# irecsys/CARSKit

Measured on AMD Instinct MI355X. Metric: SGD rating-updates/sec, CAMF_CI k=128, higher is better.
Workload: dtype f32

## Files before the change

carskit_amd/capi.py:

```python
import ctypes as C
import os

import numpy as np

_HERE = os.path.dirname(os.path.abspath(__file__))
LIB_PATH = os.environ.get("CMI_LIB_PATH") or os.path.join(_HERE, "lib", "libcarskit_mi355x.so")

OK, E_INVALID, E_NO_DEVICE, E_HIP, E_NUMERIC, E_UNSUPPORTED, E_HOST, E_BUSY = 0, -1, -2, -3, -4, -5, -6, -7

MODEL_IDS = {"BiasedMF": 0, "CAMF_C": 1, "CAMF_CI": 2, "CAMF_CU": 3, "CAMF_CUCI": 4, "PMF": 5,
             "SVD++": 6, "CAMF_ICS": 7, "CAMF_LCS": 8, "CAMF_MCS": 9}
STATE_IDS = {"P": 0, "Q": 1, "userBias": 2, "itemBias": 3, "condBias": 4, "ucBias": 5, "icBias": 6,
             "Y": 7, "ccMatrix": 8, "cfMatrix": 9, "cVector": 10}
MODEL_STATES = {
    "BiasedMF": ("P", "Q", "userBias", "itemBias"),
    "CAMF_C": ("P", "Q", "userBias", "itemBias", "condBias"),
    "CAMF_CI": ("P", "Q", "userBias", "icBias"),
    "CAMF_CU": ("P", "Q", "itemBias", "ucBias"),
    "CAMF_CUCI": ("P", "Q", "ucBias", "icBias"),
    "PMF": ("P", "Q"),
    "SVD++": ("P", "Q", "userBias", "itemBias", "Y"),
    "CAMF_ICS": ("P", "Q", "ccMatrix"),
    "CAMF_LCS": ("P", "Q", "cfMatrix"),
    "CAMF_MCS": ("P", "Q", "cVector"),
# ... 19 lines not shown
    ("cmi_abi_version", C.c_int, []),
    ("cmi_device_count", C.c_int, []),
    ("cmi_create", C.c_int, [C.c_int, C.c_int, C.c_int, C.c_int, C.c_int, C.c_int, C.c_uint, C.POINTER(_vp)]),
    ("cmi_destroy", C.c_int, [_vp]),
    ("cmi_last_error", C.c_char_p, [_vp]),
    ("cmi_set_ratings", C.c_int, [_vp, _i64, _vp, _vp, _vp, _vp, _i32, _vp, _vp]),
    ("cmi_set_state", C.c_int, [_vp, C.c_int, _vp, _i64, C.c_int]),
    ("cmi_get_state", C.c_int, [_vp, C.c_int, _vp, _i64, C.c_int]),
    ("cmi_set_sim_params", C.c_int, [_vp, C.c_int, C.c_int, _vp, C.c_int]),
    ("cmi_set_hparams", C.c_int, [_vp, _dbl, _dbl, _dbl, _dbl, _dbl]),
    ("cmi_set_device_share", C.c_int, [_vp, C.c_int]),
    ("cmi_train_epoch", C.c_int, [_vp, _dbl, C.POINTER(_dbl)]),
    ("cmi_train", C.c_int, [_vp, C.c_int, _dbl, _dbl, C.c_int, _dbl, C.c_int, _vp, _vp, C.POINTER(C.c_int),
                            C.POINTER(_dbl)]),
    ("cmi_train_from", C.c_int, [_vp, C.c_int, _dbl, C.c_int, _dbl, _dbl, C.c_int, _dbl, C.c_int, _vp, _vp, C.POINTER(C.c_int),
                                 C.POINTER(_dbl)]),
    ("cmi_predict_batch", C.c_int, [_vp, _i64, _vp, _vp, _vp, C.c_int, _dbl, _dbl, _vp]),
    ("cmi_eval_ratings", C.c_int, [_vp, _i64, _vp, _vp, _vp, _vp, _dbl, _dbl, _vp, C.POINTER(_i64)]),
    ("cmi_set_eval_ratings", C.c_int, [_vp, _i64, _vp, _vp, _vp, _vp]),
    ("cmi_eval_resident", C.c_int, [_vp, _dbl, _dbl, _vp, C.POINTER(_i64)]),
    ("cmi_eval_rankings", C.c_int, [_vp, _i64, _vp, _vp, _vp, _vp, _i64, _vp, _vp, _vp, _vp, _dbl, C.c_int, C.c_int,
                                    C.c_int, _vp, C.POINTER(_i64), _vp, _vp, _vp, _vp, _vp]),
    ("cmi_fm_eval_rankings", C.c_int, [_vp, _i64, _vp, _vp, _vp, _vp, _i64, _vp, _vp, _vp, _vp, _dbl, C.c_int, C.c_int,
                                       C.c_int, _vp, C.POINTER(_i64), _vp, _vp, _vp, _vp, _vp]),
    ("cmi_last_rank_ms", C.c_int, [_vp, C.POINTER(C.c_float), C.POINTER(_dbl)]),
    ("cmi_last_rank_host_ms", C.c_int, [_vp, _vp]),
    ("cmi_last_rank_kernel_ms", C.c_int, [_vp, _vp]),
    ("cmi_group_set_eval_ratings", C.c_int, [_vp, _i64, _vp, _vp, _vp, _vp]),
    ("cmi_group_eval_resident", C.c_int, [_vp, _dbl, _dbl, _vp, C.POINTER(_i64)]),
    ("cmi_comm_unique_id", C.c_int, [_vp]),
    ("cmi_comm_init", C.c_int, [_vp, _vp, C.c_int, C.c_int]),
    ("cmi_comm_exchange", C.c_int, [_vp, _dbl]),
    ("cmi_comm_train_epoch", C.c_int, [_vp, _dbl, _dbl, C.POINTER(_dbl)]),
    ("cmi_comm_last_exchange_ms", C.c_int, [_vp, C.POINTER(C.c_float)]),
    ("cmi_rank_plan", C.c_int, [C.c_int32, C.c_int32, _i64, _vp, _vp, _vp, _vp, _i64, _vp, _vp, _vp, _vp, _dbl, C.c_int,
                                C.POINTER(_i64), _vp, _vp, _vp, _vp, _vp, _vp, _vp]),
    ("cmi_rank_list_measures", C.c_int, [_vp, C.c_int, _vp, C.c_int, C.c_int, C.c_int, _vp]),
    ("cmi_narrow_runs", C.c_int, [_i64, _vp, _i64, _i64, _vp, C.POINTER(_i64)]),
    ("cmi_conflict_free_blocks", C.c_int, [_i64, _vp, _vp, C.c_int32, C.c_int32, C.c_int32, _vp, _i64, C.POINTER(_i64)]),
    ("cmi_java_int_hashset_order", C.c_int, [_i64, _vp, _vp, C.POINTER(_i64)]),
    ("cmi_state_device_ptr", C.c_int, [_vp, C.c_int, C.POINTER(_vp), C.POINTER(_i64), C.POINTER(C.c_int)]),
    ("cmi_stream", C.c_int, [_vp, C.POINTER(_vp)]),
    ("cmi_synchronize", C.c_int, [_vp]),
    ("cmi_train_epoch_async", C.c_int, [_vp, _dbl]),
    ("cmi_last_loss", C.c_int, [_vp, C.POINTER(_dbl)]),
    ("cmi_save_model", C.c_int, [_vp, C.c_char_p, C.c_double, C.c_double, C.c_int]),
    ("cmi_load_model", C.c_int, [_vp, C.c_char_p, C.POINTER(C.c_double), C.POINTER(C.c_double), C.POINTER(C.c_int)]),
    ("cmi_measure_hbm", C.c_int, [C.c_int, _i64, C.POINTER(C.c_double)]),
    ("cmi_schedule_info", C.c_int, [_vp, C.POINTER(_i64)]),
    ("cmi_schedule_traffic", C.c_int, [_vp, C.POINTER(_i64)]),
    ("cmi_schedule_note", C.c_char_p, [_vp]),
    ("cmi_arena_positions", C.c_int, [_i64, _vp, _i32, _vp, _vp]),
    ("cmi_exchange_setup", C.c_int, [_vp, _i64, C.POINTER(_vp), C.POINTER(_i64)]),
    ("cmi_group_create", C.c_int, [C.c_int, C.c_int, C.c_int, C.c_int, C.c_int, C.c_int, _vp, C.c_uint, C.POINTER(_vp)]),
    ("cmi_group_destroy", C.c_int, [_vp]),
    ("cmi_group_last_error", C.c_char_p, [_vp]),
    ("cmi_group_size", C.c_int, [_vp]),
    ("cmi_group_set_hparams", C.c_int, [_vp, C.c_double, C.c_double, C.c_double, C.c_double, C.c_double]),
    ("cmi_group_set_ratings", C.c_int, [_vp, _i64, _vp, _vp, _vp, _vp, _i32, _vp, _vp]),
    ("cmi_group_set_state", C.c_int, [_vp, C.c_int, _vp, _i64, C.c_int]),
    ("cmi_group_get_state", C.c_int, [_vp, C.c_int, _vp, _i64, C.c_int]),
    ("cmi_group_train_epoch", C.c_int, [_vp, C.c_double, C.POINTER(C.c_double)]),
    ("cmi_group_set_lr_scale", C.c_int, [_vp, C.c_double]),
    ("cmi_group_train", C.c_int, [_vp, C.c_int, C.c_double, C.c_double, C.c_int, C.c_double, C.c_int, _vp, _vp, C.POINTER(C.c_int),
                                  C.POINTER(C.c_double)]),
    ("cmi_group_train_from", C.c_int, [_vp, C.c_int, C.c_double, C.c_int, C.c_double, C.c_double, C.c_int, C.c_double, C.c_int, _vp, _vp,
                                       C.POINTER(C.c_int), C.POINTER(C.c_double)]),
    ("cmi_group_eval_ratings", C.c_int, [_vp, _i64, _vp, _vp, _vp, _vp, C.c_double, C.c_double, _vp, C.POINTER(_i64)]),
    ("cmi_group_predict_batch", C.c_int, [_vp, _i64, _vp, _vp, _vp, C.c_int, C.c_double, C.c_double, _vp]),
    ("cmi_group_shard_info", C.c_int, [_vp, C.c_int, C.POINTER(_i64)]),
    ("cmi_group_last_times", C.c_int, [_vp, C.POINTER(C.c_float), C.POINTER(C.c_float)]),
    ("cmi_group_exchange_path", C.c_char_p, [_vp]),
    ("cmi_group_member", C.c_int, [_vp, C.c_int, C.POINTER(_vp)]),
    ("cmi_exchange_pack", C.c_int, [_vp]),
    ("cmi_exchange_apply", C.c_int, [_vp, C.c_double]),
    ("cmi_loss_device_ptr", C.c_int, [_vp, C.POINTER(_vp)]),
    ("cmi_last_epoch_ms", C.c_int, [_vp, C.POINTER(C.c_float)]),
    ("cmi_level_schedule", C.c_int, [_i64, _vp, _vp, _i32, _i32, C.c_int, _vp, _vp, _i64, C.POINTER(_i64)]),
    ("cmi_owner_schedule", C.c_int, [_i64, _vp, _vp, _i32, _i32, C.c_int, C.c_int, C.c_int, _vp, _vp, _vp, _vp, C.POINTER(C.c_int)]),
    ("cmi_chain_schedule", C.c_int, [_i64, _vp, _vp, _i32, _i32, C.c_int, C.c_int, _vp, _vp, _i64, _vp, _i64, C.POINTER(_i64),
                                     C.POINTER(_i64), C.POINTER(C.c_int)]),
    ("cmi_chain_schedule_device", C.c_int, [C.c_int, _i64, _vp, _vp, _i32, _i32, C.c_int, C.c_int, _vp, _vp, _i64, _vp, _i64, C.POINTER(_i64),
                                     C.POINTER(_i64), C.POINTER(C.c_int)]),
    ("cmi_dao_read", C.c_int, [C.c_char_p, C.POINTER(_vp)]),
    ("cmi_dao_read_shared", C.c_int, [C.c_char_p, _vp, C.POINTER(_vp)]),
    ("cmi_dao_destroy", C.c_int, [_vp]),
    ("cmi_dao_last_error", C.c_char_p, [_vp]),
    ("cmi_dao_counts", C.c_int, [_vp, C.POINTER(_i64)]),
    ("cmi_dao_matrix", C.c_int, [_vp, _vp, _vp, _vp]),
    ("cmi_dao_ui_maps", C.c_int, [_vp, _vp, _vp]),
    ("cmi_dao_ctx_nnz", _i64, [_vp]),
    ("cmi_dao_ctx_table", C.c_int, [_vp, _vp, _vp]),
    ("cmi_dao_cond_info", C.c_int, [_vp, _vp, _vp, C.POINTER(_i32)]),
    ("cmi_dao_rating_scale", C.c_int, [_vp, _vp, _i32, C.POINTER(_i32)]),
    ("cmi_dao_raw_id", C.c_char_p, [_vp, C.c_int, _i32]),
    ("cmi_java_hashmap_order", C.c_int, [_i64, _vp, _vp, C.POINTER(C.c_int)]),
    ("cmi_transform_compact_to_binary", C.c_int, [C.c_char_p, C.c_char_p, C.POINTER(C.c_int)]),
    ("cmi_validate_data_format", C.c_int, [C.c_char_p]),
    ("cmi_transform", C.c_int, [C.c_char_p, C.c_char_p, C.c_char_p, C.c_char_p, C.POINTER(C.c_int)]),
    ("cmi_fm_create", C.c_int, [C.c_int, C.c_int, C.c_int, C.c_int, C.c_int, C.c_int, C.c_uint, C.POINTER(_vp)]),
    ("cmi_fm_destroy", C.c_int, [_vp]),
    ("cmi_fm_last_error", C.c_char_p, [_vp]),
    ("cmi_fm_set_hparams", C.c_int, [_vp, _dbl, _dbl, _i64]),
    ("cmi_fm_set_ratings", C.c_int, [_vp, _i64, _vp, _vp, _vp, _vp]),
    ("cmi_fm_set_model", C.c_int, [_vp, _dbl, _vp, _vp]),
    ("cmi_fm_get_model", C.c_int, [_vp, C.POINTER(_dbl), _vp, _vp]),
    ("cmi_fm_init", C.c_int, [_vp]),
    ("cmi_fm_sweep", C.c_int, [_vp]),
    ("cmi_fm_train", C.c_int, [_vp, C.c_int]),
    ("cmi_fm_predict_batch", C.c_int, [_vp, _i64, _vp, _vp, _vp, C.c_int, _dbl, _dbl, _vp]),
    ("cmi_knn_measure", C.c_int, [C.c_char_p]),
    ("cmi_knn_create", C.c_int, [C.c_int, C.c_int, C.c_int, C.c_int, C.c_uint, C.POINTER(_vp)]),
    ("cmi_knn_destroy", C.c_int, [_vp]),
    ("cmi_knn_last_error", C.c_char_p, [_vp]),
    ("cmi_knn_set_ratings", C.c_int, [_vp, _i64, _vp, _vp, _vp]),
    ("cmi_knn_build", C.c_int, [_vp, C.c_int, C.c_int, _dbl, _dbl]),
    ("cmi_knn_get_similarity", C.c_int, [_vp, C.c_int32, C.c_int32, _vp]),
    ("cmi_knn_predict_batch", C.c_int, [_vp, _i64, _vp, _vp, C.c_int, _dbl, C.c_int, _dbl, _dbl, _vp]),
    ("cmi_knn_last_build_ms", C.c_int, [_vp, C.POINTER(C.c_float)]),
    ("cmi_fm_synchronize", C.c_int, [_vp]),
    ("cmi_fm_stream", C.c_int, [_vp, C.POINTER(_vp)]),
    ("cmi_fm_num_phases", C.c_int, [_vp]),
    ("cmi_fm_phase_reduce", C.c_int, [_vp, C.c_int]),
    ("cmi_fm_phase_buffer", C.c_int, [_vp, C.c_int, C.POINTER(_vp), C.POINTER(_i64)]),
    ("cmi_fm_phase_apply", C.c_int, [_vp, C.c_int]),
    ("cmi_fm_phase_run", C.c_int, [_vp, C.c_int]),
    ("cmi_fm_layout", C.c_int, [_vp, _vp]),
    ("cmi_fm_comm_init", C.c_int, [_vp, _vp, C.c_int, C.c_int]),
    ("cmi_fm_comm_sweep", C.c_int, [_vp]),
    ("cmi_fm_time_reduce", C.c_int, [_vp, C.c_int, C.c_int, C.POINTER(_dbl)]),
]

_LIB = None


RANK_MEASURES = ("Pre5", "Pre10", "PreN", "Rec5", "Rec10", "RecN", "AUC5", "AUC10", "AUCN", "MAP5", "MAP10", "MAPN",
                 "NDCG5", "NDCG10", "NDCGN", "MRR5", "MRR10", "MRRN", "D5", "D10", "DN")


def java_int_hashset_order(values):
    v = np.ascontiguousarray(values, dtype=np.int32)
    out, n = np.zeros(max(len(v), 1), np.int32), _i64()
    rc = lib().cmi_java_int_hashset_order(len(v), _p(v), _p(out), C.byref(n))
    if rc:
        raise CmiError(rc, "cmi_java_int_hashset_order")
    return out[:n.value].copy()


def narrow_runs(level_off, max_tuples=256, min_levels=16):
    off = np.ascontiguousarray(level_off, dtype=np.int64)
    run = np.zeros(max(len(off) - 1, 1), np.int32)
    nl = _i64()
    rc = lib().cmi_narrow_runs(len(off) - 1, _p(off), max_tuples, min_levels, _p(run), C.byref(nl))
    if rc:
        raise CmiError(rc, "cmi_narrow_runs")
    return run[:len(off) - 1].copy(), nl.value


def conflict_free_blocks(u, j, n_users, n_items, max_block=64):
    u = np.ascontiguousarray(u, dtype=np.int32)
    j = np.ascontiguousarray(j, dtype=np.int32)
    nb = _i64()
    rc = lib().cmi_conflict_free_blocks(len(u), _p(u), _p(j), n_users, n_items, max_block, None, 0, C.byref(nb))
    if rc:
        raise CmiError(rc, "cmi_conflict_free_blocks")
    off = np.zeros(nb.value + 1, np.int32)
    rc = lib().cmi_conflict_free_blocks(len(u), _p(u), _p(j), n_users, n_items, max_block, _p(off), len(off), C.byref(nb))
    if rc:
        raise CmiError(rc, "cmi_conflict_free_blocks")
    return off


def rank_list_measures(ranked, truth, num_dropped, num_recs):
    rk = np.ascontiguousarray(ranked, dtype=np.int32)
    tr = np.ascontiguousarray(sorted(set(truth)), dtype=np.int32)
    out = np.zeros(18)
    rc = lib().cmi_rank_list_measures(_p(rk), len(rk), _p(tr), len(tr), int(num_dropped), int(num_recs), _p(out))
    if rc:
        raise CmiError(rc, "cmi_rank_list_measures")
    return dict(zip(RANK_MEASURES[:18], out.tolist()))


def rank_plan(n_users, n_items, train, test, bin_thold=-1.0, num_ignore=0):
    c32 = lambda a: np.ascontiguousarray(a, dtype=np.int32)
    f64 = lambda a: np.ascontiguousarray(a, dtype=np.float64)
    tu, tj, tc, tr = c32(train[0]), c32(train[1]), c32(train[2]), f64(train[3])
    su, sj, sc, sr = c32(test[0]), c32(test[1]), c32(test[2]), f64(test[3])
    sizes = (_i64 * 4)()
    args = (n_users, n_items, len(tu), _p(tu), _p(tj), _p(tc), _p(tr), len(su), _p(su), _p(sj), _p(sc), _p(sr), float(bin_thold),
            int(num_ignore), sizes)
    rc = lib().cmi_rank_plan(*args, None, None, None, None, None, None, None)
    if rc:
        raise CmiError(rc, "cmi_rank_plan")
    nc, nq, nt, ne = list(sizes)
    cand, qu, qc = np.zeros(max(nc, 1), np.int32), np.zeros(max(nq, 1), np.int32), np.zeros(max(nq, 1), np.int32)
    tp, ti = np.zeros(nq + 1, np.int64), np.zeros(max(nt, 1), np.int32)
    ep, ei = np.zeros(nq + 1, np.int64), np.zeros(max(ne, 1), np.int32)
    rc = lib().cmi_rank_plan(*args, _p(cand), _p(qu), _p(qc), _p(tp), _p(ti), _p(ep), _p(ei))
    if rc:
        raise CmiError(rc, "cmi_rank_plan")
    queries = [(int(qu[q]), int(qc[q]), ti[tp[q]:tp[q + 1]].tolist(), ei[ep[q]:ep[q + 1]].tolist()) for q in range(nq)]
    return cand[:nc].tolist(), queries


COMM_ID_BYTES = 128


def comm_unique_id():
    buf = (C.c_char * COMM_ID_BYTES)()
    rc = lib().cmi_comm_unique_id(buf)
    if rc:
        raise CmiError(rc, "cmi_comm_unique_id")
    return bytes(buf)


class CmiError(RuntimeError):
    def __init__(self, code, msg):
        super().__init__("libcarskit_mi355x error %d: %s" % (code, msg))
        self.code = code


def lib():
    global _LIB
    if _LIB is None:
        if not os.path.exists(LIB_PATH):
            raise OSError("%s not found: build it with `python __graft_entry__.py` or `make -C carskit_amd/csrc` "
                          "(there is no Python/CPU fallback for the compute path)" % LIB_PATH)
        L = C.CDLL(LIB_PATH)
        for name, res, args in SYMBOLS:
            fn = getattr(L, name)
            fn.restype = res
            fn.argtypes = args
        _LIB = L
    return _LIB


def device_count():
    return lib().cmi_device_count()


def _p(a):
    return None if a is None else a.ctypes.data_as(C.c_void_p)


def measure_hbm(device=0, nbytes=4 << 30):
    out = (C.c_double * 2)()
    rc = lib().cmi_measure_hbm(device, nbytes, out)
    if rc != OK:
        raise CmiError(rc, "cmi_measure_hbm")
    return float(out[0]), float(out[1])


def level_schedule(u, j, n_users, n_items, order=0):
    u = np.ascontiguousarray(u, dtype=np.int32)
    j = np.ascontiguousarray(j, dtype=np.int32)
    n = len(u)
    nl = _i64()
    rc = lib().cmi_level_schedule(n, _p(u), _p(j), n_users, n_items, order, None, None, 0, C.byref(nl))
    if rc != OK:
        raise CmiError(rc, "cmi_level_schedule")
    perm = np.empty(n, dtype=np.int32)
    off = np.empty(nl.value + 1, dtype=np.int64)
    rc = lib().cmi_level_schedule(n, _p(u), _p(j), n_users, n_items, order, _p(perm), _p(off), len(off), C.byref(nl))
    if rc != OK:
        raise CmiError(rc, "cmi_level_schedule")
    return perm, off


def chain_schedule(u, j, n_users, n_items, hub=-1, max_chain=16):
    u = np.ascontiguousarray(u, dtype=np.int32)
    j = np.ascontiguousarray(j, dtype=np.int32)
    n = len(u)
    nu, nl, hub_used = _i64(), _i64(), C.c_int()
    rc = lib().cmi_chain_schedule(n, _p(u), _p(j), n_users, n_items, hub, max_chain, None, None, 0, None, 0, C.byref(nu),
                                  C.byref(nl), C.byref(hub_used))
    if rc != OK:
        raise CmiError(rc, "cmi_chain_schedule")
    perm = np.empty(n, dtype=np.int32)
    unit_off = np.empty(nu.value + 1, dtype=np.int32)
    level_off = np.empty(nl.value + 1, dtype=np.int64)
    rc = lib().cmi_chain_schedule(n, _p(u), _p(j), n_users, n_items, hub, max_chain, _p(perm), _p(unit_off), len(unit_off),
                                  _p(level_off), len(level_off), C.byref(nu), C.byref(nl), C.byref(hub_used))
    if rc != OK:
        raise CmiError(rc, "cmi_chain_schedule")
    return perm, unit_off, level_off, bool(hub_used.value)


def chain_schedule_device(u, j, n_users, n_items, hub=-1, max_chain=16, device=0):
    u = np.ascontiguousarray(u, dtype=np.int32)
    j = np.ascontiguousarray(j, dtype=np.int32)
    n = len(u)
    nu, nl, hub_used = _i64(), _i64(), C.c_int()
    rc = lib().cmi_chain_schedule(n, _p(u), _p(j), n_users, n_items, hub, max_chain, None, None, 0, None, 0, C.byref(nu), C.byref(nl), C.byref(hub_used))
    if rc != OK:
        raise CmiError(rc, "cmi_chain_schedule")
    perm = np.empty(n, dtype=np.int32)
    unit_off = np.empty(nu.value + 1, dtype=np.int32)
    level_off = np.empty(nl.value + 1, dtype=np.int64)
    rc = lib().cmi_chain_schedule_device(device, n, _p(u), _p(j), n_users, n_items, hub, max_chain, _p(perm), _p(unit_off), len(unit_off),
                                         _p(level_off), len(level_off), C.byref(nu), C.byref(nl), C.byref(hub_used))
    if rc != OK:
        raise CmiError(rc, "cmi_chain_schedule_device")
    return perm, unit_off[:nu.value + 1], level_off[:nl.value + 1], bool(hub_used.value)


def owner_schedule(u, j, n_users, n_items, n_owners, hub=-1, depth=8):
    u = np.ascontiguousarray(u, dtype=np.int32)
    j = np.ascontiguousarray(j, dtype=np.int32)
    n = len(u)
    perm = np.empty(n, dtype=np.int32)
    own_off = np.empty(n_owners + 1, dtype=np.int64)
    want = np.empty(n, dtype=np.uint32)
    flags = np.empty(n, dtype=np.uint32)
    hub_used = C.c_int()
    rc = lib().cmi_owner_schedule(n, _p(u), _p(j), n_users, n_items, hub, n_owners, depth, _p(perm), _p(own_off), _p(want), _p(flags),
                                  C.byref(hub_used))
    if rc != OK:
        raise CmiError(rc, "cmi_owner_schedule")
    return perm, own_off, want, flags, bool(hub_used.value)


def arena_positions(spoke, n_spokes):
    spoke = np.ascontiguousarray(spoke, dtype=np.int32)
    nxt, first = np.empty(len(spoke), dtype=np.int32), np.empty(n_spokes, dtype=np.int32)
    rc = lib().cmi_arena_positions(len(spoke), _p(spoke), n_spokes, _p(nxt), _p(first))
    if rc != OK:
        raise CmiError(rc, "cmi_arena_positions")
    return nxt, first


def _eval_rankings(fn, chk, h, train, test, bin_thold=-1.0, num_recs=10, num_ignore=0, strategy="ucu", with_lists=False):
    c32 = lambda a: np.ascontiguousarray(a, dtype=np.int32)
    f64 = lambda a: np.ascontiguousarray(a, dtype=np.float64)
    tu, tj, tc, tr = c32(train[0]), c32(train[1]), c32(train[2]), f64(train[3])
    su, sj, sc, sr = c32(test[0]), c32(test[1]), c32(test[2]), f64(test[3])
    out, nq = np.zeros(len(RANK_MEASURES)), _i64()
    n = max(len(su), 1)
    if with_lists:
        qu, qc, qn = (np.zeros(n, np.int32) for _ in range(3))
        items, scores = np.zeros(n * num_recs, np.int32), np.zeros(n * num_recs)
    else:
        qu = qc = qn = items = scores = None
    chk(fn(h, len(tu), _p(tu), _p(tj), _p(tc), _p(tr), len(su), _p(su), _p(sj), _p(sc),
                                       _p(sr), float(bin_thold), int(num_recs), int(num_ignore),
                                       {"ucu": 0, "uc": 1}[strategy], _p(out), C.byref(nq), _p(qu), _p(qc), _p(qn),
                                       _p(items), _p(scores)))
    res = dict(zip(RANK_MEASURES, out.tolist()))
    res["n_queries"] = nq.value
    if not with_lists:
        return res
    lists = {}
    for q in range(nq.value):
        if qn[q] > 0:
            lists[(int(qu[q]), int(qc[q]))] = [(int(items[q * num_recs + i]), float(scores[q * num_recs + i]))
                                               for i in range(qn[q])]
    return res, lists


class _Handle:

    _api = ("", "", "")

    def __init__(self, *args):
        self.L = lib()
        create, _, last_error = (getattr(self.L, n) for n in self._api)
        self.h = _vp()
        rc = create(*args, C.byref(self.h))
        if rc != OK:
            self.h = None
            raise CmiError(rc, last_error(None).decode())

    def _chk(self, rc):
        if rc != OK:
            raise CmiError(rc, getattr(self.L, self._api[2])(self.h).decode())

    def close(self):
        if getattr(self, "h", None):
            getattr(self.L, self._api[1])(self.h)
            self.h = None

    def __del__(self):
        try:
            self.close()
        except Exception:
            pass

# ... 141 lines not shown
        r = np.ascontiguousarray(r, dtype=np.float64)
        n_ctx = 0 if ctx_ptr is None else len(ctx_ptr) - 1
        self._chk(self.L.cmi_set_ratings(self.h, len(r), _p(u), _p(j), _p(ctx), _p(r), n_ctx, _p(ctx_ptr),
                                         _p(ctx_conds)))

    def set_state(self, name, arr):
        a = np.ascontiguousarray(arr)
        if a.dtype not in (np.float32, np.float64):
            a = a.astype(np.float64)
        self._chk(self.L.cmi_set_state(self.h, STATE_IDS[name], _p(a), a.size, 1 if a.dtype == np.float64 else 0))

    def set_states(self, state):
        for name, arr in state.items():
            if arr is not None:
                self.set_state(name, arr)

    def state_shape(self, name):
        return {"P": (self.n_users, self.k), "Q": (self.n_items, self.k), "userBias": (self.n_users,),
                "itemBias": (self.n_items,), "condBias": (self.n_conds,), "ucBias": (self.n_users, self.n_conds),
                "icBias": (self.n_items, self.n_conds), "Y": (self.n_items, self.k), "ccMatrix": (self.n_conds, self.n_conds),
                "cfMatrix": (self.n_conds, self.num_f), "cVector": (self.n_conds,)}[name]

    def get_state(self, name, dtype=np.float64):
        out = np.empty(self.state_shape(name), dtype=dtype)
        self._chk(self.L.cmi_get_state(self.h, STATE_IDS[name], _p(out), out.size, 1 if dtype == np.float64 else 0))
        return out

    def get_states(self, dtype=np.float64):
        return {name: self.get_state(name, dtype) for name in MODEL_STATES[self.model]}

    def set_hparams(self, regU, regI, regB, regC, global_mean):
        self._chk(self.L.cmi_set_hparams(self.h, regU, regI, regB, regC, global_mean))

    def set_device_share(self, instances):
        self._chk(self.L.cmi_set_device_share(self.h, int(instances)))

    def train_epoch(self, lrate):
        loss = _dbl()
        self._chk(self.L.cmi_train_epoch(self.h, lrate, C.byref(loss)))
        return loss.value

    def train_epoch_async(self, lrate):
        self._chk(self.L.cmi_train_epoch_async(self.h, lrate))

    def last_loss(self):
        loss = _dbl()
        self._chk(self.L.cmi_last_loss(self.h, C.byref(loss)))
        return loss.value

    def train(self, num_iters, init_lrate, max_lrate=-1.0, bold_driver=False, decay=-1.0, early_stop=0, first_iter=1,
              prev_loss=0.0):
        losses, lrs = np.zeros(num_iters), np.zeros(num_iters)
        n, final = C.c_int(0), _dbl(0)
        rc = self.L.cmi_train_from(self.h, first_iter, prev_loss, num_iters, init_lrate, max_lrate, int(bold_driver), decay,
                                   early_stop, _p(losses), _p(lrs), C.byref(n), C.byref(final))
        self.iters_run, self.final_lrate = n.value, final.value
        self._chk(rc)
        return losses[:n.value], lrs[:n.value]

    def synchronize(self):
        self._chk(self.L.cmi_synchronize(self.h))

    def stream_ptr(self):
        p = _vp()
        self._chk(self.L.cmi_stream(self.h, C.byref(p)))
        return p.value

    def last_epoch_ms(self):
        ms = C.c_float()
        self._chk(self.L.cmi_last_epoch_ms(self.h, C.byref(ms)))
        return ms.value

    def schedule_info(self):
        info = (_i64 * 8)()
        self._chk(self.L.cmi_schedule_info(self.h, info))
        d = dict(zip(("levels", "max_level", "tuples", "dmax", "state_bytes", "tuple_bytes", "kind", "flow_blocks"),
                     list(info)))
        d["kind"] = ("level", "serial", "flow", "two-lane", "chain-item", "chain-user", "owner-item", "owner-user")[d["kind"]]
        if d["kind"].startswith("owner"):
            d["teams"] = d["flow_blocks"] >> 32
            d["flow_blocks"] &= 0xffffffff
        return d

    def schedule_note(self):
        return self.L.cmi_schedule_note(self.h).decode()

    def schedule_traffic(self):
        out = (_i64 * 4)()
        self._chk(self.L.cmi_schedule_traffic(self.h, out))
        return {"sector": out[0], "own": out[1], "algorithmic": out[2], "models_reuse": bool(out[3] & 1), "spoke_arena": bool(out[3] & 2)}

    def stream(self):
        s = _vp()
        self._chk(self.L.cmi_stream(self.h, C.byref(s)))
        return s.value

    def save_model(self, path, lrate=0.0, last_loss=0.0, epochs_done=0):
        self._chk(self.L.cmi_save_model(self.h, str(path).encode(), lrate, last_loss, epochs_done))

    def load_model(self, path):
        lr, ll, ep = C.c_double(), C.c_double(), C.c_int()
        self._chk(self.L.cmi_load_model(self.h, str(path).encode(), C.byref(lr), C.byref(ll), C.byref(ep)))
        if self.model == "CAMF_LCS" and self.n_conds > 0:
            self.num_f = self.state_device_ptr("cfMatrix")[1] // self.n_conds
        return lr.value, ll.value, ep.value

    def exchange_setup(self, pad_to=1):
        ptr, cnt = _vp(), _i64()
        self._chk(self.L.cmi_exchange_setup(self.h, pad_to, C.byref(ptr), C.byref(cnt)))
        return ptr.value, cnt.value, (np.float64 if self.flags & FLAG_STATE_F64 else np.float32)

    def exchange_pack(self):
        self._chk(self.L.cmi_exchange_pack(self.h))

    def exchange_apply(self, scale):
        self._chk(self.L.cmi_exchange_apply(self.h, float(scale)))

    def loss_device_ptr(self):
        p = _vp()
        self._chk(self.L.cmi_loss_device_ptr(self.h, C.byref(p)))
        return p.value

    def comm_init(self, unique_id, rank, world):
        buf = (C.c_char * COMM_ID_BYTES).from_buffer_copy(bytes(unique_id))
        self._chk(self.L.cmi_comm_init(self.h, buf, int(rank), int(world)))

    def comm_last_exchange_ms(self):
        ms = C.c_float()
        self._chk(self.L.cmi_comm_last_exchange_ms(self.h, C.byref(ms)))
        return ms.value

    def comm_exchange(self, scale):
        self._chk(self.L.cmi_comm_exchange(self.h, float(scale)))

    def comm_train_epoch(self, lrate, scale):
        loss = _dbl()
        self._chk(self.L.cmi_comm_train_epoch(self.h, float(lrate), float(scale), C.byref(loss)))
        return loss.value

    def state_device_ptr(self, name):
        ptr, cnt, dt = _vp(), _i64(), C.c_int()
        self._chk(self.L.cmi_state_device_ptr(self.h, STATE_IDS[name], C.byref(ptr), C.byref(cnt), C.byref(dt)))
        return ptr.value, cnt.value, (np.float64 if dt.value else np.float32)

    def predict(self, u, j, ctx=None, bound=None):
        c32 = lambda a: None if a is None else np.ascontiguousarray(a, dtype=np.int32)
        u, j, ctx = c32(u), c32(j), c32(ctx)
        out = np.empty(len(u))
        lo, hi = bound if bound else (0.0, 0.0)
        self._chk(self.L.cmi_predict_batch(self.h, len(u), _p(u), _p(j), _p(ctx), 1 if bound else 0, lo, hi, _p(out)))
        return out

    def eval_ratings(self, u, j, ctx, r, min_rate, max_rate):
        c32 = lambda a: None if a is None else np.ascontiguousarray(a, dtype=np.int32)
        u, j, ctx = c32(u), c32(j), c32(ctx)
        r = np.ascontiguousarray(r, dtype=np.float64)
        out, cnt = np.zeros(5), _i64()
        self._chk(self.L.cmi_eval_ratings(self.h, len(r), _p(u), _p(j), _p(ctx), _p(r), min_rate, max_rate, _p(out),
                                          C.byref(cnt)))
        res = dict(zip(("MAE", "RMSE", "NMAE", "rMAE", "rRMSE"), out.tolist()))
        res["n"] = cnt.value
        return res

    def set_eval_ratings(self, u, j, ctx, r):
        c32 = lambda a: None if a is None else np.ascontiguousarray(a, dtype=np.int32)
        u, j, ctx = c32(u), c32(j), c32(ctx)
# ... 173 lines not shown
```

carskit_amd/csrc/chain_kernels.hip:

```cpp
#include "mf_sgd_kernels.hpp"
#include "sgd_device.hpp"

#include <cstdlib>

namespace cmi {

template <typename T>
struct Vec16;
template <>
struct Vec16<float> {
    typedef float4 type;
    static constexpr int E = 4;
};
template <>
struct Vec16<double> {
    typedef double2 type;
    static constexpr int E = 2;
};
__device__ __forceinline__ void unpack(const float4 &v, float *x) { x[0] = v.x, x[1] = v.y, x[2] = v.z, x[3] = v.w; }
__device__ __forceinline__ void unpack(const double2 &v, double *x) { x[0] = v.x, x[1] = v.y; }
__device__ __forceinline__ float4 pack(const float *x) { return make_float4(x[0], x[1], x[2], x[3]); }
__device__ __forceinline__ double2 pack(const double *x) { return make_double2(x[0], x[1]); }

__device__ __forceinline__ void chain_lds_order() { asm volatile("" ::: "memory"); }

template <typename T, int NV>
struct SpokeRow {
    typename Vec16<T>::type v[NV];
    T sc;
    T *psc;
    int spoke, cond;
    T *dst;
};

template <typename T, int MODEL, int NV, bool RAGGED, bool HUB_ITEM>
__device__ __forceinline__ void chain_load_spoke(const SgdArgs<T> &a, int spoke, int cond, int l16, int K, SpokeRow<T, NV> &r, int64_t pos = 0,
                                                 int nx = 0) {
    using M = Traits<MODEL>;
    using V = typename Vec16<T>::type;
    constexpr int E = Vec16<T>::E;
    constexpr bool SC = HUB_ITEM ? M::has_uc : M::has_ic;
    T *tab = HUB_ITEM ? a.P : a.Q;
    const T *src = a.arena ? a.arena + (size_t)pos * K : tab + (size_t)spoke * K;
    r.dst = a.arena ? a.arena + (size_t)nx * K : tab + (size_t)spoke * K;
    const V *row = reinterpret_cast<const V *>(src) + l16;
    r.spoke = spoke;
    r.cond = cond;
#pragma unroll
    for (int v = 0; v < NV; ++v) {
        T z[E];
#pragma unroll
        for (int c = 0; c < E; ++c) z[c] = (T)0;
        r.v[v] = pack(z);
        if (!RAGGED || E * l16 + 16 * E * v < K) r.v[v] = row[v * 16];
    }
    r.sc = (T)0;
    r.psc = nullptr;
    if (SC && cond >= 0) {
        r.psc = (HUB_ITEM ? a.ucBias : a.icBias) + (size_t)spoke * a.n_conds + cond;
        r.sc = *r.psc;
    }
}

template <typename T>
struct ChainHp {
    T lr, regU, regI, regB, regC, gm;
};

template <typename T, int MODEL, int NV, bool RAGGED, bool HUB_ITEM>
__device__ __forceinline__ void chain_step(const SgdArgs<T> &a, const ChainHp<T> &hp, T (&h)[NV][Vec16<T>::E], T &hb, T *s_hc, T *s_sb,
                                           const SpokeRow<T, NV> &cur, T rr, int l16, int K, double &gloss) {
    using M = Traits<MODEL>;
    using V = typename Vec16<T>::type;
    constexpr int E = Vec16<T>::E;
    constexpr bool HB = HUB_ITEM ? M::has_bj : M::has_bu;
    constexpr bool SB = HUB_ITEM ? M::has_bu : M::has_bj;
    constexpr bool HC = HUB_ITEM ? M::has_ic : M::has_uc;
    constexpr bool SC = HUB_ITEM ? M::has_uc : M::has_ic;
    const T lr = hp.lr, regU = hp.regU, regI = hp.regI, regB = hp.regB, regC = hp.regC;

    T sp[NV][E];
#pragma unroll
    for (int v = 0; v < NV; ++v) unpack(cur.v[v], sp[v]);
    T part = (T)0;
#pragma unroll
    for (int v = 0; v < NV; ++v)
#pragma unroll
        for (int c = 0; c < E; ++c) part += HUB_ITEM ? sp[v][c] * h[v][c] : h[v][c] * sp[v][c];
    const T dot = row_sum16(part);

    T hcv = (T)0;
    if (HC) {
        chain_lds_order();
        if (cur.cond >= 0) hcv = s_hc[cur.cond];
    }
    const T sbv = SB ? *s_sb : (T)0;
    const T bu = HUB_ITEM ? sbv : hb, bj = HUB_ITEM ? hb : sbv;
    const T bic = HUB_ITEM ? hcv : cur.sc, buc = HUB_ITEM ? cur.sc : hcv;
    T pred = hp.gm;
    if (M::has_bu) pred += bu;
    if (M::has_bj) pred += bj;
    pred += dot;
    if (M::has_ctx) {
        T term = (T)0;
        if (M::has_ic && M::has_uc) term = bic + buc;
        else if (M::has_ic) term = bic;
        else if (M::has_uc) term = buc;
        pred += row_sum16(term);
    }
    const T e = rr - pred;

    if (HB) hb = hb + lr * (e - regB * hb);
    if (SB && l16 == 0) *s_sb = sbv + lr * (e - regB * sbv);
    T ctx_loss = (T)0;
    if (cur.cond >= 0) {
        if (M::has_ic) ctx_loss += bic * bic;
        if (M::has_uc) ctx_loss += buc * buc;
        if (HC) s_hc[cur.cond] = hcv + lr * (e - regC * hcv);
        if (SC) *cur.psc = cur.sc + lr * (e - regC * cur.sc);
    }
    if (HC) chain_lds_order();

    T lsum = (T)0;
    V *srow = reinterpret_cast<V *>(cur.dst) + l16;
#pragma unroll
    for (int v = 0; v < NV; ++v) {
        T sn[E];
#pragma unroll
        for (int c = 0; c < E; ++c) {
            const T p = HUB_ITEM ? sp[v][c] : h[v][c], q = HUB_ITEM ? h[v][c] : sp[v][c];
            const T pn = p + lr * (e * q - regU * p);
            const T qn = q + lr * (e * p - regI * q);
            lsum += (regU * p) * p + (regI * q) * q;
            h[v][c] = HUB_ITEM ? qn : pn;
            sn[c] = HUB_ITEM ? pn : qn;
        }
        if (!RAGGED || E * l16 + 16 * E * v < K) srow[v * 16] = pack(sn);
    }
    const T reg_loss = row_sum16(lsum);
    const T ctx_sum = M::has_ctx ? row_sum16(ctx_loss) : (T)0;
    if (l16 == 0) {
        double l = (double)e * (double)e;
        if (M::has_bu) l += (double)regB * bu * bu;
        if (M::has_bj) l += (double)regB * bj * bj;
        if (M::has_ctx) l += (double)regC * ctx_sum;
        gloss += l + (double)reg_loss;
    }
}

__host__ __device__ inline size_t chain_group_lds(int n_conds_hub, int dmax, size_t esize) {
    size_t b = (size_t)n_conds_hub * esize + 32 * esize + 32 * 4 + (size_t)16 * (dmax > 0 ? dmax : 0) * 4;
    return (b + 15) & ~(size_t)15;
}

template <typename T>
struct ChainPre {
    int32_t tb, len;
    int hub, sp0, cd0, my_sp, my_nx, nx0;
    T my_rr;
    int cdv[4];
};

template <typename T, bool HAS_CTX, bool HUB_ITEM>
__device__ __forceinline__ ChainPre<T> chain_prefetch_ids(const SgdArgs<T> &a, int32_t tb, int32_t te, int l16, int dmax) {
    ChainPre<T> p;
    p.tb = tb;
    p.len = te - tb;
    p.hub = HUB_ITEM ? a.sj[tb] : a.su[tb];
    p.sp0 = HUB_ITEM ? a.su[tb] : a.sj[tb];
    p.cd0 = (HAS_CTX && l16 < dmax) ? a.sconds[(int64_t)tb * dmax + l16] : -1;
    p.my_sp = 0;
    p.my_nx = 0;
    p.my_rr = (T)0;
    p.nx0 = a.next_pos ? a.next_pos[tb] : 0;
    if (l16 < p.len) {
        p.my_sp = HUB_ITEM ? a.su[tb + l16] : a.sj[tb + l16];
        p.my_rr = a.sr[tb + l16];
        if (a.next_pos) p.my_nx = a.next_pos[tb + l16];
    }
    const int n_cd = p.len * dmax;
#pragma unroll
    for (int r = 0; r < 4; ++r) {
        p.cdv[r] = -1;
        if (l16 + 16 * r < n_cd) p.cdv[r] = a.sconds[(int64_t)tb * dmax + l16 + 16 * r];
    }
    return p;
}

template <typename T, int MODEL, int NV, bool RAGGED, bool HUB_ITEM>
__device__ __forceinline__ void chain_unit(const SgdArgs<T> &a, const ChainHp<T> &hp, const ChainPre<T> &pre, unsigned char *gbase, int l16,
                                           int K, int dmax, double &gloss) {
    using M = Traits<MODEL>;
    using V = typename Vec16<T>::type;
    constexpr int E = Vec16<T>::E;
    constexpr bool HB = HUB_ITEM ? M::has_bj : M::has_bu;
    constexpr bool HC = HUB_ITEM ? M::has_ic : M::has_uc;
    constexpr bool SB = HUB_ITEM ? M::has_bu : M::has_bj;
    const int len = pre.len;
    const int32_t tb = pre.tb;
    T *s_hc = reinterpret_cast<T *>(gbase);
    T *s_rr = s_hc + (HC ? a.n_conds : 0);
    T *s_sb = s_rr + 16;
    int *s_sp = reinterpret_cast<int *>(s_sb + 16);
    int *s_nx = s_sp + 16;
    int *s_cd = s_nx + 16;
    const int n_cd = len * dmax;

    T *htab = HUB_ITEM ? a.Q : a.P;
    V *hrow = reinterpret_cast<V *>(htab + (size_t)pre.hub * K) + l16;
    T h[NV][E];
#pragma unroll
    for (int v = 0; v < NV; ++v) {
#pragma unroll
        for (int c = 0; c < E; ++c) h[v][c] = (T)0;
        if (!RAGGED || E * l16 + 16 * E * v < K) {
            const V t = hrow[v * 16];
            unpack(t, h[v]);
        }
    }
    T hb = (T)0;
    T *phb = nullptr;
    if (HB) {
        phb = (HUB_ITEM ? a.itemBias : a.userBias) + pre.hub;
        hb = *phb;
    }
    T *hc_row = nullptr;
    T hcv4[4];
    if (HC) {
        hc_row = (HUB_ITEM ? a.icBias : a.ucBias) + (size_t)pre.hub * a.n_conds;
#pragma unroll
        for (int r = 0; r < 4; ++r) {
            hcv4[r] = (T)0;
            if (l16 + 16 * r < a.n_conds) hcv4[r] = hc_row[l16 + 16 * r];
        }
    }
    T *sb_tab = HUB_ITEM ? a.userBias : a.itemBias;
    T my_sb = (T)0;
    if (SB && l16 < len) my_sb = sb_tab[pre.my_sp];
    SpokeRow<T, NV> A, B;
    chain_load_spoke<T, MODEL, NV, RAGGED, HUB_ITEM>(a, pre.sp0, pre.cd0, l16, K, A, tb, pre.nx0);

    if (l16 < len) {
        s_sp[l16] = pre.my_sp;
        s_nx[l16] = pre.my_nx;
        s_rr[l16] = pre.my_rr;
        if (SB) s_sb[l16] = my_sb;
    }
#pragma unroll
    for (int r = 0; r < 4; ++r)
        if (l16 + 16 * r < n_cd) s_cd[l16 + 16 * r] = pre.cdv[r];
    for (int c = l16 + 64; c < n_cd; c += 16) s_cd[c] = a.sconds[(int64_t)tb * dmax + c];
    if (HC) {
#pragma unroll
        for (int r = 0; r < 4; ++r)
            if (l16 + 16 * r < a.n_conds) s_hc[l16 + 16 * r] = hcv4[r];
        for (int c = l16 + 64; c < a.n_conds; c += 16) s_hc[c] = hc_row[c];
    }
    chain_lds_order();

    __builtin_amdgcn_s_waitcnt(0x0F70);
    const int pairs = len >> 1;
    for (int t = 0; t < pairs; ++t) {
        const int i = 2 * t;
        chain_load_spoke<T, MODEL, NV, RAGGED, HUB_ITEM>(a, s_sp[i + 1], l16 < dmax ? s_cd[(i + 1) * dmax + l16] : -1, l16, K, B, tb + i + 1, s_nx[i + 1]);
        chain_lds_order();
        chain_step<T, MODEL, NV, RAGGED, HUB_ITEM>(a, hp, h, hb, s_hc, s_sb + i, A, s_rr[i], l16, K, gloss);
        {
            const int nx = i + 2 < len ? i + 2 : len - 1;
            chain_load_spoke<T, MODEL, NV, RAGGED, HUB_ITEM>(a, s_sp[nx], l16 < dmax ? s_cd[nx * dmax + l16] : -1, l16, K, A, tb + nx, s_nx[nx]);
        }
        chain_lds_order();
        chain_step<T, MODEL, NV, RAGGED, HUB_ITEM>(a, hp, h, hb, s_hc, s_sb + i + 1, B, s_rr[i + 1], l16, K, gloss);
    }
    if (len & 1) chain_step<T, MODEL, NV, RAGGED, HUB_ITEM>(a, hp, h, hb, s_hc, s_sb + len - 1, A, s_rr[len - 1], l16, K, gloss);

#pragma unroll
    for (int v = 0; v < NV; ++v)
        if (!RAGGED || E * l16 + 16 * E * v < K) hrow[v * 16] = pack(h[v]);
    if (HB && l16 == 0) *phb = hb;
    if (SB) {
        chain_lds_order();
        if (l16 < len) sb_tab[s_sp[l16]] = s_sb[l16];
    }
    if (HC) {
        chain_lds_order();
        for (int c = l16; c < a.n_conds; c += 16) hc_row[c] = s_hc[c];
    }
}

template <typename T, int MODEL, int NV, bool RAGGED, bool HUB_ITEM>
__global__ __launch_bounds__(256) void sgd_chain_level(SgdArgs<T> a, const int32_t *__restrict__ unit_off, int64_t ubegin, int count,
                                                       int64_t slot0) {
    using M = Traits<MODEL>;
    constexpr int E = Vec16<T>::E;
    static_assert(MODEL != CAMF_C, "CAMF_C has no level schedule (shared condBias)");
    constexpr bool HC = HUB_ITEM ? M::has_ic : M::has_uc;
    extern __shared__ __attribute__((aligned(16))) unsigned char chain_smem[];
    __shared__ double s_loss[16];
    const int tid = threadIdx.x, l16 = tid & 15, gib = tid >> 4;
    const int g = blockIdx.x * 16 + gib;
    const int K = RAGGED ? a.k : NV * 16 * E;
    const int dmax = M::has_ctx ? a.dmax : 0;
    double gloss = 0.0;
    const HParams hpd = *a.hp;
    const ChainHp<T> hp{(T)hpd.lr, (T)hpd.regU, (T)hpd.regI, (T)hpd.regB, (T)hpd.regC, (T)hpd.gm};

    if (g < count) {
        const int32_t tb = unit_off[ubegin + g], te = unit_off[ubegin + g + 1];
        const ChainPre<T> pre = chain_prefetch_ids<T, M::has_ctx, HUB_ITEM>(a, tb, te, l16, dmax);
        chain_unit<T, MODEL, NV, RAGGED, HUB_ITEM>(a, hp, pre, chain_smem + (size_t)gib * chain_group_lds(HC ? a.n_conds : 0, dmax, sizeof(T)),
                                                   l16, K, dmax, gloss);
    }

    if (l16 == 0) s_loss[gib] = gloss;
    __syncthreads();
    if (tid == 0) {
        double s = 0.0;
#pragma unroll
        for (int i = 0; i < 16; ++i) s += s_loss[i];
        a.loss_part[slot0 + blockIdx.x] = s;
    }
}

struct SmallSpoke {
    float v[4];
    float sb, sc;
    float *psc;
    int spoke, cond;
};

template <int MODEL, int LPT, bool HUB_ITEM>
__device__ __forceinline__ void small_load_spoke(const SgdArgs<float> &a, int spoke, int cond, int lt, int k, SmallSpoke &r) {
    using M = Traits<MODEL>;
    constexpr bool SB = HUB_ITEM ? M::has_bu : M::has_bj;
    constexpr bool SC = HUB_ITEM ? M::has_uc : M::has_ic;
    const float *row = (HUB_ITEM ? a.P : a.Q) + (size_t)spoke * k + lt;
    r.spoke = spoke;
    r.cond = cond;
#pragma unroll
    for (int v = 0; v < 4; ++v) {
        r.v[v] = 0.f;
        if (lt + v * LPT < k) r.v[v] = row[v * LPT];
    }
    r.sb = r.sc = 0.f;
    r.psc = nullptr;
    if (SB) r.sb = (HUB_ITEM ? a.userBias : a.itemBias)[spoke];
    if (SC && cond >= 0) {
        r.psc = (HUB_ITEM ? a.ucBias : a.icBias) + (size_t)spoke * a.n_conds + cond;
        r.sc = *r.psc;
    }
}

template <int MODEL, int LPT, bool HUB_ITEM>
__device__ __forceinline__ void small_step(const SgdArgs<float> &a, const ChainHp<float> &hp, float (&h)[4], float &hb, float *s_hc,
                                           const SmallSpoke &cur, float rr, int lt, int k, double &gloss) {
    using M = Traits<MODEL>;
    constexpr bool HB = HUB_ITEM ? M::has_bj : M::has_bu;
    constexpr bool SB = HUB_ITEM ? M::has_bu : M::has_bj;
    constexpr bool HC = HUB_ITEM ? M::has_ic : M::has_uc;
    constexpr bool SC = HUB_ITEM ? M::has_uc : M::has_ic;
    const float lr = hp.lr, regU = hp.regU, regI = hp.regI, regB = hp.regB, regC = hp.regC;
    float part = 0.f;
#pragma unroll
    for (int v = 0; v < 4; ++v) part += HUB_ITEM ? cur.v[v] * h[v] : h[v] * cur.v[v];
    const float dot = group_sum<LPT>(part);
    float hcv = 0.f;
    if (HC) {
        chain_lds_order();
        if (cur.cond >= 0) hcv = s_hc[cur.cond];
    }
    const float bu = HUB_ITEM ? cur.sb : hb, bj = HUB_ITEM ? hb : cur.sb;
    const float bic = HUB_ITEM ? hcv : cur.sc, buc = HUB_ITEM ? cur.sc : hcv;
    float pred = hp.gm;
    if (M::has_bu) pred += bu;
    if (M::has_bj) pred += bj;
    pred += dot;
    if (M::has_ctx) {
        float term = 0.f;
        if (M::has_ic && M::has_uc) term = bic + buc;
        else if (M::has_ic) term = bic;
        else if (M::has_uc) term = buc;
        pred += group_sum<LPT>(term);
    }
    const float e = rr - pred;
    if (HB) hb = hb + lr * (e - regB * hb);
    if (SB && lt == 0) (HUB_ITEM ? a.userBias : a.itemBias)[cur.spoke] = cur.sb + lr * (e - regB * cur.sb);
    float ctx_loss = 0.f;
    if (cur.cond >= 0) {
        if (M::has_ic) ctx_loss += bic * bic;
        if (M::has_uc) ctx_loss += buc * buc;
        if (HC) s_hc[cur.cond] = hcv + lr * (e - regC * hcv);
        if (SC) *cur.psc = cur.sc + lr * (e - regC * cur.sc);
    }
    if (HC) chain_lds_order();
    float lsum = 0.f;
    float *srow = (HUB_ITEM ? a.P : a.Q) + (size_t)cur.spoke * k + lt;
#pragma unroll
    for (int v = 0; v < 4; ++v)
        if (lt + v * LPT < k) {
            const float pv = HUB_ITEM ? cur.v[v] : h[v], qv = HUB_ITEM ? h[v] : cur.v[v];
            const float pn = pv + lr * (e * qv - regU * pv);
            const float qn = qv + lr * (e * pv - regI * qv);
            lsum += (regU * pv) * pv + (regI * qv) * qv;
            h[v] = HUB_ITEM ? qn : pn;
            srow[v * LPT] = HUB_ITEM ? pn : qn;
        }
    const float reg_loss = group_sum<LPT>(lsum);
    const float ctx_sum = M::has_ctx ? group_sum<LPT>(ctx_loss) : 0.f;
    if (lt == 0) {
        double l = (double)e * (double)e;
        if (M::has_bu) l += (double)regB * bu * bu;
        if (M::has_bj) l += (double)regB * bj * bj;
        if (M::has_ctx) l += (double)regC * ctx_sum;
        gloss += l + (double)reg_loss;
    }
}

template <int MODEL, int LPT, bool HUB_ITEM>
__global__ __launch_bounds__(256) void sgd_chain_small(SgdArgs<float> a, const int32_t *__restrict__ unit_off, int64_t ubegin, int count,
                                                       int64_t slot0) {
    using M = Traits<MODEL>;
    static_assert(MODEL != CAMF_C, "CAMF_C has no level schedule (shared condBias)");
    constexpr bool HB = HUB_ITEM ? M::has_bj : M::has_bu;
    constexpr bool HC = HUB_ITEM ? M::has_ic : M::has_uc;
    constexpr int GPB = 256 / LPT;
    extern __shared__ __attribute__((aligned(16))) unsigned char chain_smem[];
    __shared__ double s_loss[GPB];
    const int tid = threadIdx.x, lt = tid % LPT, gib = tid / LPT;
    const int g = blockIdx.x * GPB + gib;
    const int k = a.k;
    const int dmax = M::has_ctx ? a.dmax : 0;
    double gloss = 0.0;
    const HParams hpd = *a.hp;
    const ChainHp<float> hp{(float)hpd.lr, (float)hpd.regU, (float)hpd.regI, (float)hpd.regB, (float)hpd.regC, (float)hpd.gm};

    if (g < count) {
        const int32_t tb = unit_off[ubegin + g], te = unit_off[ubegin + g + 1];
        const int len = te - tb;
        unsigned char *gbase = chain_smem + (size_t)gib * chain_group_lds(HC ? a.n_conds : 0, dmax, sizeof(float));
        float *s_hc = reinterpret_cast<float *>(gbase);
        float *s_rr = s_hc + (HC ? a.n_conds : 0);
        int *s_sp = reinterpret_cast<int *>(s_rr + 16);
        int *s_cd = s_sp + 16;
        const int n_cd = len * dmax;

        const int hub = HUB_ITEM ? a.sj[tb] : a.su[tb];
        const int sp0 = HUB_ITEM ? a.su[tb] : a.sj[tb];
        const int cd0 = lt < dmax ? a.sconds[(int64_t)tb * dmax + lt] : -1;
        int my_sp[16 / LPT];
        float my_rr[16 / LPT];
#pragma unroll
        for (int r = 0; r < 16 / LPT; ++r) {
            my_sp[r] = 0;
            my_rr[r] = 0.f;
            if (lt + r * LPT < len) {
                my_sp[r] = HUB_ITEM ? a.su[tb + lt + r * LPT] : a.sj[tb + lt + r * LPT];
                my_rr[r] = a.sr[tb + lt + r * LPT];
            }
        }
        int cdv[4];
#pragma unroll
        for (int r = 0; r < 4; ++r) {
            cdv[r] = -1;
            if (lt + r * LPT < n_cd) cdv[r] = a.sconds[(int64_t)tb * dmax + lt + r * LPT];
        }
        float *hrow = (HUB_ITEM ? a.Q : a.P) + (size_t)hub * k + lt;
        float h[4];
#pragma unroll
        for (int v = 0; v < 4; ++v) {
            h[v] = 0.f;
            if (lt + v * LPT < k) h[v] = hrow[v * LPT];
        }
        float hb = 0.f;
        float *phb = nullptr;
        if (HB) {
            phb = (HUB_ITEM ? a.itemBias : a.userBias) + hub;
            hb = *phb;
        }
        float *hc_row = HC ? (HUB_ITEM ? a.icBias : a.ucBias) + (size_t)hub * a.n_conds : nullptr;
        SmallSpoke A, B;
        small_load_spoke<MODEL, LPT, HUB_ITEM>(a, sp0, cd0, lt, k, A);
#pragma unroll
        for (int r = 0; r < 16 / LPT; ++r)
            if (lt + r * LPT < len) {
                s_sp[lt + r * LPT] = my_sp[r];
                s_rr[lt + r * LPT] = my_rr[r];
            }
#pragma unroll
        for (int r = 0; r < 4; ++r)
            if (lt + r * LPT < n_cd) s_cd[lt + r * LPT] = cdv[r];
        for (int c = lt + 4 * LPT; c < n_cd; c += LPT) s_cd[c] = a.sconds[(int64_t)tb * dmax + c];
        if (HC)
            for (int c = lt; c < a.n_conds; c += LPT) s_hc[c] = hc_row[c];
        chain_lds_order();

        int i = 0;
        while (true) {
            if (i + 1 < len) small_load_spoke<MODEL, LPT, HUB_ITEM>(a, s_sp[i + 1], lt < dmax ? s_cd[(i + 1) * dmax + lt] : -1, lt, k, B);
            small_step<MODEL, LPT, HUB_ITEM>(a, hp, h, hb, s_hc, A, s_rr[i], lt, k, gloss);
            if (++i >= len) break;
            if (i + 1 < len) small_load_spoke<MODEL, LPT, HUB_ITEM>(a, s_sp[i + 1], lt < dmax ? s_cd[(i + 1) * dmax + lt] : -1, lt, k, A);
            small_step<MODEL, LPT, HUB_ITEM>(a, hp, h, hb, s_hc, B, s_rr[i], lt, k, gloss);
            if (++i >= len) break;
        }
#pragma unroll
        for (int v = 0; v < 4; ++v)
            if (lt + v * LPT < k) hrow[v * LPT] = h[v];
        if (HB && lt == 0) *phb = hb;
        if (HC) {
            chain_lds_order();
            for (int c = lt; c < a.n_conds; c += LPT) hc_row[c] = s_hc[c];
        }
    }
    if (lt == 0) s_loss[gib] = gloss;
    __syncthreads();
    if (tid < 64) {
        double sum = 0.0;
        for (int q = tid; q < GPB; q += 64) sum += s_loss[q];
        sum = wave_sum64(sum);
        if (tid == 0) a.loss_part[slot0 + blockIdx.x] = sum;
    }
}

template <typename T, bool TO_ARENA>
__global__ __launch_bounds__(256) void arena_rows_kernel(T *table, T *arena, const int32_t *__restrict__ first_pos, int64_t n_rows, int k) {
    using V = typename Vec16<T>::type;
    constexpr int E = Vec16<T>::E;
    const int vec_per_row = k / E;
    const int64_t i = (int64_t)blockIdx.x * blockDim.x + threadIdx.x;
    const int64_t row = i / vec_per_row;
// ... 14 lines not shown
    return hipGetLastError();
}
template <typename T>
hipError_t launch_arena_gather(T *table, const T *arena, const int32_t *first_pos, int64_t n_rows, int k, hipStream_t s) {
    const int64_t n = n_rows * (k / Vec16<T>::E);
    if (n <= 0) return hipSuccess;
    hipLaunchKernelGGL((arena_rows_kernel<T, false>), dim3((unsigned)((n + 255) / 256)), dim3(256), 0, s, table, const_cast<T *>(arena), first_pos, n_rows, k);
    return hipGetLastError();
}
template hipError_t launch_arena_scatter<float>(const float *, float *, const int32_t *, int64_t, int, hipStream_t);
template hipError_t launch_arena_scatter<double>(const double *, double *, const int32_t *, int64_t, int, hipStream_t);
template hipError_t launch_arena_gather<float>(float *, const float *, const int32_t *, int64_t, int, hipStream_t);
template hipError_t launch_arena_gather<double>(double *, const double *, const int32_t *, int64_t, int, hipStream_t);


bool has_chain_path(int model, int k, int dmax, int n_conds, bool f64, bool strict) {
    if (strict || model == CAMF_C) return false;
    if (dmax > 16) return false;
    if (f64) {
        if (k < 32 || k > 256 || k % 2 != 0) return false;
    } else {
        if (k > 256 || (k >= 64 && k % 4 != 0)) return false;
    }
    const int groups = chain_groups_per_block(k, dmax, f64);
    if (groups * chain_lds_bytes(model, n_conds, dmax, f64, true) / 16 > 64 * 1024 || groups * chain_lds_bytes(model, n_conds, dmax, f64, false) / 16 > 64 * 1024)
        return false;
    return true;
}

size_t chain_lds_bytes(int model, int n_conds, int dmax, bool f64, bool hub_is_item) {
    const ModelParams mp = model_params(model);
    const bool hc = hub_is_item ? mp.has_ic : mp.has_uc;
    return 16 * chain_group_lds(hc ? n_conds : 0, mp.has_ctx ? dmax : 0, f64 ? 8 : 4);
}

int chain_groups_per_block(int k, int dmax, bool f64) { return (!f64 && k < 64) ? 256 / small_lpt(k, dmax) : 16; }
int chain_level_blocks(int k, int dmax, bool f64, int count) {
    const int g = chain_groups_per_block(k, dmax, f64);
    return (count + g - 1) / g;
}

template <typename T, int MODEL, int NV, bool RAGGED>
static void *chain_kernel_hub(bool hub_is_item) {
    return hub_is_item ? (void *)sgd_chain_level<T, MODEL, NV, RAGGED, true> : (void *)sgd_chain_level<T, MODEL, NV, RAGGED, false>;
}

template <typename T, int MODEL>
static void *chain_kernel_k(int k, bool hub_is_item) {
    constexpr int E = Vec16<T>::E;
    const int per = 16 * E;
    if (k % per == 0) {
        switch (k / per) {
        case 1: return chain_kernel_hub<T, MODEL, 1, false>(hub_is_item);
        case 2: return chain_kernel_hub<T, MODEL, 2, false>(hub_is_item);
        case 4: return chain_kernel_hub<T, MODEL, 4, false>(hub_is_item);
        case 8: if (E == 2) return chain_kernel_hub<T, MODEL, 8, false>(hub_is_item); break;
        }
    }
    const int nv = (k + per - 1) / per;
    if (nv <= 2) return chain_kernel_hub<T, MODEL, 2, true>(hub_is_item);
    if (nv <= 3) return chain_kernel_hub<T, MODEL, 3, true>(hub_is_item);
    if (nv <= 4) return chain_kernel_hub<T, MODEL, 4, true>(hub_is_item);
    if (E == 2) {
        if (nv <= 6) return chain_kernel_hub<T, MODEL, 6, true>(hub_is_item);
        if (nv <= 8) return chain_kernel_hub<T, MODEL, 8, true>(hub_is_item);
    }
    return nullptr;
}

template <int MODEL, int LPT>
static void *chain_small_hub(bool hub_is_item) {
    return hub_is_item ? (void *)sgd_chain_small<MODEL, LPT, true> : (void *)sgd_chain_small<MODEL, LPT, false>;
}
template <int MODEL>
static void *chain_small_lpt_ptr(int lpt, bool hub_is_item) {
    switch (lpt) {
    case 4: return chain_small_hub<MODEL, 4>(hub_is_item);
    case 8: return chain_small_hub<MODEL, 8>(hub_is_item);
    default: return chain_small_hub<MODEL, 16>(hub_is_item);
    }
}

template <typename T>
hipError_t launch_chain_level(const SgdArgs<T> &a, const LaunchCfg &cfg, bool hub_is_item, const int32_t *unit_off, int64_t ubegin,
                              int count, int64_t slot0, hipStream_t s) {
    if (count <= 0) return hipSuccess;
    const bool f64 = sizeof(T) == 8;
    const int groups = chain_groups_per_block(a.k, a.dmax, f64);
    void *fn = dispatch_model<ModelSet::PARALLEL>(cfg.model, (void *)nullptr, [&](auto m) {
        constexpr int MODEL = decltype(m)::value;
        return (!f64 && a.k < 64) ? chain_small_lpt_ptr<MODEL>(256 / groups, hub_is_item) : chain_kernel_k<T, MODEL>(a.k, hub_is_item);
    });
    if (!fn) return hipErrorInvalidValue;
    SgdArgs<T> args = a;
    void *params[] = {&args, &unit_off, &ubegin, &count, &slot0};
    const size_t lds = (size_t)groups * (chain_lds_bytes(cfg.model, a.n_conds, a.dmax, f64, hub_is_item) / 16);
    return hipLaunchKernel(fn, dim3((unsigned)chain_level_blocks(a.k, a.dmax, f64, count)), dim3(256), params, lds, s);
}
template hipError_t launch_chain_level<float>(const SgdArgs<float> &, const LaunchCfg &, bool, const int32_t *, int64_t, int, int64_t,
                                              hipStream_t);
template hipError_t launch_chain_level<double>(const SgdArgs<double> &, const LaunchCfg &, bool, const int32_t *, int64_t, int, int64_t,
                                               hipStream_t);

}
```

carskit_amd/csrc/cmi_api.cpp:

```cpp
#include "../../include/carskit_mi355x.h"

#include <hip/hip_runtime.h>

#include <algorithm>
#include <chrono>
#include <cmath>
#include <cstdio>
#include <cstdlib>
#include <cstring>
#include <functional>
#include <initializer_list>
#include <string>
#include <condition_variable>
#include <mutex>
#include <vector>

#include "abi.hpp"
#include "cmi_instance.hpp"
#include "host_pool.hpp"
#include "level_schedule.hpp"
#include "sched_device.hpp"
#include "mf_sgd_kernels.hpp"

using namespace cmi;

std::string &cmi_thread_err() {
    static thread_local std::string err;
    return err;
}

#include "owner_gate.hpp"

bool cmi_model_has(int model, int which) {
    switch (which) {
    case CMI_STATE_P:
    case CMI_STATE_Q: return true;
    case CMI_STATE_USER_BIAS: return model == CMI_MODEL_BIASEDMF || model == CMI_MODEL_CAMF_C || model == CMI_MODEL_CAMF_CI || model == CMI_MODEL_SVDPP;
    case CMI_STATE_ITEM_BIAS: return model == CMI_MODEL_BIASEDMF || model == CMI_MODEL_CAMF_C || model == CMI_MODEL_CAMF_CU || model == CMI_MODEL_SVDPP;
    case CMI_STATE_Y: return model == CMI_MODEL_SVDPP;
    case CMI_STATE_CC_MATRIX: return model == CMI_MODEL_CAMF_ICS;
    case CMI_STATE_CF_MATRIX: return model == CMI_MODEL_CAMF_LCS;
    case CMI_STATE_C_VECTOR: return model == CMI_MODEL_CAMF_MCS;
    case CMI_STATE_COND_BIAS: return model == CMI_MODEL_CAMF_C;
    case CMI_STATE_UC_BIAS: return model == CMI_MODEL_CAMF_CU || model == CMI_MODEL_CAMF_CUCI;
    case CMI_STATE_IC_BIAS: return model == CMI_MODEL_CAMF_CI || model == CMI_MODEL_CAMF_CUCI;
    }
    return false;
}

static int64_t state_elems(const cmi_instance *h, int which) {
    switch (which) {
    case CMI_STATE_P: return (int64_t)h->n_users * h->k;
    case CMI_STATE_Q: return (int64_t)h->n_items * h->k;
    case CMI_STATE_USER_BIAS: return h->n_users;
    case CMI_STATE_ITEM_BIAS: return h->n_items;
    case CMI_STATE_COND_BIAS: return h->n_conds;
    case CMI_STATE_UC_BIAS: return (int64_t)h->n_users * h->n_conds;
    case CMI_STATE_IC_BIAS: return (int64_t)h->n_items * h->n_conds;
    case CMI_STATE_Y: return (int64_t)h->n_items * h->k;
    case CMI_STATE_CC_MATRIX: return (int64_t)h->n_conds * h->n_conds;
    case CMI_STATE_CF_MATRIX: return (int64_t)h->n_conds * h->num_f;
    case CMI_STATE_C_VECTOR: return h->n_conds;
    }
    return 0;
}

static size_t esize(const cmi_instance *h) { return h->f64 ? 8 : 4; }
static bool is_ext_model(int model) { return model >= CMI_MODEL_SVDPP && model <= CMI_MODEL_CAMF_MCS; }
static bool is_2d_model(int model) { return model == CMI_MODEL_BIASEDMF || model == CMI_MODEL_PMF || model == CMI_MODEL_SVDPP; }

extern "C" int cmi_abi_version(void) { return CMI_ABI_VERSION; }

extern "C" int cmi_device_count(void) {
    int n = 0;
    if (hipGetDeviceCount(&n) != hipSuccess) return 0;
    return n;
}

extern "C" const char *cmi_last_error(cmi_handle h) { return h ? h->err.c_str() : cmi_thread_err().c_str(); }

static void free_eval_set(cmi_instance *h) {
    abi_free(h->d_eu, h->d_ej, h->d_ectx, h->d_er, h->d_epart);
    h->n_eval = 0;
}

static void release_arena(cmi_instance *h) {
    abi_free(h->d_arena, h->d_next, h->d_first);
    h->arena_on = h->arena_valid = false;
    h->table_valid = true;
}

static void free_ratings(cmi_instance *h) {
    if (h->arena_on && h->arena_valid && !h->table_valid) cmi_sync_table_from_arena(h);
    release_arena(h);
    h->arena_probe = false;
    free_eval_set(h);
    if (h->graph_exec) {
        hipGraphExecDestroy(h->graph_exec);
        h->graph_exec = nullptr;
    }
    abi_free(h->d_su, h->d_sj, h->d_sconds, h->d_ctx_ptr, h->d_ctx_conds, h->d_sr, h->d_loss_part, h->d_flow_err, h->d_tail_off, h->d_blk_off,
             h->d_unit_off, h->d_ui_ptr, h->d_ui_items, h->d_own_recs, h->d_own_off, h->d_tagged);
    h->sched = Sched::NONE;
    h->level_kernel = LevelKernel::GENERIC;
    h->owner_stalled = false;
    h->n_units = 0;
    h->blk_off.clear();
    h->n_launches = h->n_tail = 0;
    h->tail_len.clear();
    h->have_ratings = false;
    h->n = 0;
}

extern "C" int cmi_destroy(cmi_handle h) {
    if (!h) return CMI_OK;
    hipSetDevice(h->device);
    if (h->stream) hipStreamSynchronize(h->stream);
    free_ratings(h);
    cmi_comm_release(h);
    h->rank_ws.release();
    for (void *&p : h->state) abi_free(p);
    abi_free(h->d_empty, h->d_xbucket, h->d_xsnap, h->d_scratch, h->d_loss, h->d_hp);
    if (h->h_loss) hipHostFree(h->h_loss);
    if (h->ev0) hipEventDestroy(h->ev0);
    if (h->ev1) hipEventDestroy(h->ev1);
    if (h->stream) hipStreamDestroy(h->stream);
    delete h;
    return CMI_OK;
}

extern "C" int cmi_create(int model, int k, int n_users, int n_items, int n_conds, int device, unsigned flags,
                          cmi_handle *out) {
    return abi_barrier(cmi_thread_err(), "cmi_create", [&] {
        if (out) *out = nullptr;
        if (!out || model < 0 || model > CMI_MODEL_CAMF_MCS || k <= 0 || n_users <= 0 || n_items <= 0 || n_conds < 0) {
            cmi_thread_err() = "cmi_create: invalid argument";
            return CMI_E_INVALID;
        }
        if (int rc = abi_check_device(cmi_thread_err(), "cmi_create", device)) return rc;
        if (model == CMI_MODEL_CAMF_C && !(flags & CMI_FLAG_SCHED_SERIAL)) {
            cmi_thread_err() =
                "cmi_create: CAMF_C updates the shared condBias vector on every tuple, so its tuples do not commute and "
                "no order-exact level schedule exists; pass CMI_FLAG_SCHED_SERIAL";
            return CMI_E_UNSUPPORTED;
        }
        if (is_ext_model(model) && !(flags & CMI_FLAG_SCHED_SERIAL)) {
            cmi_thread_err() =
                "cmi_create: SVD++ / CAMF_ICS / CAMF_LCS / CAMF_MCS update parameters shared by (nearly) every tuple, so no order-exact "
                "parallel schedule exists; pass CMI_FLAG_SCHED_SERIAL";
            return CMI_E_UNSUPPORTED;
        }
        cmi_instance *h = new cmi_instance();
        h->model = model;
        h->k = k;
        h->n_users = n_users;
        h->n_items = n_items;
        h->n_conds = n_conds;
        h->device = device;
        h->flags = flags;
        h->f64 = flags & CMI_FLAG_STATE_F64;
        h->strict = flags & CMI_FLAG_STRICT;
        h->use_graph = !(flags & CMI_FLAG_NO_GRAPH);
        const char *step = "";
        hipError_t e = hipSuccess;
    #define TRY(x)                                                                                          \
        if (e == hipSuccess) {                                                                              \
            step = #x;                                                                                      \
            e = (x);                                                                                        \
        }
        TRY(hipSetDevice(device));
        TRY(hipStreamCreateWithFlags(&h->stream, hipStreamNonBlocking));
        TRY(hipEventCreate(&h->ev0));
        TRY(hipEventCreate(&h->ev1));
        for (int w = 0; w < CMI_STATE_COUNT; ++w) {
            if (!cmi_model_has(model, w)) continue;
            h->state_count[w] = state_elems(h, w);
            size_t bytes = (size_t)h->state_count[w] * esize(h);
            if (bytes == 0) continue;
            TRY(hipMalloc(&h->state[w], bytes));
            TRY(hipMemsetAsync(h->state[w], 0, bytes, h->stream));
        }
        TRY(hipMalloc((void **)&h->d_scratch, 256 * sizeof(double)));
        TRY(hipMalloc((void **)&h->d_loss, sizeof(double)));
        TRY(hipMalloc((void **)&h->d_hp, sizeof(HParams)));
        TRY(hipHostMalloc((void **)&h->h_loss, sizeof(double), hipHostMallocDefault));
// ... 540 lines not shown
        if (h->tail_len[(size_t)l] > 0) blocks = 1;
        else if (h->tail_len[(size_t)l] < 0) blocks = 0;
        if (h->tail_len[(size_t)l] >= 0) ++h->n_launches;
        h->slot_off[(size_t)l + 1] = h->slot_off[(size_t)l] + blocks;
    }
    h->n_slots = h->slot_off[(size_t)n_levels];
    h->n_tail = 0;
    for (int32_t t : h->tail_len)
        if (t > 0) h->n_tail += t;
}

static void gather_stream(const cmi_instance *h, const RatingsIn &in, int dmax, const LevelSchedule &sch, HostStream &hs) {
    const int64_t ns = in.n;
    const int32_t *u = in.u, *j = in.j, *ctx = in.ctx;
    const double *r = in.r;
    hs.su = HostBuf<int32_t>((size_t)ns);
    hs.sj = HostBuf<int32_t>((size_t)ns);
    hs.sconds = HostBuf<int32_t>((size_t)ns * (size_t)dmax);
    hs.sr32 = HostBuf<float>(h->f64 ? 0 : (size_t)ns);
    hs.sr64 = HostBuf<double>(h->f64 ? (size_t)ns : 0);
    const bool in_order = in_input_order(h->sched);
    parallel_ranges(ns, host_threads(ns), [&](int, int64_t s0, int64_t s1) {
        for (int64_t s = s0; s < s1; ++s) {
            if (!in_order && s + 16 < s1) {
                const int64_t tp = sch.perm[(size_t)s + 16];
                if (tp >= 0) {
                    __builtin_prefetch(&u[tp]);
                    __builtin_prefetch(&j[tp]);
                    __builtin_prefetch(&r[tp]);
                    if (dmax > 0) __builtin_prefetch(&ctx[tp]);
                }
            }
            const int64_t t = in_order ? s : sch.perm[(size_t)s];
            int32_t *row = dmax > 0 ? &hs.sconds[(size_t)s * (size_t)dmax] : nullptr;
            if (t < 0) {
                hs.su[(size_t)s] = -1;
                hs.sj[(size_t)s] = 0;
                if (h->f64) hs.sr64[(size_t)s] = 0.0;
                else hs.sr32[(size_t)s] = 0.f;
                for (int d = 0; d < dmax; ++d) row[d] = -1;
                continue;
            }
            hs.su[(size_t)s] = u[t];
            hs.sj[(size_t)s] = j[t];
            if (h->f64) hs.sr64[(size_t)s] = r[t];
            else hs.sr32[(size_t)s] = (float)r[t];
            if (dmax > 0) {
                const int32_t b = in.ctx_ptr[ctx[t]], e = in.ctx_ptr[ctx[t] + 1];
                int d = 0;
                for (int32_t q = b; q < e; ++q) row[d++] = in.ctx_conds[q];
                for (; d < dmax; ++d) row[d] = -1;
            }
        }
    });
}

static hipError_t upload_stream(cmi_instance *h, const RatingsIn &in, int dmax, bool dev_stream, const HostStream &hs,
                                ChainDeviceKeep &keep, const ChainSchedule &csch) {
    const int64_t ns = in.n;
    hipError_t e = hipSuccess;
    if (!dev_stream) {
        e = abi_upload(&h->d_su, hs.su, h->stream);
        if (e == hipSuccess) e = abi_upload(&h->d_sj, hs.sj, h->stream);
        if (e == hipSuccess) e = abi_upload(&h->d_sconds, hs.sconds, h->stream);
        if (e == hipSuccess) e = h->f64 ? abi_upload(&h->d_sr, hs.sr64, h->stream) : abi_upload(&h->d_sr, hs.sr32, h->stream);
    }
    if (e == hipSuccess && !is_2d_model(h->model)) {
        std::vector<int32_t> cp(in.ctx_ptr, in.ctx_ptr + in.n_ctx + 1), cc(in.ctx_conds, in.ctx_conds + in.ctx_ptr[in.n_ctx]);
        h->ctx_nnz = (int64_t)cc.size();
        e = abi_upload(&h->d_ctx_ptr, cp, h->stream);
        if (e == hipSuccess) e = abi_upload(&h->d_ctx_conds, cc, h->stream);
        if (e == hipSuccess) e = hipStreamSynchronize(h->stream);
    }
    if (e == hipSuccess && dev_stream) {
        e = hipMalloc((void **)&h->d_su, (size_t)ns * 4);
        if (e == hipSuccess) e = hipMalloc((void **)&h->d_sj, (size_t)ns * 4);
        if (e == hipSuccess && dmax > 0) e = hipMalloc((void **)&h->d_sconds, (size_t)ns * (size_t)dmax * 4);
        if (e == hipSuccess) e = hipMalloc(&h->d_sr, (size_t)ns * esize(h));
        if (e == hipSuccess)
            e = (hipError_t)stream_build_device(h->stream, ns, keep.d_u, keep.d_j, keep.d_perm, in.ctx, in.r, h->d_ctx_ptr, h->d_ctx_conds, dmax,
                                                h->f64, h->d_su, h->d_sj, h->d_sconds, h->d_sr);
    }
    free_keep(keep);
    if (e == hipSuccess && h->sched == Sched::CHAIN) e = abi_upload(&h->d_unit_off, csch.unit_off, h->stream);
    return e;
}

static hipError_t setup_arena(cmi_instance *h, int64_t n, bool dev_stream, const HostStream &hs, SpecArena &spec) {
    if (h->sched != Sched::CHAIN || !arena_kernel_ok(h)) return hipSuccess;
    const int64_t spokes = h->chain_hub_item ? h->n_users : h->n_items;
    const size_t table_bytes = (size_t)spokes * (size_t)h->k * esize(h), arena_bytes = (size_t)n * (size_t)h->k * esize(h);
    size_t free_b = 0, total_b = 0;
    (void)hipMemGetInfo(&free_b, &total_b);
    if (spec.ptr && spec.bytes == arena_bytes) free_b += spec.bytes;
    const bool forced = h->flags & CMI_FLAG_SPOKE_ARENA;
    const bool large = table_bytes >= ((size_t)2 << 30) && (double)arena_bytes <= 0.6 * (double)free_b;
    const char *pe = getenv("CMI_ARENA_PROBE");
    const bool probe = !forced && !large && (pe ? atoi(pe) != 0 : (!h->strict && table_bytes >= ((size_t)256 << 20) && (double)arena_bytes <= 0.3 * (double)free_b));
    h->arena_probe = false;
    if (!forced && !large && !probe) return hipSuccess;
    const int32_t *d_spoke = h->chain_hub_item ? h->d_su : h->d_sj;
    hipError_t e = hipMalloc((void **)&h->d_next, (size_t)n * 4);
    if (e == hipSuccess) e = hipMalloc((void **)&h->d_first, (size_t)spokes * 4);
    if (e == hipSuccess && (hipError_t)arena_positions_device(h->stream, n, d_spoke, spokes, h->d_next, h->d_first) != hipSuccess) {
        (void)hipGetLastError();
        HostBuf<int32_t> nxt((size_t)n), first((size_t)spokes), back(dev_stream ? (size_t)n : 0);
        if (dev_stream) {
            e = hipMemcpyAsync(back.data(), d_spoke, (size_t)n * 4, hipMemcpyDeviceToHost, h->stream);
            if (e == hipSuccess) e = hipStreamSynchronize(h->stream);
        }
        if (e == hipSuccess) {
            const HostBuf<int32_t> &sp = dev_stream ? back : (h->chain_hub_item ? hs.su : hs.sj);
            arena_positions(n, sp.data(), spokes, nxt.data(), first.data());
            e = hipMemcpyAsync(h->d_next, nxt.data(), (size_t)n * 4, hipMemcpyHostToDevice, h->stream);
        }
        if (e == hipSuccess) e = hipMemcpyAsync(h->d_first, first.data(), (size_t)spokes * 4, hipMemcpyHostToDevice, h->stream);
        if (e == hipSuccess) e = hipStreamSynchronize(h->stream);
    }
    if (e == hipSuccess) {
        h->d_arena = spec.take(arena_bytes);
        if (!h->d_arena) e = hipMalloc(&h->d_arena, arena_bytes);
    }
    if (e == hipSuccess) e = hipStreamSynchronize(h->stream);
    if (e == hipSuccess) {
        h->arena_on = true;
        h->arena_valid = false;
        h->table_valid = true;
        h->arena_which = h->chain_hub_item ? CMI_STATE_P : CMI_STATE_Q;
        h->arena_probe = probe;
        h->arena_probe_table = pe && atoi(pe) < 0;
    } else if (!forced) {
        (void)hipGetLastError();
        release_arena(h);
        e = hipSuccess;
    }
    return e;
}

static hipError_t pack_owner_records(cmi_instance *h, const RatingsIn &in, const OwnerSchedule &osch, const LevelSchedule &sch) {
    const int64_t n = in.n;
    const int32_t n_spokes = h->owner_hub_item ? h->n_users : h->n_items;
    const int64_t rec_bytes = h->own_stride * 8;
    const int pad = 2 * owner_depth();
    const int ncw = owner_mask_words(h->model, h->n_conds);
    const size_t rb = owner_rec_bytes(ncw);
    std::vector<uint64_t> recs(((size_t)n + (size_t)h->n_owners * (size_t)pad) * (rb / 8), 0);
    auto put = [&](int64_t pos, uint32_t off, int32_t hub, uint32_t want, uint32_t flags, double rating, const uint64_t *mask) {
        unsigned char *q = reinterpret_cast<unsigned char *>(recs.data()) + (size_t)pos * rb;
        memcpy(q, &off, 4);
        memcpy(q + 4, &hub, 4);
        memcpy(q + 8, &want, 4);
        memcpy(q + 12, &flags, 4);
        if (h->f64) memcpy(q + 16, &rating, 8);
        else {
            const float rf = (float)rating;
            memcpy(q + 16, &rf, 4);
        }
        if (mask) memcpy(q + 24, mask, 8 * (size_t)ncw);
    };
    int64_t out = 0;
    int32_t w = 0;
    auto nop = [&](int32_t owner) {
        put(out++, (uint32_t)(((int64_t)n_spokes + owner) * rec_bytes), 0, 0, OWN_HUB_FWD | OWN_SPK_FWD | OWN_NOP, 0.0, nullptr);
    };
    for (; w < h->n_owners && osch.own_off[(size_t)w + 1] == 0; ++w)
        for (int i = 0; i < pad; ++i) nop(w);
    for (int64_t s = 0; s < n; ++s) {
        const int64_t t = sch.perm[(size_t)s];
        uint64_t mask[6] = {0, 0, 0, 0, 0, 0};
        if (!is_2d_model(h->model))
            for (int32_t c = in.ctx_ptr[in.ctx[t]]; c < in.ctx_ptr[in.ctx[t] + 1]; ++c) mask[in.ctx_conds[c] >> 6] |= (uint64_t)1 << (in.ctx_conds[c] & 63);
        put(out++, (uint32_t)((int64_t)(h->owner_hub_item ? in.u[t] : in.j[t]) * rec_bytes), h->owner_hub_item ? in.j[t] : in.u[t], osch.want[(size_t)s],
            osch.flags[(size_t)s], in.r[t], mask);
        while (w < h->n_owners && s + 1 == osch.own_off[(size_t)w + 1]) {
            for (int i = 0; i < pad; ++i) nop(w);
            ++w;
        }
    }
    for (; w < h->n_owners; ++w)
        for (int i = 0; i < pad; ++i) nop(w);
    hipError_t e = abi_upload(&h->d_own_recs, recs, h->stream);
    if (e == hipSuccess) e = abi_upload(&h->d_own_off, osch.own_off, h->stream);
    if (e == hipSuccess) e = hipMalloc(&h->d_tagged, ((size_t)n_spokes + (size_t)h->n_owners) * (size_t)h->own_stride * 8);
    if (e == hipSuccess) e = hipMalloc((void **)&h->d_flow_err, 16);
    if (e == hipSuccess) e = hipMemsetAsync(h->d_flow_err, 0, 16, h->stream);
    if (e == hipSuccess) e = hipStreamSynchronize(h->stream);
    return e;
}

static hipError_t build_user_items(cmi_instance *h, const RatingsIn &in) {
    const int64_t n = in.n;
    std::vector<int32_t> ptr((size_t)h->n_users + 1, 0), items((size_t)n);
    for (int64_t t = 0; t < n; ++t) ptr[(size_t)in.u[t] + 1]++;
    for (int32_t x = 0; x < h->n_users; ++x) ptr[(size_t)x + 1] += ptr[(size_t)x];
    {
        std::vector<int32_t> cur(ptr.begin(), ptr.end() - 1);
        for (int64_t t = 0; t < n; ++t) items[(size_t)cur[(size_t)in.u[t]]++] = in.j[t];
    }
    for (int32_t x = 0; x < h->n_users; ++x) std::sort(items.begin() + ptr[(size_t)x], items.begin() + ptr[(size_t)x + 1]);
    hipError_t e = abi_upload(&h->d_ui_ptr, ptr, h->stream);
    if (e == hipSuccess) e = abi_upload(&h->d_ui_items, items, h->stream);
    if (e == hipSuccess) e = hipStreamSynchronize(h->stream);
    return e;
}

static hipError_t alloc_launch_buffers(cmi_instance *h) {
    hipError_t e = hipSuccess;
    if (h->n_slots > 0) {
        e = hipMalloc((void **)&h->d_loss_part, (size_t)h->n_slots * sizeof(double));
        if (e == hipSuccess) e = hipMemsetAsync(h->d_loss_part, 0, (size_t)h->n_slots * sizeof(double), h->stream);
    }
    if (e == hipSuccess && h->sched == Sched::CAMFC_BLOCKS) e = abi_upload(&h->d_blk_off, h->blk_off, h->stream);
    if (e == hipSuccess && h->n_tail > 0) e = abi_upload(&h->d_tail_off, h->level_off, h->stream);
    return e;
}

static int build_ratings(cmi_instance *h, const RatingsIn &in) {
    const bool times = getenv("CMI_SETUP_TIMES") != nullptr;
    auto T0 = std::chrono::steady_clock::now();
    auto lap = [&](const char *w) {
        if (!times) return;
        const auto t = std::chrono::steady_clock::now();
        fprintf(stderr, "set_ratings %s %.3f s\n", w, std::chrono::duration<double>(t - T0).count());
        T0 = t;
    };
    const int64_t n = in.n;
    int dmax = 0;
    if (int rc = validate_ratings(h, in, dmax)) return rc;
    lap("validate");
    h->n = n;
    h->n_ctx = is_2d_model(h->model) ? 0 : in.n_ctx;
    h->dmax = dmax;

    bool chain_ok = false;
    if (int rc = check_schedule_flags(h, dmax, chain_ok)) return rc;
    SpecArena spec;
    speculative_arena(h, n, chain_ok, spec);
    lap("arena allocation");
    LevelSchedule sch;
    ChainSchedule csch;
    OwnerSchedule osch;
    ChainDeviceKeep keep;
    h->sched = choose_schedule(h, in, dmax, chain_ok, csch, keep);
    if (h->sched == Sched::LEVELS) h->level_kernel = level_kernel(h->k, dmax, h->f64, LaunchCfg{h->model, h->strict});
    if (h->sched == Sched::OWNER) {
        if (int rc = build_owner_lists(h, in, osch, sch)) return rc;
    } else {
        if (int rc = build_levels(h, in, csch, sch)) return rc;
        level_slots(h, dmax, sch);
    }
    lap("schedule");
    const bool dev_stream = h->sched == Sched::CHAIN && keep.d_perm != nullptr;
    HostStream hs;
    if (!dev_stream) gather_stream(h, in, dmax, sch, hs);
    lap("stream");
    hipError_t e = upload_stream(h, in, dmax, dev_stream, hs, keep, csch);
    lap("uploads");
    if (e == hipSuccess) e = setup_arena(h, n, dev_stream, hs, spec);
    lap("arena");
    if (e == hipSuccess && h->sched == Sched::OWNER) e = pack_owner_records(h, in, osch, sch);
    if (e == hipSuccess && h->model == CMI_MODEL_SVDPP) e = build_user_items(h, in);
    if (e == hipSuccess) e = alloc_launch_buffers(h);
    if (e == hipSuccess) e = hipStreamSynchronize(h->stream);
    if (e != hipSuccess) CMI_FAIL(h, CMI_E_HIP, "set_ratings: upload failed: %s", hipGetErrorString(e));
    lap("rest");
    if (h->sched == Sched::OWNER)
        h->tuple_bytes = (n + (int64_t)h->n_owners * 2 * owner_depth()) * (int64_t)owner_rec_bytes(owner_mask_words(h->model, h->n_conds));
    else
        h->tuple_bytes = n * (8 + (int64_t)esize(h) + 4 * (int64_t)dmax) + (h->sched == Sched::CHAIN ? 4 * (h->n_units + 1) : 0) +
                         (h->arena_on ? 4 * n : 0);
    h->have_ratings = true;
    return CMI_OK;
}

static int set_ratings_impl(cmi_instance *h, const RatingsIn &in) {
    if (int rc = check_ratings_args(h, in)) return rc;
    CMI_HIP(h, hipSetDevice(h->device));
    CMI_HIP(h, hipStreamSynchronize(h->stream));
    free_ratings(h);
    const int rc = build_ratings(h, in);
    if (rc != CMI_OK) free_ratings(h);
    return rc;
}

extern "C" int cmi_set_ratings(cmi_handle h, int64_t n, const int32_t *u, const int32_t *j, const int32_t *ctx,
                               const double *r, int32_t n_ctx, const int32_t *ctx_ptr, const int32_t *ctx_conds) {
    if (!h) return CMI_E_INVALID;
    return abi_barrier(h->err, "set_ratings", [&] { return set_ratings_impl(h, RatingsIn{n, u, j, ctx, r, n_ctx, ctx_ptr, ctx_conds}); },
                       [h] { free_ratings(h); });
}

extern "C" int cmi_schedule_info(cmi_handle h, int64_t info[8]) {
    if (!h || !info) return CMI_E_INVALID;
    if (!h->have_ratings) CMI_FAIL(h, CMI_E_INVALID, "schedule_info: call cmi_set_ratings first");
    info[0] = h->n_tail > 0 ? h->n_launches : h->sched_levels;
    info[1] = h->max_level;
    info[2] = h->n;
    info[3] = h->dmax;
    int64_t sb = 0;
    for (int w = 0; w < CMI_STATE_COUNT; ++w) sb += h->state_count[w] * (int64_t)esize(h);
    info[4] = sb;
    info[5] = h->tuple_bytes;
    info[6] = info[7] = 0;
    switch (h->sched) {
    case Sched::SERIAL:
    case Sched::EXT_SERIAL: info[6] = 1; break;
    case Sched::CAMFC_BLOCKS: info[6] = 1; info[7] = (int64_t)h->blk_off.size() - 1; break;
    case Sched::CHAIN: info[6] = h->chain_hub_item ? 4 : 5; info[7] = h->n_units; break;
    case Sched::OWNER: info[6] = h->owner_hub_item ? 6 : 7; info[7] = (int64_t)h->n_owners | ((int64_t)h->n_team << 32); break;
    default: break;
    }
    return CMI_OK;
}

extern "C" int cmi_schedule_traffic(cmi_handle h, int64_t out[4]) {
    if (!h || !out) return CMI_E_INVALID;
    if (!h->have_ratings) CMI_FAIL(h, CMI_E_INVALID, "schedule_traffic: call cmi_set_ratings first");
    const int64_t e = (int64_t)esize(h), K = h->k, D = h->dmax, NC = h->n_conds, n = h->n;
    const bool bu = cmi_model_has(h->model, CMI_STATE_USER_BIAS), bj = cmi_model_has(h->model, CMI_STATE_ITEM_BIAS);
    const bool uc = cmi_model_has(h->model, CMI_STATE_UC_BIAS), ic = cmi_model_has(h->model, CMI_STATE_IC_BIAS);
    const bool cb = cmi_model_has(h->model, CMI_STATE_COND_BIAS);
    const int64_t SECT = 64;
    const int64_t row = 2 * K * e, stream = 8 + e + 4 * D;
    const int64_t row_sectors = (NC * e + SECT - 1) / SECT;
    const int64_t cells_sect = 2 * SECT * std::min<int64_t>(D, row_sectors), cells_own = 2 * e * D;
    const int64_t ctx_row_sect = 2 * row_sectors * SECT, ctx_row_own = 2 * NC * e;
    const int64_t S = (bu ? 1 : 0) + (bj ? 1 : 0), T = (uc ? 1 : 0) + (ic ? 1 : 0) + (cb ? 1 : 0);
    out[2] = n * (12 + e + 4 * D + 2 * row + 2 * e * S + 2 * e * D * T);
    if (h->sched == Sched::CHAIN) {
        const bool hi = h->chain_hub_item;
        const bool hub_b = hi ? bj : bu, spk_b = hi ? bu : bj, hub_c = hi ? ic : uc, spk_c = hi ? uc : ic;
        const int64_t unit_sect = row + (hub_b ? 2 * SECT : 0) + (hub_c ? ctx_row_sect : 0) + 4;
        const int64_t unit_own = row + (hub_b ? 2 * e : 0) + (hub_c ? ctx_row_own : 0) + 4;
        const int64_t arena_idx = h->arena_on ? 4 : 0;
        const int64_t tup_sect = stream + arena_idx + row + (spk_b ? 2 * SECT : 0) + (spk_c ? cells_sect : 0);
        const int64_t tup_own = stream + arena_idx + row + (spk_b ? 2 * e : 0) + (spk_c ? cells_own : 0);
        out[0] = h->n_units * unit_sect + n * tup_sect;
        out[1] = h->n_units * unit_own + n * tup_own;
        out[3] = 1 | (h->arena_on ? 2 : 0);
    } else {
        out[0] = n * (stream + 2 * row + S * 2 * SECT + T * cells_sect);
        out[1] = n * (stream + 2 * row + S * 2 * e + T * cells_own);
        out[3] = 0;
    }
    return CMI_OK;
}

extern "C" const char *cmi_schedule_note(cmi_handle h) { return h ? h->sched_note.c_str() : ""; }


template <typename T>
static SgdArgs<T> make_args(cmi_instance *h) {
    SgdArgs<T> a;
    a.P = (T *)h->state[CMI_STATE_P];
    a.Q = (T *)h->state[CMI_STATE_Q];
    a.userBias = (T *)h->state[CMI_STATE_USER_BIAS];
    a.itemBias = (T *)h->state[CMI_STATE_ITEM_BIAS];
    a.condBias = (T *)h->state[CMI_STATE_COND_BIAS];
    a.ucBias = (T *)h->state[CMI_STATE_UC_BIAS];
    a.icBias = (T *)h->state[CMI_STATE_IC_BIAS];
    a.su = h->d_su;
    a.sj = h->d_sj;
    a.sr = (const T *)h->d_sr;
    a.sconds = h->d_sconds;
    a.hp = h->d_hp;
    a.loss_part = h->d_loss_part;
    a.k = h->k;
    a.n_conds = h->n_conds;
    a.dmax = h->dmax;
    if (h->arena_on) {
        a.arena = (T *)h->d_arena;
        a.next_pos = h->d_next;
    }
#ifdef CMI_OWNER_TRACE
    a.trace = h->d_trace;
#endif
    return a;
}

#ifdef CMI_OWNER_TRACE
extern "C" int cmi_debug_owner_trace(cmi_handle h) {
    if (!h || h->sched != Sched::OWNER) return CMI_E_INVALID;
    if (hipSetDevice(h->device) != hipSuccess) return CMI_E_HIP;
    if (!h->d_trace) {
        h->trace_doubles = ((size_t)h->n + (size_t)h->n_owners * 2 * (size_t)owner_depth()) * 12 * 64;
        CMI_HIP(h, hipMalloc((void **)&h->d_trace, h->trace_doubles * 8));
    }
    CMI_HIP(h, hipMemsetAsync(h->d_trace, 0, h->trace_doubles * 8, h->stream));
    CMI_HIP(h, hipStreamSynchronize(h->stream));
    return CMI_OK;
}
extern "C" int cmi_debug_owner_trace_dump(cmi_handle h, const char *path) {
    if (!h || !h->d_trace || !path) return CMI_E_INVALID;
    return abi_barrier(h->err, "debug_owner_trace_dump", [&] {
        if (hipSetDevice(h->device) != hipSuccess) return CMI_E_HIP;
        std::vector<double> host(h->trace_doubles);
        CMI_HIP(h, hipMemcpyAsync(host.data(), h->d_trace, h->trace_doubles * 8, hipMemcpyDeviceToHost, h->stream));
        CMI_HIP(h, hipStreamSynchronize(h->stream));
        FILE *f = fopen(path, "wb");
        if (!f) CMI_FAIL(h, CMI_E_INVALID, "cannot open %s", path);
        const size_t wrote = fwrite(host.data(), 8, host.size(), f);
        fclose(f);
        (void)hipFree(h->d_trace);
        h->d_trace = nullptr;
        return wrote == host.size() ? CMI_OK : CMI_E_INVALID;
    });
}
#endif

int cmi_sync_table_from_arena(cmi_instance *h) {
    if (!h->arena_on || h->table_valid) return CMI_OK;
    CMI_HIP(h, hipSetDevice(h->device));
    const int64_t rows = h->arena_which == CMI_STATE_P ? h->n_users : h->n_items;
    CMI_HIP(h, h->f64 ? launch_arena_gather<double>((double *)h->state[h->arena_which], (const double *)h->d_arena, h->d_first, rows, h->k, h->stream)
                      : launch_arena_gather<float>((float *)h->state[h->arena_which], (const float *)h->d_arena, h->d_first, rows, h->k, h->stream));
    h->table_valid = true;
// ... 2 lines not shown
static int sync_arena_from_table(cmi_instance *h) {
    if (!h->arena_on || h->arena_valid) return CMI_OK;
    const int64_t rows = h->arena_which == CMI_STATE_P ? h->n_users : h->n_items;
    CMI_HIP(h, h->f64 ? launch_arena_scatter<double>((const double *)h->state[h->arena_which], (double *)h->d_arena, h->d_first, rows, h->k, h->stream)
                      : launch_arena_scatter<float>((const float *)h->state[h->arena_which], (float *)h->d_arena, h->d_first, rows, h->k, h->stream));
    h->arena_valid = true;
    return CMI_OK;
}

template <typename T>
static ExtArgs<T> make_ext_args(cmi_instance *h) {
    ExtArgs<T> a;
    a.P = (T *)h->state[CMI_STATE_P];
    a.Q = (T *)h->state[CMI_STATE_Q];
    a.userBias = (T *)h->state[CMI_STATE_USER_BIAS];
    a.itemBias = (T *)h->state[CMI_STATE_ITEM_BIAS];
    a.Y = (T *)h->state[CMI_STATE_Y];
    a.cc = (T *)h->state[CMI_STATE_CC_MATRIX];
    a.cf = (T *)h->state[CMI_STATE_CF_MATRIX];
    a.cv = (T *)h->state[CMI_STATE_C_VECTOR];
    a.su = h->d_su;
    a.sj = h->d_sj;
    a.sr = (const T *)h->d_sr;
    a.sconds = h->d_sconds;
    a.empty_conds = h->d_empty;
    a.ui_ptr = h->d_ui_ptr;
    a.ui_items = h->d_ui_items;
    a.hp = h->d_hp;
    a.upbound = 1.0 / std::sqrt((double)h->n_ctx_dims);
    a.lowbound = 1.0 / std::pow(10.0, 100.0);
    a.k = h->k;
    a.n_conds = h->n_conds;
    a.dmax = h->dmax;
    a.num_f = h->num_f;
    a.n_empty = (int32_t)h->empty_conds.size();
    return a;
}

template <typename T>
static hipError_t enqueue_owner_epoch(cmi_instance *h) {
    int cus = 0;
    if (hipDeviceGetAttribute(&cus, hipDeviceAttributeMultiprocessorCount, h->device) != hipSuccess || cus < 1) cus = 1;
    OwnerDeviceLock guard(h->device, h->n_team + (h->n_owners - h->n_team + 3) / 4, cus);
    if (!guard.ok) {
        h->owner_busy = true;
        h->owner_busy_why = guard.why;
        return hipErrorNotReady;
    }
    const int32_t n_spokes = h->owner_hub_item ? h->n_users : h->n_items;
    const uint32_t tag0 = (uint32_t)(++h->owner_epoch_seq) * 0x9E3779B1u;
    const bool strict = sizeof(T) == 8 && h->strict;
    hipError_t e = launch_owner_epoch<T>(make_args<T>(h), h->model, h->owner_hub_item, strict, h->d_own_recs, h->d_own_off, h->n_owners,
                                         h->n_team, h->d_tagged, h->own_stride, n_spokes, h->d_flow_err, tag0, h->stream);
    if (e == hipSuccess) e = launch_reduce_loss(h->d_loss_part, h->n_slots, h->d_scratch, h->d_loss, h->stream);
    int32_t stalled = 0;
    if (e == hipSuccess) e = hipMemcpyAsync(&stalled, h->d_flow_err, 4, hipMemcpyDeviceToHost, h->stream);
    if (e == hipSuccess) e = hipStreamSynchronize(h->stream);
    if (e == hipSuccess && stalled) {
        h->owner_stalled = true;
        e = hipErrorLaunchFailure;
    }
    return e;
}

template <typename T>
static hipError_t enqueue_levels(cmi_instance *h) {
    const LaunchCfg cfg{h->model, h->strict};
    switch (h->sched) {
    case Sched::EXT_SERIAL: return launch_ext_serial<T>(make_ext_args<T>(h), h->model, h->strict, h->n, h->d_loss, h->stream);
    case Sched::SERIAL: return launch_serial<T>(make_args<T>(h), cfg, h->n, h->d_loss, h->stream);
    case Sched::CAMFC_BLOCKS: return launch_camfc_blocks<T>(make_args<T>(h), h->d_blk_off, (int)h->blk_off.size() - 1, h->d_loss, h->stream);
    case Sched::OWNER: return enqueue_owner_epoch<T>(h);
    case Sched::CHAIN:
    case Sched::LEVELS: break;
    default: return hipErrorInvalidValue;
    }
    const SgdArgs<T> a = make_args<T>(h);
    const int64_t n_levels = (int64_t)h->level_off.size() - 1;
    hipError_t e = hipSuccess;
    for (int64_t l = 0; l < n_levels && e == hipSuccess; ++l) {
        const int64_t b = h->level_off[(size_t)l], slot = h->slot_off[(size_t)l];
        const int cnt = (int)(h->level_off[(size_t)l + 1] - b);
        const int32_t run = h->tail_len[(size_t)l];
        if (h->sched == Sched::CHAIN) e = launch_chain_level<T>(a, cfg, h->chain_hub_item, h->d_unit_off, b, cnt, slot, h->stream);
        else if (run > 0) {
            e = launch_narrow_run<T>(a, cfg, h->level_kernel, h->d_tail_off + l, run, slot, h->stream);
            l += run - 1;
        } else e = launch_level<T>(a, cfg, h->level_kernel, b, cnt, slot, h->stream);
    }
    if (e == hipSuccess) e = launch_reduce_loss(h->d_loss_part, h->n_slots, h->d_scratch, h->d_loss, h->stream);
    return e;
}
static hipError_t enqueue_levels(cmi_instance *h) { return h->f64 ? enqueue_levels<double>(h) : enqueue_levels<float>(h); }

static int arena_probe(cmi_instance *h);

static int enqueue_epoch(cmi_instance *h, double lrate, bool probing = false) {
    if (!h->have_ratings) CMI_FAIL(h, CMI_E_INVALID, "train: call cmi_set_ratings first");
    CMI_HIP(h, hipSetDevice(h->device));
    if (h->arena_probe && !probing)
        if (int rc = arena_probe(h)) return rc;
    h->hp.lr = lrate;
    CMI_HIP(h, launch_set_hparams(h->d_hp, h->hp, h->stream));
    if (h->n == 0) {
        CMI_HIP(h, hipMemsetAsync(h->d_loss, 0, sizeof(double), h->stream));
        h->epoch_timed = false;
        return CMI_OK;
    }
    const bool graph = h->use_graph && (h->sched == Sched::LEVELS || h->sched == Sched::CHAIN) && (h->n_tail > 0 ? h->n_launches : (int64_t)h->level_off.size() - 1) <= 65536;
    if (graph && !h->graph_exec) {
        hipGraph_t g = nullptr;
        CMI_HIP(h, hipStreamBeginCapture(h->stream, hipStreamCaptureModeThreadLocal));
        hipError_t e = enqueue_levels(h);
        hipError_t e2 = hipStreamEndCapture(h->stream, &g);
        if (e != hipSuccess || e2 != hipSuccess) {
            if (g) hipGraphDestroy(g);
            CMI_FAIL(h, CMI_E_HIP, "graph capture failed: %s", hipGetErrorString(e != hipSuccess ? e : e2));
        }
        e = hipGraphInstantiate(&h->graph_exec, g, nullptr, nullptr, 0);
        hipGraphDestroy(g);
        if (e != hipSuccess) {
            h->graph_exec = nullptr;
            CMI_FAIL(h, CMI_E_HIP, "hipGraphInstantiate failed: %s", hipGetErrorString(e));
        }
    }
    if (h->arena_on) {
        if (int rc = sync_arena_from_table(h)) return rc;
        h->table_valid = false;
    }
    CMI_HIP(h, hipEventRecord(h->ev0, h->stream));
    if (graph) CMI_HIP(h, hipGraphLaunch(h->graph_exec, h->stream));
    else {
        const hipError_t e = enqueue_levels(h);
        if (h->owner_busy) {
            h->owner_busy = false;
            CMI_FAIL(h, CMI_E_BUSY, "owner epoch not started on device %d: %s (persistent kernels of two processes must not share a device); "
                     "the model is untouched -- retry, or use CMI_FLAG_NO_OWNER", h->device, h->owner_busy_why);
        }
        if (h->owner_stalled)
            CMI_FAIL(h, CMI_E_HIP, "owner epoch stalled: a tuple waited past its bound for a predecessor's record (is another persistent kernel "
                     "holding compute units of device %d?) -- the model state is invalid; reload it and use CMI_FLAG_NO_OWNER", h->device);
        CMI_HIP(h, e);
    }
    CMI_HIP(h, hipEventRecord(h->ev1, h->stream));
    h->epoch_timed = true;
    return CMI_OK;
}

static int arena_probe(cmi_instance *h) {
    h->arena_probe = false;
    float ms[2] = {0.f, 0.f};
    for (int form = 0; form < 2; ++form) {
        h->arena_on = form == 1;
        if (h->graph_exec) {
            hipGraphExecDestroy(h->graph_exec);
            h->graph_exec = nullptr;
        }
        for (int rep = 0; rep < 2; ++rep)
            if (int rc = enqueue_epoch(h, 0.0, true)) return rc;
        CMI_HIP(h, hipStreamSynchronize(h->stream));
        CMI_HIP(h, hipEventElapsedTime(&ms[form], h->ev0, h->ev1));
        if (form == 1)
            if (int rc = cmi_sync_table_from_arena(h)) return rc;
    }
    const bool keep = ms[1] < 0.97f * ms[0] && !h->arena_probe_table;
    char note[200];
    snprintf(note, sizeof note, "spoke arena probe: table %.2f ms, arena %.2f ms per epoch -> %s", ms[0], ms[1], keep ? "arena" : "table");
// ... 429 lines not shown
    return abi_barrier(h->err, "eval_resident", [&] {
        double sums[5];
        if (int rc = cmi_eval_resident_sums(h, min_rate, max_rate, sums)) return rc;
        const double cnt = sums[4];
        const double mae = sums[0] / cnt;
        out[0] = mae;
        out[1] = std::sqrt(sums[1] / cnt);
        out[2] = mae / (max_rate - min_rate);
        out[3] = sums[2] / cnt;
        out[4] = std::sqrt(sums[3] / cnt);
        if (count) *count = (int64_t)cnt;
        return CMI_OK;
    });
}

extern "C" int cmi_level_schedule(int64_t n, const int32_t *u, const int32_t *j, int32_t n_users, int32_t n_items,
                                  int order, int32_t *perm, int64_t *level_off, int64_t level_cap,
                                  int64_t *n_levels) {
    return abi_barrier(cmi_thread_err(), "cmi_level_schedule", [&] {
        if (n < 0 || (n > 0 && (!u || !j)) || n_users <= 0 || n_items <= 0 || !n_levels || order < 0 || order > 3)
            return CMI_E_INVALID;
        for (int64_t t = 0; t < n; ++t)
            if (u[t] < 0 || u[t] >= n_users || j[t] < 0 || j[t] >= n_items) return CMI_E_INVALID;
        LevelSchedule sch;
        if (!build_level_schedule(n, u, j, n_users, n_items, order, sch)) return CMI_E_UNSUPPORTED;
        *n_levels = sch.n_levels();
        if (level_off) {
            if (level_cap < sch.n_levels() + 1) return CMI_E_INVALID;
            for (size_t i = 0; i < sch.level_off.size(); ++i) level_off[i] = sch.level_off[i];
        }
        if (perm)
            for (int64_t s = 0; s < n; ++s) perm[s] = sch.perm[(size_t)s];
        return CMI_OK;
    });
}

extern "C" int cmi_chain_schedule(int64_t n, const int32_t *u, const int32_t *j, int32_t n_users, int32_t n_items, int hub,
                                  int max_chain, int32_t *perm, int32_t *unit_off, int64_t unit_cap, int64_t *level_off,
                                  int64_t level_cap, int64_t *n_units, int64_t *n_levels, int *hub_used) {
    return abi_barrier(cmi_thread_err(), "cmi_chain_schedule", [&] {
        if (n < 0 || (n > 0 && (!u || !j)) || n_users <= 0 || n_items <= 0 || !n_units || !n_levels || max_chain < 1) return CMI_E_INVALID;
        for (int64_t t = 0; t < n; ++t)
            if (u[t] < 0 || u[t] >= n_users || j[t] < 0 || j[t] >= n_items) return CMI_E_INVALID;
        ChainSchedule cs;
        if (!build_chain_schedule(n, u, j, n_users, n_items, hub, max_chain, cs)) return CMI_E_UNSUPPORTED;
        *n_units = cs.n_units();
        *n_levels = cs.n_levels();
        if (hub_used) *hub_used = cs.hub_is_item;
        if (!perm) return CMI_OK;
        if (!unit_off || !level_off || unit_cap < cs.n_units() + 1 || level_cap < cs.n_levels() + 1) return CMI_E_INVALID;
        std::copy(cs.perm.begin(), cs.perm.end(), perm);
        std::copy(cs.unit_off.begin(), cs.unit_off.end(), unit_off);
        std::copy(cs.level_off.begin(), cs.level_off.end(), level_off);
        return CMI_OK;
    });
}

extern "C" int cmi_chain_schedule_device(int device, int64_t n, const int32_t *u, const int32_t *j, int32_t n_users, int32_t n_items, int hub,
                                         int max_chain, int32_t *perm, int32_t *unit_off, int64_t unit_cap, int64_t *level_off,
                                         int64_t level_cap, int64_t *n_units, int64_t *n_levels, int *hub_used) {
    return abi_barrier(cmi_thread_err(), "cmi_chain_schedule_device", [&] {
        if (n < 0 || (n > 0 && (!u || !j)) || n_users <= 0 || n_items <= 0 || !n_units || !n_levels || max_chain < 1) return CMI_E_INVALID;
        if (device < 0 || device >= cmi_device_count()) return CMI_E_NO_DEVICE;
        for (int64_t t = 0; t < n; ++t)
            if (u[t] < 0 || u[t] >= n_users || j[t] < 0 || j[t] >= n_items) return CMI_E_INVALID;
        ChainSchedule cs;
        hipStream_t st = nullptr;
        if (hipSetDevice(device) != hipSuccess || hipStreamCreateWithFlags(&st, hipStreamNonBlocking) != hipSuccess) return CMI_E_HIP;
        const bool ok = build_chain_schedule_device(device, st, n, u, j, n_users, n_items, hub, max_chain, cs);
        (void)hipStreamDestroy(st);
        if (!ok) return CMI_E_UNSUPPORTED;
        *n_units = cs.n_units();
        *n_levels = cs.n_levels();
        if (hub_used) *hub_used = cs.hub_is_item;
        if (!perm) return CMI_OK;
        if (!unit_off || !level_off || unit_cap < cs.n_units() + 1 || level_cap < cs.n_levels() + 1) return CMI_E_INVALID;
        std::copy(cs.perm.begin(), cs.perm.end(), perm);
        std::copy(cs.unit_off.begin(), cs.unit_off.end(), unit_off);
        std::copy(cs.level_off.begin(), cs.level_off.end(), level_off);
        return CMI_OK;
    });
}

extern "C" int cmi_owner_schedule(int64_t n, const int32_t *u, const int32_t *j, int32_t n_users, int32_t n_items, int hub, int n_owners,
                                  int depth, int32_t *perm, int64_t *own_off, uint32_t *want, uint32_t *flags, int *hub_used) {
    return abi_barrier(cmi_thread_err(), "cmi_owner_schedule", [&] {
        if (n < 0 || (n > 0 && (!u || !j)) || n_users <= 0 || n_items <= 0 || n_owners < 1 || depth < 1 || !perm || !own_off || !want || !flags)
            return CMI_E_INVALID;
        for (int64_t t = 0; t < n; ++t)
            if (u[t] < 0 || u[t] >= n_users || j[t] < 0 || j[t] >= n_items) return CMI_E_INVALID;
        OwnerSchedule os;
        if (!build_owner_schedule(n, u, j, n_users, n_items, hub, n_owners, depth, os)) return CMI_E_UNSUPPORTED;
        if (hub_used) *hub_used = os.hub_is_item;
        std::copy(os.perm.begin(), os.perm.end(), perm);
        std::copy(os.own_off.begin(), os.own_off.end(), own_off);
        std::copy(os.want.begin(), os.want.end(), want);
        std::copy(os.flags.begin(), os.flags.end(), flags);
        return CMI_OK;
    });
}

extern "C" int cmi_narrow_runs(int64_t n_levels, const int64_t *level_off, int64_t max_tuples, int64_t min_levels,
                               int32_t *run_len, int64_t *n_launches) {
    return abi_barrier(cmi_thread_err(), "cmi_narrow_runs", [&] {
        if (n_levels < 0 || !level_off || !n_launches || (n_levels > 0 && !run_len)) return CMI_E_INVALID;
        std::vector<int64_t> off(level_off, level_off + n_levels + 1);
        std::vector<int32_t> rl;
        *n_launches = build_narrow_runs(off, max_tuples, min_levels, rl);
        for (int64_t l = 0; l < n_levels; ++l) run_len[l] = rl[(size_t)l];
        return CMI_OK;
    });
}

extern "C" int cmi_conflict_free_blocks(int64_t n, const int32_t *u, const int32_t *j, int32_t n_users, int32_t n_items,
                                        int32_t max_block, int32_t *off, int64_t off_cap, int64_t *n_blocks) {
    return abi_barrier(cmi_thread_err(), "cmi_conflict_free_blocks", [&] {
        if (n < 0 || (n > 0 && (!u || !j)) || n_users <= 0 || n_items <= 0 || max_block <= 0 || !n_blocks || n >= ((int64_t)1 << 31))
            return CMI_E_INVALID;
        for (int64_t t = 0; t < n; ++t)
            if (u[t] < 0 || u[t] >= n_users || j[t] < 0 || j[t] >= n_items) return CMI_E_INVALID;
        std::vector<int32_t> o;
        build_conflict_free_blocks(n, u, j, n_users, n_items, max_block, o);
        *n_blocks = (int64_t)o.size() - 1;
        if (!off) return CMI_OK;
        if (off_cap < (int64_t)o.size()) return CMI_E_INVALID;
        std::copy(o.begin(), o.end(), off);
        return CMI_OK;
    });
}
```

carskit_amd/csrc/cmi_instance.hpp:

```cpp
#pragma once
#include "rank_host.hpp"
#include "../../include/carskit_mi355x.h"

#include <hip/hip_runtime.h>

#include <cstdio>
#include <functional>
#include <string>
#include <vector>

#include "mf_sgd_kernels.hpp"

enum class Sched {
    NONE,
    LEVELS,
    SERIAL,
    CAMFC_BLOCKS,
    EXT_SERIAL,
    CHAIN,
    OWNER,
};

struct cmi_instance {
    int model = 0, k = 0, n_users = 0, n_items = 0, n_conds = 0, device = 0;
    unsigned flags = 0;
    bool f64 = false, strict = false, use_graph = true;
    Sched sched = Sched::NONE;
    cmi::LevelKernel level_kernel = cmi::LevelKernel::GENERIC;
    bool chain_hub_item = true;
    int32_t *d_unit_off = nullptr;
    int64_t n_units = 0;
    bool arena_on = false, arena_valid = false, table_valid = true;
    bool arena_probe_table = false;
    bool arena_probe = false;
    int arena_which = 0;
    void *d_arena = nullptr;
    int32_t *d_next = nullptr, *d_first = nullptr;
    bool owner_hub_item = true;
    uint32_t owner_epoch_seq = 0;
    bool owner_busy = false;
    const char *owner_busy_why = "";
    int device_share = 1;
    int n_owners = 0, n_team = 0;
    bool owner_stalled = false;
    void *d_own_recs = nullptr;
    int64_t *d_own_off = nullptr;
    void *d_tagged = nullptr;
    int64_t own_stride = 0;
#ifdef CMI_OWNER_TRACE
    double *d_trace = nullptr;
    size_t trace_doubles = 0;
#endif
    std::string err;
    std::string sched_note;
    hipStream_t stream = nullptr;
    void *state[CMI_STATE_COUNT] = {};
    int64_t state_count[CMI_STATE_COUNT] = {};
    int64_t n = 0;
    int dmax = 0;
    int32_t n_ctx = 0;
    int32_t *d_su = nullptr, *d_sj = nullptr, *d_sconds = nullptr, *d_ctx_ptr = nullptr, *d_ctx_conds = nullptr;
    void *d_sr = nullptr;
    int32_t *d_flow_err = nullptr;
    int64_t ctx_nnz = 0;
    std::vector<int64_t> level_off, slot_off;
    int64_t n_launches = 0, n_tail = 0;
    std::vector<int32_t> tail_len;
    int64_t *d_tail_off = nullptr;
    std::vector<int32_t> blk_off;
    int32_t *d_blk_off = nullptr;
    int64_t n_slots = 0, max_level = 0, tuple_bytes = 0, sched_levels = 0;
    double *d_loss_part = nullptr, *d_scratch = nullptr, *d_loss = nullptr;
    cmi::HParams *d_hp = nullptr;
    cmi::HParams hp{0, 0, 0, 0, 0, 0};
    double *h_loss = nullptr;
    hipGraphExec_t graph_exec = nullptr;
    hipEvent_t ev0 = nullptr, ev1 = nullptr;
    bool have_ratings = false, epoch_timed = false;
    double last_loss = 0.0;
    int32_t *d_eu = nullptr, *d_ej = nullptr, *d_ectx = nullptr;
    double *d_er = nullptr, *d_epart = nullptr;
    int64_t n_eval = 0;
    void *d_xbucket = nullptr, *d_xsnap = nullptr;
    int64_t x_count = 0;
    std::vector<int> x_which;
    std::vector<int64_t> x_off;
    int num_f = 0, n_ctx_dims = 1;
    bool sim_params_set = false;
    std::vector<int32_t> empty_conds;
    int32_t *d_empty = nullptr, *d_ui_ptr = nullptr, *d_ui_items = nullptr;
    void *comm = nullptr;
    int comm_rank = 0, comm_world = 0;
    hipEvent_t evx0 = nullptr, evx1 = nullptr;
    bool exchange_timed = false;
    cmi::RankWorkspace rank_ws;
    float last_rank_ms = 0.f;
    double last_rank_flops = 0.0;
};

bool cmi_model_has(int model, int which);
template <typename T>
cmi::ExtEvalArgs<T> cmi_ext_eval_args(cmi_instance *h, const int32_t *du, const int32_t *dj, const int32_t *dctx, const double *dr,
                                      double *dpreds, double *dpart, int bound, double lo, double hi, double min_rate);

int cmi_train_loop(const std::function<int(double, double *)> &epoch, std::string &err, int first_iter, double prev_loss, int num_iters,
                   double init_lrate, double max_lrate, int bold_driver, double decay, int early_stop, double *losses, double *lrates,
                   int *iters_run, double *final_lrate);
int cmi_eval_sums(cmi_instance *h, int64_t n, const int32_t *u, const int32_t *j, const int32_t *ctx, const double *r, double min_rate,
                  double max_rate, double sums[5]);

int cmi_eval_resident_sums(cmi_instance *h, double min_rate, double max_rate, double sums[5]);
void cmi_comm_release(cmi_instance *h);

// ... 2 lines not shown
```

carskit_amd/csrc/level_schedule.cpp:

```cpp
#include "level_schedule.hpp"

#include <system_error>
#include <cstdlib>
#include <thread>

#include "host_pool.hpp"

#include <queue>
#include <functional>
#include <utility>
#include <algorithm>
#include <numeric>

namespace cmi {

bool build_level_schedule(int64_t n, const int32_t *u, const int32_t *j, int32_t n_users, int32_t n_items,
                          int within_level_order, LevelSchedule &out) {
    out.perm.clear();
    out.level_off.clear();
    out.max_level = 0;
    if (n <= 0) {
        out.level_off.push_back(0);
        return true;
    }
// ... 152 lines not shown
    const int32_t n_hubs = hub ? n_items : n_users, n_spokes = hub ? n_users : n_items;
    const std::vector<int64_t> &deg = hub ? deg_j : deg_u;

    std::vector<int32_t> order;
    order.reserve((size_t)n_hubs);
    for (int32_t x = 0; x < n_hubs; ++x)
        if (deg[(size_t)x] > 0) order.push_back(x);
    std::sort(order.begin(), order.end(), [&](int32_t a, int32_t b) { return deg[(size_t)a] != deg[(size_t)b] ? deg[(size_t)a] > deg[(size_t)b] : a < b; });
    typedef std::pair<int64_t, int32_t> Load;
    std::priority_queue<Load, std::vector<Load>, std::greater<Load>> heap;
    for (int32_t w = 0; w < n_owners; ++w) heap.push(Load(0, w));
    std::vector<int32_t> owner((size_t)n_hubs, -1);
    std::vector<int64_t> load((size_t)n_owners, 0);
    for (int32_t x : order) {
        Load l = heap.top();
        heap.pop();
        owner[(size_t)x] = l.second;
        l.first += deg[(size_t)x];
        load[(size_t)l.second] = l.first;
        heap.push(l);
    }
    out.own_off.assign((size_t)n_owners + 1, 0);
    out.max_load = 0;
    for (int32_t w = 0; w < n_owners; ++w) {
        out.own_off[(size_t)w + 1] = out.own_off[(size_t)w] + load[(size_t)w];
        out.max_load = std::max(out.max_load, load[(size_t)w]);
    }
    out.perm.assign((size_t)n, 0);
    out.want.assign((size_t)n, 0);
    out.flags.assign((size_t)n, 0);
    {
        std::vector<int64_t> cur(out.own_off.begin(), out.own_off.end() - 1);
        std::vector<uint32_t> seen((size_t)n_spokes, 0);
        for (int64_t t = 0; t < n; ++t) {
            const int64_t pos = cur[(size_t)owner[(size_t)hv[t]]]++;
            out.perm[(size_t)pos] = (int32_t)t;
            out.want[(size_t)pos] = seen[(size_t)sv[t]]++;
        }
    }
    std::vector<int64_t> last_pos((size_t)n_hubs, -1);
    for (int32_t w = 0; w < n_owners; ++w) {
        const int64_t b = out.own_off[(size_t)w], e = out.own_off[(size_t)w + 1];
        for (int64_t pos = b; pos < e; ++pos) {
            const int64_t t = out.perm[(size_t)pos];
            uint32_t f = 0;
            const int64_t lp = last_pos[(size_t)hv[t]];
            if (lp >= 0) {
                if (pos - lp == 1) f |= OWN_HUB_FWD;
                else if (pos - lp <= depth) f |= OWN_HUB_LATE;
            }
            last_pos[(size_t)hv[t]] = pos;
            if (pos > b) {
                const int64_t tp = out.perm[(size_t)pos - 1];
                if (sv[tp] == sv[t] && out.want[(size_t)pos] == out.want[(size_t)pos - 1] + 1) f |= OWN_SPK_FWD;
            }
            out.flags[(size_t)pos] = f;
        }
        for (int64_t pos = b; pos < e; ++pos) {
            const uint32_t nf = pos + 1 < e ? out.flags[(size_t)pos + 1] : 0u;
            if (!(nf & OWN_HUB_FWD)) out.flags[(size_t)pos] |= OWN_HUB_STORE;
            if (!(nf & OWN_SPK_FWD)) out.flags[(size_t)pos] |= OWN_SPK_STORE;
        }
    }
    return true;
}


int64_t count_plain_levels(int64_t n, const int32_t *u, const int32_t *j, int32_t n_users, int32_t n_items) {
    if (n <= 0) return 0;
    int32_t nl = 0;
    int64_t nu = 0;
    chain_pass(n, j, u, n_items, n_users, 1, nullptr, nullptr, nullptr, nullptr, nl, nu);
    return nl;
}

bool build_chain_schedule(int64_t n, const int32_t *u, const int32_t *j, int32_t n_users, int32_t n_items, int hub, int max_chain,
                          ChainSchedule &out) {
    out = ChainSchedule();
    out.unit_off.push_back(0);
    out.level_off.push_back(0);
    if (max_chain < 1) max_chain = 1;
    if (max_chain > 255) max_chain = 255;
    out.hub_is_item = hub == 0 ? 0 : 1;
    if (n <= 0) return true;
    if (n >= (int64_t)1 << 31) return false;
    struct Side {
        std::vector<int32_t> unit_of, unit_level;
        std::vector<uint8_t> pos, unit_len;
        int32_t nl = 0;
        int64_t nu = 0;
    };
    auto run_side = [&](int item_hub, Side &sd) {
        sd.unit_of.resize((size_t)n);
        sd.pos.resize((size_t)n);
        if (item_hub) chain_pass(n, j, u, n_items, n_users, max_chain, &sd.unit_of, &sd.pos, &sd.unit_level, &sd.unit_len, sd.nl, sd.nu);
        else chain_pass(n, u, j, n_users, n_items, max_chain, &sd.unit_of, &sd.pos, &sd.unit_level, &sd.unit_len, sd.nl, sd.nu);
    };
    Side side;
    auto pick = [&](int64_t units_item, int64_t units_user) {
        if (hub == -2) return (double)units_user <= 1.3 * (double)units_item ? 0 : 1;
        if (hub == -3) return (double)units_item <= 1.3 * (double)units_user ? 1 : 0;
        return units_item <= units_user ? 1 : 0;
    };
    if (hub < 0 && n > ((int64_t)32 << 20)) {
        const int64_t m = n / 8;
        int32_t l1 = 0, l0 = 0;
        int64_t ui = 0, uu = 0;
        bool threaded = true;
        std::thread th;
        try {
            th = std::thread([&]() { chain_pass(m, u, j, n_users, n_items, max_chain, nullptr, nullptr, nullptr, nullptr, l0, uu); });
        } catch (const std::system_error &) {
            threaded = false;
        }
        chain_pass(m, j, u, n_items, n_users, max_chain, nullptr, nullptr, nullptr, nullptr, l1, ui);
        if (threaded) th.join();
        else chain_pass(m, u, j, n_users, n_items, max_chain, nullptr, nullptr, nullptr, nullptr, l0, uu);
        hub = pick(ui, uu);
    }
    if (hub < 0) {
        Side other;
        bool threaded = true;
        std::thread th;
        try {
            th = std::thread([&]() { run_side(0, other); });
        } catch (const std::system_error &) {
            threaded = false;
        }
        run_side(1, side);
        if (threaded) th.join();
        else run_side(0, other);
        hub = pick(side.nu, other.nu);
        if (!hub) std::swap(side, other);
    } else run_side(hub ? 1 : 0, side);
    out.hub_is_item = hub ? 1 : 0;
    const int32_t nl = side.nl;
    const int64_t nu = side.nu;
    const std::vector<int32_t> &unit_of = side.unit_of, &unit_level = side.unit_level;
    const std::vector<uint8_t> &unit_len = side.unit_len, &pos = side.pos;
    const size_t nkeys = (size_t)nl * (size_t)max_chain;
    std::vector<int64_t> key_off(nkeys + 1, 0);
    auto key = [&](int64_t q) { return (size_t)(unit_level[(size_t)q] - 1) * (size_t)max_chain + (size_t)(max_chain - unit_len[(size_t)q]); };
    for (int64_t q = 0; q < nu; ++q) key_off[key(q) + 1]++;
    for (size_t x = 0; x < nkeys; ++x) key_off[x + 1] += key_off[x];
    out.level_off.assign((size_t)nl + 1, 0);
    for (int32_t l = 0; l <= nl; ++l) out.level_off[(size_t)l] = key_off[(size_t)l * (size_t)max_chain];
    for (int32_t l = 0; l < nl; ++l) out.max_level_units = std::max(out.max_level_units, out.level_off[(size_t)l + 1] - out.level_off[(size_t)l]);
    std::vector<int32_t> rank((size_t)nu);
    {
        std::vector<int64_t> cur(key_off.begin(), key_off.end() - 1);
        for (int64_t q = 0; q < nu; ++q) rank[(size_t)q] = (int32_t)cur[key(q)]++;
    }
    out.unit_off.assign((size_t)nu + 1, 0);
    for (int64_t q = 0; q < nu; ++q) out.unit_off[(size_t)rank[(size_t)q] + 1] = unit_len[(size_t)q];
    for (int64_t q = 0; q < nu; ++q) out.unit_off[(size_t)q + 1] += out.unit_off[(size_t)q];
    out.perm.resize((size_t)n);
    parallel_ranges(n, host_threads(n), [&](int, int64_t b, int64_t e) {
        for (int64_t t = b; t < e; ++t)
            out.perm[(size_t)out.unit_off[(size_t)rank[(size_t)unit_of[(size_t)t]]] + pos[(size_t)t]] = (int32_t)t;
    });
    return true;
}

}
```

carskit_amd/csrc/level_schedule.hpp:

```cpp
#pragma once
#include <stdint.h>
#include <vector>

namespace cmi {

enum { LEVEL_ORDER_CRS = 0, LEVEL_ORDER_ITEM = 1, LEVEL_ORDER_USER = 2, LEVEL_ORDER_XCD = 3 };
static const int LEVEL_XCD_BLOCK = 32;

struct LevelSchedule {
    std::vector<int32_t> perm;
    std::vector<int64_t> level_off;
    int64_t max_level = 0;
    int64_t n_levels() const { return (int64_t)level_off.size() - 1; }
};

bool build_level_schedule(int64_t n, const int32_t *u, const int32_t *j, int32_t n_users, int32_t n_items,
                          int within_level_order, LevelSchedule &out);


struct ChainSchedule {
    std::vector<int32_t> perm;
    std::vector<int32_t> unit_off;
    std::vector<int64_t> level_off;
    int hub_is_item = 1;
    int64_t max_level_units = 0;
    int64_t n_units() const { return (int64_t)unit_off.size() - 1; }
    int64_t n_levels() const { return (int64_t)level_off.size() - 1; }
};
bool build_chain_schedule(int64_t n, const int32_t *u, const int32_t *j, int32_t n_users, int32_t n_items, int hub, int max_chain,
                          ChainSchedule &out);

enum { OWN_HUB_FWD = 1, OWN_HUB_LATE = 2, OWN_HUB_STORE = 4, OWN_SPK_FWD = 8, OWN_SPK_STORE = 16,
       OWN_NOP = 32  };
struct OwnerSchedule {
    std::vector<int32_t> perm;
    std::vector<int64_t> own_off;
    std::vector<uint32_t> want;
    std::vector<uint32_t> flags;
    int hub_is_item = 1;
    int64_t max_load = 0;
    int64_t n_owners() const { return (int64_t)own_off.size() - 1; }
};
bool build_owner_schedule(int64_t n, const int32_t *u, const int32_t *j, int32_t n_users, int32_t n_items, int hub, int n_owners,
                          int depth, OwnerSchedule &out);

int64_t count_plain_levels(int64_t n, const int32_t *u, const int32_t *j, int32_t n_users, int32_t n_items);

int64_t build_narrow_runs(const std::vector<int64_t> &level_off, int64_t max_tuples, int64_t min_levels, std::vector<int32_t> &run_len);

void build_conflict_free_blocks(int64_t n, const int32_t *u, const int32_t *j, int32_t n_users, int32_t n_items, int max_block,
                                std::vector<int32_t> &off);

}
```

carskit_amd/csrc/mf_sgd_kernels.hpp:

```cpp
#pragma once

#include <hip/hip_runtime.h>
#include <stdint.h>

namespace cmi {

enum Model { BIASEDMF = 0, CAMF_C = 1, CAMF_CI = 2, CAMF_CU = 3, CAMF_CUCI = 4, PMF = 5,
             SVDPP = 6, CAMF_ICS = 7, CAMF_LCS = 8, CAMF_MCS = 9 };

struct ModelParams {
    bool has_bu, has_bj, has_bc, has_ic, has_uc;
    bool has_ctx;
};
constexpr ModelParams model_params(int model) {
    return {model == BIASEDMF || model == CAMF_C || model == CAMF_CI, model == BIASEDMF || model == CAMF_C || model == CAMF_CU,
            model == CAMF_C, model == CAMF_CI || model == CAMF_CUCI, model == CAMF_CU || model == CAMF_CUCI,
            !(model == BIASEDMF || model == PMF)};
}

struct HParams {
    double lr, regU, regI, regB, regC, gm;
};

template <typename T>
struct SgdArgs {
    T *P, *Q;
    T *userBias, *itemBias;
    T *condBias;
    T *ucBias, *icBias;
    const int32_t *su, *sj;
    const T *sr;
    const int32_t *sconds;
    const HParams *hp;
    double *loss_part;
    int32_t k, n_conds, dmax;
    T *arena = nullptr;
    const int32_t *next_pos = nullptr;
    uint32_t owner_tag0 = 0;
#ifdef CMI_OWNER_TRACE
    double *trace = nullptr;
#endif
};

template <typename T>
hipError_t launch_arena_scatter(const T *table, T *arena, const int32_t *first_pos, int64_t n_rows, int k, hipStream_t s);
template <typename T>
hipError_t launch_arena_gather(T *table, const T *arena, const int32_t *first_pos, int64_t n_rows, int k, hipStream_t s);

bool camfc_pipe_supported(int k, int n_conds, int dmax);
template <typename T>
hipError_t launch_camfc_pipe(const SgdArgs<T> &a, int64_t n, double *loss_out, hipStream_t s);

struct LaunchCfg {
    int model;
    bool strict;
};

enum class LevelKernel { GENERIC, FAST, SMALL };
LevelKernel level_kernel(int k, int dmax, bool f64, const LaunchCfg &cfg);
int small_lpt(int k, int dmax);
int level_blocks(LevelKernel kn, int k, int dmax, int count);
template <typename T>
hipError_t launch_level(const SgdArgs<T> &a, const LaunchCfg &cfg, LevelKernel kn, int64_t begin, int count, int64_t slot0,
                        hipStream_t s);
template <typename T>
hipError_t launch_narrow_run(const SgdArgs<T> &a, const LaunchCfg &cfg, LevelKernel kn, const int64_t *tail_off, int n_tail,
                             int64_t slot, hipStream_t s);
size_t camfc_blocks_lds(int n_conds, int dmax, size_t esize);
template <typename T>
hipError_t launch_camfc_blocks(const SgdArgs<T> &a, const int32_t *blk_off, int n_blocks, double *loss_out, hipStream_t s);

bool has_chain_path(int model, int k, int dmax, int n_conds, bool f64, bool strict);
size_t chain_lds_bytes(int model, int n_conds, int dmax, bool f64, bool hub_is_item);
int chain_groups_per_block(int k, int dmax, bool f64);
int chain_level_blocks(int k, int dmax, bool f64, int count);
template <typename T>
hipError_t launch_chain_level(const SgdArgs<T> &a, const LaunchCfg &cfg, bool hub_is_item, const int32_t *unit_off, int64_t ubegin,
                              int count, int64_t slot0, hipStream_t s);

template <typename T>
hipError_t launch_serial(const SgdArgs<T> &a, const LaunchCfg &cfg, int64_t n, double *loss_out, hipStream_t s);

hipError_t launch_set_hparams(HParams *dst, HParams v, hipStream_t s);
hipError_t launch_reduce_loss(const double *loss_part, int64_t n_slots, double *scratch, double *loss_out,
                              hipStream_t s);

template <typename T>
struct EvalArgs {
    const T *P, *Q, *userBias, *itemBias, *condBias, *ucBias, *icBias;
    const int32_t *u, *j, *ctx;
    const double *r;
    const int32_t *ctx_ptr, *ctx_conds;
    double *preds;
    double *part;
    double gm, lo, hi, min_rate;
    int32_t k, n_conds, bound, model;
};
int eval_blocks(int64_t n);
template <typename T>
hipError_t launch_eval(const EvalArgs<T> &a, int64_t n, hipStream_t s);

hipError_t launch_delta_pack(const void *state, const void *snap, void *bucket, int64_t n, bool f64, hipStream_t s);
hipError_t launch_delta_apply(void *state, void *snap, const void *bucket, double scale, int64_t n, bool f64, hipStream_t s);

template <typename T>
struct ExtArgs {
    T *P, *Q, *userBias, *itemBias;
    T *Y;
    T *cc;
    T *cf;
    T *cv;
    const int32_t *su, *sj;
    const T *sr;
    const int32_t *sconds;
    const int32_t *empty_conds;
    const int32_t *ui_ptr, *ui_items;
    const HParams *hp;
    double upbound, lowbound;
    int32_t k, n_conds, dmax, num_f, n_empty;
};
template <typename T>
hipError_t launch_ext_serial(const ExtArgs<T> &a, int model, bool strict, int64_t n, double *loss_out, hipStream_t s);
bool svdpp_team_supported(int k);
template <typename T>
hipError_t launch_svdpp_team(const ExtArgs<T> &a, int64_t n, double *loss_out, hipStream_t s);

template <typename T>
struct ExtEvalArgs {
    const T *P, *Q, *userBias, *itemBias, *Y, *cc, *cf, *cv;
    const int32_t *u, *j, *ctx;
    const double *r;
    const int32_t *ctx_ptr, *ctx_conds, *empty_conds, *ui_ptr, *ui_items;
    double *preds, *part;
    double gm, lo, hi, min_rate;
    int32_t k, n_conds, num_f, n_empty, bound, model;
};
template <typename T>
hipError_t launch_ext_eval(const ExtEvalArgs<T> &a, int64_t n, hipStream_t s);
template <typename T>
hipError_t launch_ext_rank_items(const ExtEvalArgs<T> &a, const int32_t *cand, int nc, T *B, int kp, hipStream_t s);
template <typename T>
hipError_t launch_ext_rank_queries(const ExtEvalArgs<T> &a, const int32_t *qu, const int32_t *qc, int nq, T *A, T *row_const, int kp,
                                   hipStream_t s);

hipError_t launch_convert(const void *src, int src_f64, void *dst, int dst_f64, int64_t n, hipStream_t s);


template <int NCW>
struct OwnerRecT {
    uint32_t off;
    int32_t hub;
    uint32_t want;
    uint32_t flags;
    union {
        double d;
        float f;
    } rating;
    uint64_t mask[NCW];
};
inline size_t owner_rec_bytes(int ncw) { return 24 + 8 * (size_t)ncw; }
// ... 11 lines not shown
```

carskit_amd/csrc/sched_device.hip:

```cpp
#include <hip/hip_runtime.h>

#include <cstring>

#include <rocprim/device/device_radix_sort.hpp>
#include <rocprim/device/device_scan.hpp>
#include <rocprim/functional.hpp>

#include <algorithm>
#include <chrono>
#include <cstdint>
#include <cstdio>
#include <cstdlib>
#include <vector>

#include "level_schedule.hpp"
#include "sched_device.hpp"

namespace cmi {

namespace {

struct DevPool {
    std::vector<void *> ptrs;
    hipError_t err = hipSuccess;
// ... 159 lines not shown
                if ((int32_t)(v >> 32) != want) break;
                const int32_t t = a.lt[pos], B = (int32_t)(v & 0xFFFFFFFFu);
                int32_t l, p;
                if (lev > B && len < a.max_chain) {
                    l = lev;
                    p = len++;
                    if (a.unit_len) a.unit_len[unit] = (uint8_t)len;
                } else {
                    l = (lev > B ? lev : B) + 1;
                    p = 0;
                    len = 1;
                    unit = t;
                    ++units;
                    if (a.unit_level) {
                        a.unit_level[t] = l;
                        a.unit_len[t] = 1;
                    }
                }
                lev = l;
                top = l > top ? l : top;
                __hip_atomic_store(&a.spoke[sp], ((unsigned long long)(uint32_t)(want + 1) << 32) | (uint32_t)l, __ATOMIC_RELAXED, __HIP_MEMORY_SCOPE_AGENT);
                if (a.unit_of) {
                    a.unit_of[t] = unit;
                    a.pos[t] = (uint8_t)p;
                }
                ++pos;
                moved = true;
            }
            if (moved) {
                a.sv[4 * h] = pos;
                a.sv[4 * h + 1] = lev;
                a.sv[4 * h + 2] = unit;
                a.sv[4 * h + 3] = len;
                progressed = true;
            }
            left = left || pos < end;
        }
        if (__builtin_amdgcn_ballot_w64(left) == 0) break;
        if (__builtin_amdgcn_ballot_w64(progressed) == 0) {
            if (++idle > a.idle_limit) break;
            __builtin_amdgcn_s_sleep(8);
        } else idle = 0;
    }
    for (int64_t h = g; h < a.n_hub; h += T) remaining += (unsigned long long)(a.hub_off[h + 1] - a.sv[4 * h]);
#pragma unroll
    for (int m = 32; m >= 1; m >>= 1) {
        units += __shfl_xor(units, m, 64);
        remaining += __shfl_xor(remaining, m, 64);
        const int32_t o = __shfl_xor(top, m, 64);
        top = o > top ? o : top;
    }
    if ((threadIdx.x & 63) == 0) {
        if (units) atomicAdd(&a.counters[0], units);
        if (top) atomicMax(&a.counters[1], (unsigned long long)top);
        if (remaining) atomicAdd(&a.counters[2], remaining);
    }
}

__global__ void k_flags(const int32_t *unit_level, int64_t n, int32_t *flag) {
    for (int64_t i = (int64_t)blockIdx.x * blockDim.x + threadIdx.x; i < n; i += (int64_t)gridDim.x * blockDim.x) flag[i] = unit_level[i] != 0;
}
__global__ void k_units(const int32_t *unit_level, const uint8_t *unit_len, const int32_t *dense, int64_t n, int32_t max_chain, uint32_t *key,
                        int32_t *uid, uint8_t *ulen) {
    for (int64_t t = (int64_t)blockIdx.x * blockDim.x + threadIdx.x; t < n; t += (int64_t)gridDim.x * blockDim.x)
        if (unit_level[t] != 0) {
            const int32_t q = dense[t];
            key[q] = (uint32_t)(unit_level[t] - 1) * (uint32_t)max_chain + (uint32_t)(max_chain - unit_len[t]);
            uid[q] = q;
            ulen[q] = unit_len[t];
        }
}
__global__ void k_rank_units(const int32_t *sorted_uid, const uint8_t *ulen, int64_t nu, int32_t *rank_of, int32_t *len_sorted) {
    for (int64_t r = (int64_t)blockIdx.x * blockDim.x + threadIdx.x; r < nu; r += (int64_t)gridDim.x * blockDim.x) {
        const int32_t q = sorted_uid[r];
        rank_of[q] = (int32_t)r;
        len_sorted[r] = ulen[q];
    }
}
__global__ void k_perm(const int32_t *unit_of, const uint8_t *pos, const int32_t *dense, const int32_t *rank_of, const int32_t *unit_off, int64_t n,
                       int32_t *perm) {
    for (int64_t t = (int64_t)blockIdx.x * blockDim.x + threadIdx.x; t < n; t += (int64_t)gridDim.x * blockDim.x)
        perm[unit_off[rank_of[dense[unit_of[t]]]] + pos[t]] = (int32_t)t;
}
__global__ void k_level_off(const uint32_t *skey, int64_t nu, int32_t nl, int32_t max_chain, int64_t *level_off) {
    const int l = blockIdx.x * blockDim.x + threadIdx.x;
    if (l > nl) return;
    const uint64_t want = (uint64_t)l * (uint64_t)max_chain;
    int64_t lo = 0, hi = nu;
    while (lo < hi) {
        const int64_t mid = (lo + hi) / 2;
        if ((uint64_t)skey[mid] < want) lo = mid + 1;
        else hi = mid;
    }
    level_off[l] = lo;
}

__global__ void k_arena(const int32_t *skey, const int32_t *spos, int64_t n, int32_t *next, int32_t *first) {
    for (int64_t i = (int64_t)blockIdx.x * blockDim.x + threadIdx.x; i < n; i += (int64_t)gridDim.x * blockDim.x) {
        const int32_t r = skey[i];
        const bool head = i == 0 || skey[i - 1] != r, tail = i + 1 == n || skey[i + 1] != r;
        if (head) first[r] = spos[i];
        if (!tail) next[spos[i]] = spos[i + 1];
    }
}
__global__ void k_arena_wrap(const int32_t *skey, const int32_t *spos, int64_t n, int32_t *next, const int32_t *first) {
    for (int64_t i = (int64_t)blockIdx.x * blockDim.x + threadIdx.x; i < n; i += (int64_t)gridDim.x * blockDim.x)
        if (i + 1 == n || skey[i + 1] != skey[i]) next[spos[i]] = first[skey[i]];
}
__global__ void k_fill(int32_t *v, int64_t n, int32_t x) {
    for (int64_t i = (int64_t)blockIdx.x * blockDim.x + threadIdx.x; i < n; i += (int64_t)gridDim.x * blockDim.x) v[i] = x;
}

inline unsigned grid_for(int64_t n) { return (unsigned)std::max<int64_t>(1, std::min<int64_t>((n + 255) / 256, 8192)); }
inline unsigned bits_for(int64_t values) {
    unsigned b = 1;
    while (b < 32 && ((int64_t)1 << b) < values) ++b;
    return b;
}

#define SD(expr)                      \
    do {                              \
        const hipError_t e_ = (expr); \
        if (e_ != hipSuccess) return e_; \
    } while (0)

hipError_t sort_by(DevPool &pool, hipStream_t s, const int32_t *key, int64_t m, int32_t n_keys, int32_t *&skey, int32_t *&st, int32_t *&off) {
    int32_t *iota = pool.get<int32_t>((size_t)m), *cnt = pool.get<int32_t>((size_t)n_keys + 1);
    skey = pool.get<int32_t>((size_t)m);
    st = pool.get<int32_t>((size_t)m);
    off = pool.get<int32_t>((size_t)n_keys + 1);
    SD(pool.err);
    hipLaunchKernelGGL(k_iota, dim3(grid_for(m)), dim3(256), 0, s, iota, m);
    size_t tb = 0;
    SD(rocprim::radix_sort_pairs(nullptr, tb, key, skey, iota, st, (size_t)m, 0u, bits_for(n_keys), s));
    void *tmp = pool.get<char>(tb);
    SD(pool.err);
    SD(rocprim::radix_sort_pairs(tmp, tb, key, skey, iota, st, (size_t)m, 0u, bits_for(n_keys), s));
    SD(hipMemsetAsync(cnt, 0, ((size_t)n_keys + 1) * 4, s));
    hipLaunchKernelGGL(k_hist, dim3(grid_for(m)), dim3(256), 0, s, key, m, cnt);
    size_t tb2 = 0;
    SD(rocprim::exclusive_scan(nullptr, tb2, cnt, off, 0, (size_t)n_keys + 1, rocprim::plus<int32_t>(), s));
    void *tmp2 = pool.get<char>(tb2);
    SD(pool.err);
    SD(rocprim::exclusive_scan(tmp2, tb2, cnt, off, 0, (size_t)n_keys + 1, rocprim::plus<int32_t>(), s));
    return hipGetLastError();
}

struct Sorted {
    int32_t *skey = nullptr, *st = nullptr, *off = nullptr, *rank = nullptr;
};

template <int HMAX>
hipError_t launch_walk(const WalkArgs &a, unsigned blocks, hipStream_t s) {
    hipLaunchKernelGGL(k_walk<HMAX>, dim3(blocks), dim3(256), 0, s, a);
    return hipGetLastError();
}
template <int HMAX>
int resident_blocks(int device) {
    int per_cu = 0, cus = 0;
    if (hipOccupancyMaxActiveBlocksPerMultiprocessor(&per_cu, k_walk<HMAX>, 256, 0) != hipSuccess) return 0;
    if (hipDeviceGetAttribute(&cus, hipDeviceAttributeMultiprocessorCount, device) != hipSuccess) return 0;
    return per_cu * cus;
}

struct WalkOut {
    int32_t *unit_of = nullptr, *unit_level = nullptr;
// ... 2 lines not shown
hipError_t walk(DevPool &pool, int device, hipStream_t s, const Sorted &hubs, const Sorted &spokes, const int32_t *spoke_of, int64_t m, int32_t n_hub,
                int32_t n_spoke, int max_chain, const WalkOut *out, int64_t &n_units, int32_t &n_levels, bool &ok) {
    ok = false;
    int32_t *sp_h = pool.get<int32_t>((size_t)m), *want_h = pool.get<int32_t>((size_t)m), *sv = pool.get<int32_t>((size_t)n_hub * 4);
    unsigned long long *spoke = pool.get<unsigned long long>((size_t)n_spoke), *counters = pool.get<unsigned long long>(3);
    SD(pool.err);
    hipLaunchKernelGGL(k_lists, dim3(grid_for(m)), dim3(256), 0, s, hubs.st, spoke_of, spokes.rank, m, sp_h, want_h);
    hipLaunchKernelGGL(k_init_state, dim3(grid_for(n_hub)), dim3(256), 0, s, hubs.off, n_hub, sv);
    SD(hipMemsetAsync(spoke, 0, (size_t)n_spoke * 8, s));
    SD(hipMemsetAsync(counters, 0, 24, s));
    if (out) {
        SD(hipMemsetAsync(out->unit_level, 0, (size_t)m * 4, s));
    }
    WalkArgs a{hubs.st, sp_h, want_h, hubs.off, n_hub, max_chain, spoke, sv, out ? out->unit_of : nullptr, out ? out->pos : nullptr,
               out ? out->unit_level : nullptr, out ? out->unit_len : nullptr, counters, 4000};
    int hmax = 1;
    unsigned blocks = 0;
    for (; hmax <= 16; hmax *= 2) {
        const int rb = hmax == 1 ? resident_blocks<1>(device) : hmax == 2 ? resident_blocks<2>(device) : hmax == 4 ? resident_blocks<4>(device)
                       : hmax == 8 ? resident_blocks<8>(device) : resident_blocks<16>(device);
        if (rb <= 0) return hipErrorUnknown;
        const int rb_used = std::max(1, rb / 2);
        if ((int64_t)rb_used * 256 * hmax >= n_hub) {
            blocks = (unsigned)std::min<int64_t>(rb_used, ((int64_t)n_hub + (int64_t)256 * hmax - 1) / ((int64_t)256 * hmax));
            break;
        }
    }
    if (getenv("CMI_SCHED_WALK_MEM")) blocks = 0;
    if (!blocks) {
        hmax = 0;
        int per_cu = 0, cus = 0;
        if (hipOccupancyMaxActiveBlocksPerMultiprocessor(&per_cu, k_walk_mem, 256, 0) != hipSuccess) return hipErrorUnknown;
        if (hipDeviceGetAttribute(&cus, hipDeviceAttributeMultiprocessorCount, device) != hipSuccess) return hipErrorUnknown;
        blocks = (unsigned)std::max(1, per_cu * cus / 2);
    }
    for (int launch = 0; launch < 4096; ++launch) {
        SD(hipMemsetAsync(counters + 2, 0, 8, s));
        switch (hmax) {
        case 0:
            hipLaunchKernelGGL(k_walk_mem, dim3(blocks), dim3(256), 0, s, a);
            SD(hipGetLastError());
            break;
        case 1: SD(launch_walk<1>(a, blocks, s)); break;
        case 2: SD(launch_walk<2>(a, blocks, s)); break;
        case 4: SD(launch_walk<4>(a, blocks, s)); break;
        case 8: SD(launch_walk<8>(a, blocks, s)); break;
        default: SD(launch_walk<16>(a, blocks, s)); break;
        }
        unsigned long long c[3];
        SD(hipMemcpyAsync(c, counters, 24, hipMemcpyDeviceToHost, s));
        SD(hipStreamSynchronize(s));
        if (c[2] == 0) {
            n_units = (int64_t)c[0];
            n_levels = (int32_t)c[1];
            ok = true;
            if (getenv("CMI_SETUP_TIMES"))
                fprintf(stderr, "[cmi] device schedule: walk over %lld tuples, %d hub rows (%s, %u blocks): %d launch(es), %lld units, %d levels\n", (long long)m,
                        n_hub, hmax ? "registers" : "memory", blocks, launch + 1, (long long)n_units, n_levels);
            return hipSuccess;
        }
    }
    return hipSuccess;
}

}

void ChainDeviceKeep::release() {
    for (int32_t **q : {&d_u, &d_j, &d_perm})
        if (*q) {
            (void)hipFree(*q);
            *q = nullptr;
        }
}

bool build_chain_schedule_device(int device, void *stream, int64_t n, const int32_t *u, const int32_t *j, int32_t n_users, int32_t n_items, int hub,
                                 int max_chain, ChainSchedule &out, ChainDeviceKeep *keep) {
    hipStream_t s = (hipStream_t)stream;
    out = ChainSchedule();
    out.unit_off.push_back(0);
    out.level_off.push_back(0);
    if (max_chain < 1) max_chain = 1;
    if (max_chain > 255) max_chain = 255;
    out.hub_is_item = hub == 0 ? 0 : 1;
    if (n <= 0) return true;
    if (n >= ((int64_t)1 << 31) - 1024) return false;
    if (hipSetDevice(device) != hipSuccess) return false;
    DevPool pool;
    int32_t *du = pool.get<int32_t>((size_t)n), *dj = pool.get<int32_t>((size_t)n);
    if (pool.err != hipSuccess) return false;
    if (hipMemcpyAsync(du, u, (size_t)n * 4, hipMemcpyHostToDevice, s) != hipSuccess) return false;
    if (hipMemcpyAsync(dj, j, (size_t)n * 4, hipMemcpyHostToDevice, s) != hipSuccess) return false;
    const bool times = getenv("CMI_SETUP_TIMES") != nullptr;
    auto T0 = std::chrono::steady_clock::now();
    auto lap = [&](const char *w) {
        if (!times) return;
        (void)hipStreamSynchronize(s);
        const auto t = std::chrono::steady_clock::now();
        fprintf(stderr, "[cmi] device schedule: %s %.3f s\n", w, std::chrono::duration<double>(t - T0).count());
        T0 = t;
    };
    auto fail = [&](const char *what, hipError_t e) {
        if (getenv("CMI_SETUP_TIMES")) fprintf(stderr, "[cmi] device schedule: %s: %s -- the host builder takes over\n", what, hipGetErrorString(e));
        (void)hipGetLastError();
        return false;
    };
    auto sorted_sides = [&](int64_t m, Sorted &by_u, Sorted &by_j) -> hipError_t {
        SD(sort_by(pool, s, du, m, n_users, by_u.skey, by_u.st, by_u.off));
        SD(sort_by(pool, s, dj, m, n_items, by_j.skey, by_j.st, by_j.off));
        by_u.rank = pool.get<int32_t>((size_t)m);
        by_j.rank = pool.get<int32_t>((size_t)m);
        SD(pool.err);
        hipLaunchKernelGGL(k_rank, dim3(grid_for(m)), dim3(256), 0, s, by_u.skey, by_u.st, by_u.off, m, by_u.rank);
        hipLaunchKernelGGL(k_rank, dim3(grid_for(m)), dim3(256), 0, s, by_j.skey, by_j.st, by_j.off, m, by_j.rank);
        return hipGetLastError();
    };
    auto pick = [&](int64_t units_item, int64_t units_user) {
        if (hub == -2) return (double)units_user <= 1.3 * (double)units_item ? 0 : 1;
        if (hub == -3) return (double)units_item <= 1.3 * (double)units_user ? 1 : 0;
        return units_item <= units_user ? 1 : 0;
    };
    auto count_side = [&](int item_hub, int64_t m, const Sorted &by_u, const Sorted &by_j, int64_t &nu, bool &ok) -> hipError_t {
        int32_t nl = 0;
        return item_hub ? walk(pool, device, s, by_j, by_u, du, m, n_items, n_users, max_chain, nullptr, nu, nl, ok)
                        : walk(pool, device, s, by_u, by_j, dj, m, n_users, n_items, max_chain, nullptr, nu, nl, ok);
    };
    Sorted by_u, by_j;
    bool have_full = false;
    if (hub < 0 && n > ((int64_t)32 << 20)) {
        const int64_t m = n / 8;
        Sorted pu, pj;
        if (hipError_t e = sorted_sides(m, pu, pj)) return fail("prefix sorts", e);
        int64_t ui = 0, uu = 0;
        bool ok1 = false, ok0 = false;
        if (hipError_t e = count_side(1, m, pu, pj, ui, ok1)) return fail("prefix walk (items)", e);
        if (hipError_t e = count_side(0, m, pu, pj, uu, ok0)) return fail("prefix walk (users)", e);
        if (!ok1 || !ok0) return fail("prefix walk", hipSuccess);
        hub = pick(ui, uu);
        lap("side chosen on the first eighth");
    }
    if (hipError_t e = sorted_sides(n, by_u, by_j)) return fail("sorts", e);
    lap("upload + sorts");
    have_full = true;
    (void)have_full;
    if (hub < 0) {
        int64_t ui = 0, uu = 0;
        bool ok1 = false, ok0 = false;
        if (hipError_t e = count_side(1, n, by_u, by_j, ui, ok1)) return fail("count walk (items)", e);
        if (hipError_t e = count_side(0, n, by_u, by_j, uu, ok0)) return fail("count walk (users)", e);
        if (!ok1 || !ok0) return fail("count walk", hipSuccess);
        hub = pick(ui, uu);
    }
    out.hub_is_item = hub ? 1 : 0;
    WalkOut wo;
    wo.unit_of = pool.get<int32_t>((size_t)n);
    wo.unit_level = pool.get<int32_t>((size_t)n);
    wo.pos = pool.get<uint8_t>((size_t)n);
    wo.unit_len = pool.get<uint8_t>((size_t)n);
    if (pool.err != hipSuccess) return fail("allocation", pool.err);
    int64_t nu = 0;
    int32_t nl = 0;
    bool ok = false;
    {
        const hipError_t e = hub ? walk(pool, device, s, by_j, by_u, du, n, n_items, n_users, max_chain, &wo, nu, nl, ok)
                                 : walk(pool, device, s, by_u, by_j, dj, n, n_users, n_items, max_chain, &wo, nu, nl, ok);
        if (e != hipSuccess || !ok) return fail("walk", e);
    }
    lap("walk");
    int32_t *flag = pool.get<int32_t>((size_t)n), *dense = pool.get<int32_t>((size_t)n);
    uint32_t *key = pool.get<uint32_t>((size_t)nu), *skey = pool.get<uint32_t>((size_t)nu);
    int32_t *uid = pool.get<int32_t>((size_t)nu), *suid = pool.get<int32_t>((size_t)nu), *rank_of = pool.get<int32_t>((size_t)nu);
    int32_t *len_sorted = pool.get<int32_t>((size_t)nu + 1), *unit_off = pool.get<int32_t>((size_t)nu + 1), *perm = pool.get<int32_t>((size_t)n);
    uint8_t *ulen = pool.get<uint8_t>((size_t)nu);
    int64_t *level_off = pool.get<int64_t>((size_t)nl + 1);
    if (pool.err != hipSuccess) return fail("allocation", pool.err);
    hipLaunchKernelGGL(k_flags, dim3(grid_for(n)), dim3(256), 0, s, wo.unit_level, n, flag);
    {
        size_t tb = 0;
        if (hipError_t e = rocprim::exclusive_scan(nullptr, tb, flag, dense, 0, (size_t)n, rocprim::plus<int32_t>(), s)) return fail("scan", e);
        void *tmp = pool.get<char>(tb);
        if (pool.err != hipSuccess) return fail("allocation", pool.err);
        if (hipError_t e = rocprim::exclusive_scan(tmp, tb, flag, dense, 0, (size_t)n, rocprim::plus<int32_t>(), s)) return fail("scan", e);
    }
    hipLaunchKernelGGL(k_units, dim3(grid_for(n)), dim3(256), 0, s, wo.unit_level, wo.unit_len, dense, n, max_chain, key, uid, ulen);
    {
        const unsigned bits = bits_for((int64_t)nl * max_chain + 1);
        size_t tb = 0;
        if (hipError_t e = rocprim::radix_sort_pairs(nullptr, tb, key, skey, uid, suid, (size_t)nu, 0u, bits, s)) return fail("unit sort", e);
        void *tmp = pool.get<char>(tb);
        if (pool.err != hipSuccess) return fail("allocation", pool.err);
        if (hipError_t e = rocprim::radix_sort_pairs(tmp, tb, key, skey, uid, suid, (size_t)nu, 0u, bits, s)) return fail("unit sort", e);
    }
    hipLaunchKernelGGL(k_rank_units, dim3(grid_for(nu)), dim3(256), 0, s, suid, ulen, nu, rank_of, len_sorted);
    if (hipMemsetAsync(len_sorted + nu, 0, 4, s) != hipSuccess) return fail("memset", hipGetLastError());
    {
        size_t tb = 0;
        if (hipError_t e = rocprim::exclusive_scan(nullptr, tb, len_sorted, unit_off, 0, (size_t)nu + 1, rocprim::plus<int32_t>(), s)) return fail("scan", e);
        void *tmp = pool.get<char>(tb);
        if (pool.err != hipSuccess) return fail("allocation", pool.err);
        if (hipError_t e = rocprim::exclusive_scan(tmp, tb, len_sorted, unit_off, 0, (size_t)nu + 1, rocprim::plus<int32_t>(), s)) return fail("scan", e);
    }
    hipLaunchKernelGGL(k_perm, dim3(grid_for(n)), dim3(256), 0, s, wo.unit_of, wo.pos, dense, rank_of, unit_off, n, perm);
    hipLaunchKernelGGL(k_level_off, dim3((unsigned)((nl + 1 + 255) / 256)), dim3(256), 0, s, skey, nu, nl, max_chain, level_off);
    if (hipError_t e = hipGetLastError()) return fail("kernels", e);
    out.unit_off.assign((size_t)nu + 1, 0);
    out.level_off.assign((size_t)nl + 1, 0);
    if (keep) {
        for (int32_t *q : {du, dj, perm}) pool.ptrs.erase(std::find(pool.ptrs.begin(), pool.ptrs.end(), (void *)q));
        keep->d_u = du;
        keep->d_j = dj;
        keep->d_perm = perm;
    } else {
        out.perm.resize((size_t)n);
        if (hipMemcpyAsync(out.perm.data(), perm, (size_t)n * 4, hipMemcpyDeviceToHost, s) != hipSuccess) return fail("copy back", hipGetLastError());
    }
    if (hipMemcpyAsync(out.unit_off.data(), unit_off, ((size_t)nu + 1) * 4, hipMemcpyDeviceToHost, s) != hipSuccess) return fail("copy back", hipGetLastError());
    if (hipMemcpyAsync(out.level_off.data(), level_off, ((size_t)nl + 1) * 8, hipMemcpyDeviceToHost, s) != hipSuccess) return fail("copy back", hipGetLastError());
    if (hipError_t e = hipStreamSynchronize(s)) return fail("synchronize", e);
    lap("unit sort + offsets + copy back");
    out.max_level_units = 0;
    for (int32_t l = 0; l < nl; ++l) out.max_level_units = std::max(out.max_level_units, out.level_off[(size_t)l + 1] - out.level_off[(size_t)l]);
    return true;
}

namespace {
template <typename R>
__global__ void k_stream(int64_t n, const int32_t *u, const int32_t *j, const int32_t *perm, const int32_t *ctx, const double *r, const int32_t *ctx_ptr,
                         const int32_t *ctx_conds, int dmax, int32_t *su, int32_t *sj, int32_t *sconds, R *sr) {
    for (int64_t s = (int64_t)blockIdx.x * blockDim.x + threadIdx.x; s < n; s += (int64_t)gridDim.x * blockDim.x) {
        const int32_t t = perm[s];
        su[s] = u[t];
        sj[s] = j[t];
        sr[s] = (R)r[t];
        if (dmax > 0) {
            const int32_t c = ctx[t], b = ctx_ptr[c], e = ctx_ptr[c + 1];
            int32_t *row = sconds + s * dmax;
            for (int d = 0; d < dmax; ++d) row[d] = b + d < e ? ctx_conds[b + d] : -1;
        }
    }
}
}

int stream_build_device(void *stream, int64_t n, const int32_t *d_u, const int32_t *d_j, const int32_t *d_perm, const int32_t *ctx, const double *r,
                        const int32_t *d_ctx_ptr, const int32_t *d_ctx_conds, int dmax, bool f64, int32_t *d_su, int32_t *d_sj, int32_t *d_sconds,
                        void *d_sr) {
    hipStream_t s = (hipStream_t)stream;
    if (n <= 0) return (int)hipSuccess;
    DevPool pool;
    int32_t *d_ctx = dmax > 0 ? pool.get<int32_t>((size_t)n) : nullptr;
    double *d_r = pool.get<double>((size_t)n);
    if (pool.err != hipSuccess) return (int)pool.err;
    if (dmax > 0)
        if (hipError_t e = hipMemcpyAsync(d_ctx, ctx, (size_t)n * 4, hipMemcpyHostToDevice, s)) return (int)e;
    if (hipError_t e = hipMemcpyAsync(d_r, r, (size_t)n * 8, hipMemcpyHostToDevice, s)) return (int)e;
    if (f64) hipLaunchKernelGGL(k_stream<double>, dim3(grid_for(n)), dim3(256), 0, s, n, d_u, d_j, d_perm, d_ctx, d_r, d_ctx_ptr, d_ctx_conds, dmax, d_su, d_sj, d_sconds, (double *)d_sr);
    else hipLaunchKernelGGL(k_stream<float>, dim3(grid_for(n)), dim3(256), 0, s, n, d_u, d_j, d_perm, d_ctx, d_r, d_ctx_ptr, d_ctx_conds, dmax, d_su, d_sj, d_sconds, (float *)d_sr);
    if (hipError_t e = hipGetLastError()) return (int)e;
    return (int)hipStreamSynchronize(s);
}

int arena_positions_device(void *stream, int64_t n, const int32_t *d_spoke_stream, int64_t n_spokes, int32_t *d_next, int32_t *d_first) {
    hipStream_t s = (hipStream_t)stream;
    if (n <= 0) return (int)hipSuccess;
    DevPool pool;
    int32_t *skey = nullptr, *spos = nullptr, *off = nullptr;
    if (hipError_t e = sort_by(pool, s, d_spoke_stream, n, (int32_t)n_spokes, skey, spos, off)) {
        if (getenv("CMI_SETUP_TIMES")) fprintf(stderr, "[cmi] device arena lists: %s -- the host walk takes over\n", hipGetErrorString(e));
        return (int)e;
    }
    hipLaunchKernelGGL(k_fill, dim3(grid_for(n_spokes)), dim3(256), 0, s, d_first, n_spokes, -1);
    hipLaunchKernelGGL(k_arena, dim3(grid_for(n)), dim3(256), 0, s, skey, spos, n, d_next, d_first);
    hipLaunchKernelGGL(k_arena_wrap, dim3(grid_for(n)), dim3(256), 0, s, skey, spos, n, d_next, d_first);
    if (hipError_t e = hipGetLastError()) return (int)e;
    return (int)hipStreamSynchronize(s);
}

}
```

carskit_amd/csrc/sched_device.hpp:

```cpp
#pragma once
#include <stdint.h>

#include "level_schedule.hpp"

namespace cmi {

struct ChainDeviceKeep {
    int32_t *d_u = nullptr, *d_j = nullptr, *d_perm = nullptr;
    ChainDeviceKeep() = default;
    ChainDeviceKeep(const ChainDeviceKeep &) = delete;
    ChainDeviceKeep &operator=(const ChainDeviceKeep &) = delete;
    void release();
    ~ChainDeviceKeep() { release(); }
};
bool build_chain_schedule_device(int device, void *stream, int64_t n, const int32_t *u, const int32_t *j, int32_t n_users, int32_t n_items, int hub,
                                 int max_chain, ChainSchedule &out, ChainDeviceKeep *keep = nullptr);

int stream_build_device(void *stream, int64_t n, const int32_t *d_u, const int32_t *d_j, const int32_t *d_perm, const int32_t *ctx, const double *r,
                        const int32_t *d_ctx_ptr, const int32_t *d_ctx_conds, int dmax, bool f64, int32_t *d_su, int32_t *d_sj, int32_t *d_sconds,
                        void *d_sr);

int arena_positions_device(void *stream, int64_t n, const int32_t *d_spoke_stream, int64_t n_spokes, int32_t *d_next, int32_t *d_first);

}
```

include/carskit_mi355x.h:

```cpp
#ifndef CARSKIT_MI355X_H
#define CARSKIT_MI355X_H

#include <stdint.h>

#ifdef __cplusplus
extern "C" {
#endif

#define CMI_ABI_VERSION 5

#define CMI_OK 0
#define CMI_E_INVALID (-1)
#define CMI_E_NO_DEVICE (-2)
#define CMI_E_HIP (-3)
#define CMI_E_NUMERIC (-4)
#define CMI_E_UNSUPPORTED (-5)
#define CMI_E_HOST (-6)
#define CMI_E_BUSY (-7)

#define CMI_MODEL_BIASEDMF 0
#define CMI_MODEL_CAMF_C 1
#define CMI_MODEL_CAMF_CI 2
#define CMI_MODEL_CAMF_CU 3
#define CMI_MODEL_CAMF_CUCI 4
// ... 130 lines not shown
                           double min_rate, double max_rate, double *out, int64_t *count);
int cmi_group_predict_batch(cmi_group_handle g, int64_t n, const int32_t *u, const int32_t *j, const int32_t *ctx, int bound, double lo,
                            double hi, double *out);
int cmi_group_shard_info(cmi_group_handle g, int shard, int64_t info[6]);
int cmi_group_last_times(cmi_group_handle g, float *compute_ms, float *exchange_ms);
const char *cmi_group_exchange_path(cmi_group_handle g);
int cmi_group_member(cmi_group_handle g, int shard, cmi_handle *out);
int cmi_group_set_eval_ratings(cmi_group_handle g, int64_t n, const int32_t *u, const int32_t *j, const int32_t *ctx, const double *r);
int cmi_group_eval_resident(cmi_group_handle g, double min_rate, double max_rate, double out[5], int64_t *count);

#define CMI_COMM_ID_BYTES 128
int cmi_comm_unique_id(void *id );
int cmi_comm_init(cmi_handle h, const void *id, int rank, int world);
int cmi_comm_exchange(cmi_handle h, double scale);
int cmi_comm_train_epoch(cmi_handle h, double lrate, double scale, double *global_loss);
int cmi_comm_last_exchange_ms(cmi_handle h, float *ms);

typedef struct cmi_fm_instance *cmi_fm_handle;

#define CMI_FM_FLAG_DETERMINISTIC 0x1u
#define CMI_FM_FLAG_RELAXED_SUMS 0x2u
int cmi_fm_create(int k, int n_users, int n_items, int n_conds, int n_ctx_dims, int device, unsigned flags,
                  cmi_fm_handle *out);
int cmi_fm_destroy(cmi_fm_handle h);
const char *cmi_fm_last_error(cmi_fm_handle h);
int cmi_fm_set_hparams(cmi_fm_handle h, double regLw, double regLf, int64_t global_size);
int cmi_fm_set_ratings(cmi_fm_handle h, int64_t n, const int32_t *u, const int32_t *j, const int32_t *ctx,
                       const double *r);
int cmi_fm_set_model(cmi_fm_handle h, double w0, const double *w, const double *V);
int cmi_fm_get_model(cmi_fm_handle h, double *w0, double *w, double *V);
int cmi_fm_init(cmi_fm_handle h);
int cmi_fm_sweep(cmi_fm_handle h);
int cmi_fm_train(cmi_fm_handle h, int num_iters);
int cmi_fm_predict_batch(cmi_fm_handle h, int64_t n, const int32_t *u, const int32_t *j, const int32_t *ctx,
                         int bound, double lo, double hi, double *out);
int cmi_fm_synchronize(cmi_fm_handle h);
int cmi_fm_stream(cmi_fm_handle h, void **stream);
int cmi_fm_eval_rankings(cmi_fm_handle h, int64_t n_train, const int32_t *tu, const int32_t *tj, const int32_t *tctx,
                         const double *tr, int64_t n_test, const int32_t *su, const int32_t *sj, const int32_t *sctx,
                         const double *sr, double bin_thold, int num_recs, int num_ignore, int strategy, double out[21],
                         int64_t *n_queries, int32_t *q_user, int32_t *q_ctx, int32_t *q_count, int32_t *top_items,
                         double *top_scores);
int cmi_fm_num_phases(cmi_fm_handle h);
int cmi_fm_phase_reduce(cmi_fm_handle h, int phase);
int cmi_fm_phase_buffer(cmi_fm_handle h, int phase, void **dev_ptr, int64_t *count);
int cmi_fm_phase_apply(cmi_fm_handle h, int phase);
int cmi_fm_phase_run(cmi_fm_handle h, int phase);
int cmi_fm_comm_init(cmi_fm_handle h, const void *id, int rank, int world);
int cmi_fm_comm_sweep(cmi_fm_handle h);
int cmi_fm_layout(cmi_fm_handle h, int64_t out[12]);
int cmi_fm_time_reduce(cmi_fm_handle h, int phase, int reps, double *avg_ms);

typedef struct cmi_dao *cmi_dao_handle;

int cmi_dao_read(const char *path, cmi_dao_handle *out);
int cmi_dao_read_shared(const char *path, cmi_dao_handle train, cmi_dao_handle *out);
int cmi_dao_destroy(cmi_dao_handle h);
const char *cmi_dao_last_error(cmi_dao_handle h);
int cmi_dao_counts(cmi_dao_handle h, int64_t out[8]);
int cmi_dao_matrix(cmi_dao_handle h, int32_t *ui, int32_t *ctx, double *r);
int cmi_dao_ui_maps(cmi_dao_handle h, int32_t *ui_user, int32_t *ui_item);
int64_t cmi_dao_ctx_nnz(cmi_dao_handle h);
int cmi_dao_ctx_table(cmi_dao_handle h, int32_t *ctx_ptr, int32_t *ctx_conds);
int cmi_dao_cond_info(cmi_dao_handle h, int32_t *cond_dim, int32_t *empty_conds, int32_t *n_empty);
int cmi_dao_rating_scale(cmi_dao_handle h, double *out, int32_t cap, int32_t *n);
const char *cmi_dao_raw_id(cmi_dao_handle h, int kind, int32_t idx);

int cmi_java_hashmap_order(int64_t n, const char *const *keys, int64_t *positions, int *treeified);
int cmi_transform_compact_to_binary(const char *in_path, const char *out_path, int *treeified);
int cmi_validate_data_format(const char *path);
int cmi_transform(const char *train_in, const char *train_out, const char *test_in, const char *test_out, int *treeified);


int cmi_level_schedule(int64_t n, const int32_t *u, const int32_t *j, int32_t n_users, int32_t n_items, int order,
                       int32_t *perm, int64_t *level_off, int64_t level_cap, int64_t *n_levels);

int cmi_chain_schedule(int64_t n, const int32_t *u, const int32_t *j, int32_t n_users, int32_t n_items, int hub, int max_chain,
                       int32_t *perm, int32_t *unit_off, int64_t unit_cap, int64_t *level_off, int64_t level_cap,
                       int64_t *n_units, int64_t *n_levels, int *hub_used);
int cmi_chain_schedule_device(int device, int64_t n, const int32_t *u, const int32_t *j, int32_t n_users, int32_t n_items, int hub, int max_chain,
                              int32_t *perm, int32_t *unit_off, int64_t unit_cap, int64_t *level_off, int64_t level_cap,
                              int64_t *n_units, int64_t *n_levels, int *hub_used);

int cmi_narrow_runs(int64_t n_levels, const int64_t *level_off, int64_t max_tuples, int64_t min_levels, int32_t *run_len,
                    int64_t *n_launches);
int cmi_conflict_free_blocks(int64_t n, const int32_t *u, const int32_t *j, int32_t n_users, int32_t n_items, int32_t max_block,
                             int32_t *off, int64_t off_cap, int64_t *n_blocks);

int cmi_owner_schedule(int64_t n, const int32_t *u, const int32_t *j, int32_t n_users, int32_t n_items, int hub, int n_owners, int depth,
                       int32_t *perm, int64_t *own_off, uint32_t *want, uint32_t *flags, int *hub_used);

#define CMI_KNN_USER 0
#define CMI_KNN_ITEM 1
#define CMI_SIM_PCC 0
#define CMI_SIM_COS 1
#define CMI_SIM_COS_BINARY 2
#define CMI_SIM_MSD 3
#define CMI_SIM_CPC 4
#define CMI_SIM_EXJACCARD 5
typedef struct cmi_knn_instance *cmi_knn_handle;
int cmi_knn_measure(const char *name);
int cmi_knn_create(int kind, int n_users, int n_items, int device, unsigned flags, cmi_knn_handle *out);
int cmi_knn_destroy(cmi_knn_handle h);
const char *cmi_knn_last_error(cmi_knn_handle h);
int cmi_knn_set_ratings(cmi_knn_handle h, int64_t n, const int32_t *u, const int32_t *i, const double *r);
int cmi_knn_build(cmi_knn_handle h, int measure, int shrinkage, double min_rate, double max_rate);
int cmi_knn_get_similarity(cmi_knn_handle h, int32_t row0, int32_t nrows, double *dst);
#define CMI_KNN_MAX_CANDIDATES 16384
int cmi_knn_predict_batch(cmi_knn_handle h, int64_t n, const int32_t *u, const int32_t *j, int knn, double global_mean, int bound,
                          double lo, double hi, double *out);
int cmi_knn_last_build_ms(cmi_knn_handle h, float *ms);

#ifdef __cplusplus
}
#endif
#endif
```

Baseline: 3.937 billion.

## Pack chain unit headers into 16-byte records to shorten kernel prologue loads

Replaces the per-unit offset array with a 16-byte header holding the unit start, hub id, first spoke id and first arena position, built on host or device during scheduling. The chain kernels then fetch these with one vector load instead of a chain of dependent gathers through su/sj/next_pos. It also moves the first spoke row load ahead of the spoke-bias load so it is issued earlier. The cost is 16 bytes per unit instead of 4, an extra header kernel after arena setup, and new API entry points.

```diff
diff --git a/carskit_amd/capi.py b/carskit_amd/capi.py
--- a/carskit_amd/capi.py
+++ b/carskit_amd/capi.py
@@ -125,6 +125,8 @@
                                      C.POINTER(_i64), C.POINTER(C.c_int)]),
     ("cmi_chain_schedule_device", C.c_int, [C.c_int, _i64, _vp, _vp, _i32, _i32, C.c_int, C.c_int, _vp, _vp, _i64, _vp, _i64, C.POINTER(_i64),
                                      C.POINTER(_i64), C.POINTER(C.c_int)]),
+    ("cmi_chain_schedule_headers", C.c_int, [C.c_int, _i64, _vp, _vp, _i32, _i32, C.c_int, C.c_int, _vp, _i64, C.POINTER(_i64)]),
+    ("cmi_chain_unit_headers", C.c_int, [_vp, _vp, _i64, C.POINTER(_i64)]),
     ("cmi_dao_read", C.c_int, [C.c_char_p, C.POINTER(_vp)]),
     ("cmi_dao_read_shared", C.c_int, [C.c_char_p, _vp, C.POINTER(_vp)]),
     ("cmi_dao_destroy", C.c_int, [_vp]),
@@ -257,6 +259,9 @@
     return bytes(buf)
 
 
+_SINCE_UNIT_HEADERS = ("cmi_chain_schedule_headers", "cmi_chain_unit_headers")
+
+
 class CmiError(RuntimeError):
     def __init__(self, code, msg):
         super().__init__("libcarskit_mi355x error %d: %s" % (code, msg))
@@ -271,6 +276,8 @@
                           "(there is no Python/CPU fallback for the compute path)" % LIB_PATH)
         L = C.CDLL(LIB_PATH)
         for name, res, args in SYMBOLS:
+            if name in _SINCE_UNIT_HEADERS and not hasattr(L, name):
+                continue
             fn = getattr(L, name)
             fn.restype = res
             fn.argtypes = args
@@ -345,6 +352,21 @@
     if rc != OK:
         raise CmiError(rc, "cmi_chain_schedule_device")
     return perm, unit_off[:nu.value + 1], level_off[:nl.value + 1], bool(hub_used.value)
+
+
+def chain_schedule_headers(u, j, n_users, n_items, hub=-1, max_chain=16, device=-1):
+    u = np.ascontiguousarray(u, dtype=np.int32)
+    j = np.ascontiguousarray(j, dtype=np.int32)
+    n = len(u)
+    nu, nl, hub_used = _i64(), _i64(), C.c_int()
+    rc = lib().cmi_chain_schedule(n, _p(u), _p(j), n_users, n_items, hub, max_chain, None, None, 0, None, 0, C.byref(nu), C.byref(nl), C.byref(hub_used))
+    if rc != OK:
+        raise CmiError(rc, "cmi_chain_schedule")
+    hdr = np.empty((nu.value + 1, 4), dtype=np.int32)
+    rc = lib().cmi_chain_schedule_headers(device, n, _p(u), _p(j), n_users, n_items, hub, max_chain, _p(hdr), len(hdr), C.byref(nu))
+    if rc != OK:
+        raise CmiError(rc, "cmi_chain_schedule_headers")
+    return hdr[:nu.value + 1]
 
 
 def owner_schedule(u, j, n_users, n_items, n_owners, hub=-1, depth=8):
@@ -652,6 +674,13 @@
             d["flow_blocks"] &= 0xffffffff
         return d
 
+    def chain_unit_headers(self):
+        nu = _i64()
+        self._chk(self.L.cmi_chain_unit_headers(self.h, None, 0, C.byref(nu)))
+        hdr = np.empty((nu.value + 1, 4), dtype=np.int32)
+        self._chk(self.L.cmi_chain_unit_headers(self.h, _p(hdr), len(hdr), C.byref(nu)))
+        return hdr
+
     def schedule_note(self):
         return self.L.cmi_schedule_note(self.h).decode()
 
diff --git a/carskit_amd/csrc/chain_kernels.hip b/carskit_amd/csrc/chain_kernels.hip
--- a/carskit_amd/csrc/chain_kernels.hip
+++ b/carskit_amd/csrc/chain_kernels.hip
@@ -34,18 +34,14 @@
 };
 
 template <typename T, int MODEL, int NV, bool RAGGED, bool HUB_ITEM>
-__device__ __forceinline__ void chain_load_spoke(const SgdArgs<T> &a, int spoke, int cond, int l16, int K, SpokeRow<T, NV> &r, int64_t pos = 0,
-                                                 int nx = 0) {
-    using M = Traits<MODEL>;
+__device__ __forceinline__ void chain_load_spoke_rows(const SgdArgs<T> &a, int spoke, int l16, int K, SpokeRow<T, NV> &r, int64_t pos = 0, int nx = 0) {
     using V = typename Vec16<T>::type;
     constexpr int E = Vec16<T>::E;
-    constexpr bool SC = HUB_ITEM ? M::has_uc : M::has_ic;
     T *tab = HUB_ITEM ? a.P : a.Q;
     const T *src = a.arena ? a.arena + (size_t)pos * K : tab + (size_t)spoke * K;
     r.dst = a.arena ? a.arena + (size_t)nx * K : tab + (size_t)spoke * K;
     const V *row = reinterpret_cast<const V *>(src) + l16;
     r.spoke = spoke;
-    r.cond = cond;
 #pragma unroll
     for (int v = 0; v < NV; ++v) {
         T z[E];
@@ -54,12 +50,24 @@
         r.v[v] = pack(z);
         if (!RAGGED || E * l16 + 16 * E * v < K) r.v[v] = row[v * 16];
     }
+}
+template <typename T, int MODEL, int NV, bool HUB_ITEM>
+__device__ __forceinline__ void chain_load_spoke_cell(const SgdArgs<T> &a, int cond, SpokeRow<T, NV> &r) {
+    using M = Traits<MODEL>;
+    constexpr bool SC = HUB_ITEM ? M::has_uc : M::has_ic;
+    r.cond = cond;
     r.sc = (T)0;
     r.psc = nullptr;
     if (SC && cond >= 0) {
-        r.psc = (HUB_ITEM ? a.ucBias : a.icBias) + (size_t)spoke * a.n_conds + cond;
+        r.psc = (HUB_ITEM ? a.ucBias : a.icBias) + (size_t)r.spoke * a.n_conds + cond;
         r.sc = *r.psc;
     }
+}
+template <typename T, int MODEL, int NV, bool RAGGED, bool HUB_ITEM>
+__device__ __forceinline__ void chain_load_spoke(const SgdArgs<T> &a, int spoke, int cond, int l16, int K, SpokeRow<T, NV> &r, int64_t pos = 0,
+                                                 int nx = 0) {
+    chain_load_spoke_rows<T, MODEL, NV, RAGGED, HUB_ITEM>(a, spoke, l16, K, r, pos, nx);
+    chain_load_spoke_cell<T, MODEL, NV, HUB_ITEM>(a, cond, r);
 }
 
 template <typename T>
@@ -153,6 +161,15 @@
     return (b + 15) & ~(size_t)15;
 }
 
+struct ChainHdr {
+    int32_t tb, len;
+    int hub, sp0, nx0;
+};
+__device__ __forceinline__ ChainHdr chain_header(const ChainUnitHdr *__restrict__ unit_hdr, int64_t q) {
+    const ChainUnitHdr h = unit_hdr[q];
+    const int32_t te = unit_hdr[q + 1].tb;
+    return ChainHdr{h.tb, te - h.tb, h.hub, h.sp0, h.nx0};
+}
 template <typename T>
 struct ChainPre {
     int32_t tb, len;
@@ -162,17 +179,18 @@
 };
 
 template <typename T, bool HAS_CTX, bool HUB_ITEM>
-__device__ __forceinline__ ChainPre<T> chain_prefetch_ids(const SgdArgs<T> &a, int32_t tb, int32_t te, int l16, int dmax) {
+__device__ __forceinline__ ChainPre<T> chain_prefetch_ids(const SgdArgs<T> &a, const ChainHdr &hd, int l16, int dmax) {
+    const int32_t tb = hd.tb;
     ChainPre<T> p;
     p.tb = tb;
-    p.len = te - tb;
-    p.hub = HUB_ITEM ? a.sj[tb] : a.su[tb];
-    p.sp0 = HUB_ITEM ? a.su[tb] : a.sj[tb];
+    p.len = hd.len;
+    p.hub = hd.hub;
+    p.sp0 = hd.sp0;
     p.cd0 = (HAS_CTX && l16 < dmax) ? a.sconds[(int64_t)tb * dmax + l16] : -1;
     p.my_sp = 0;
     p.my_nx = 0;
     p.my_rr = (T)0;
-    p.nx0 = a.next_pos ? a.next_pos[tb] : 0;
+    p.nx0 = hd.nx0;
     if (l16 < p.len) {
         p.my_sp = HUB_ITEM ? a.su[tb + l16] : a.sj[tb + l16];
         p.my_rr = a.sr[tb + l16];
@@ -235,10 +253,11 @@
         }
     }
     T *sb_tab = HUB_ITEM ? a.userBias : a.itemBias;
+    SpokeRow<T, NV> A, B;
+    chain_load_spoke_rows<T, MODEL, NV, RAGGED, HUB_ITEM>(a, pre.sp0, l16, K, A, tb, pre.nx0);
+    chain_load_spoke_cell<T, MODEL, NV, HUB_ITEM>(a, pre.cd0, A);
     T my_sb = (T)0;
     if (SB && l16 < len) my_sb = sb_tab[pre.my_sp];
-    SpokeRow<T, NV> A, B;
-    chain_load_spoke<T, MODEL, NV, RAGGED, HUB_ITEM>(a, pre.sp0, pre.cd0, l16, K, A, tb, pre.nx0);
 
     if (l16 < len) {
         s_sp[l16] = pre.my_sp;
@@ -289,7 +308,7 @@
 }
 
 template <typename T, int MODEL, int NV, bool RAGGED, bool HUB_ITEM>
-__global__ __launch_bounds__(256) void sgd_chain_level(SgdArgs<T> a, const int32_t *__restrict__ unit_off, int64_t ubegin, int count,
+__global__ __launch_bounds__(256) void sgd_chain_level(SgdArgs<T> a, const ChainUnitHdr *__restrict__ unit_hdr, int64_t ubegin, int count,
                                                        int64_t slot0) {
     using M = Traits<MODEL>;
     constexpr int E = Vec16<T>::E;
@@ -306,9 +325,8 @@
     const ChainHp<T> hp{(T)hpd.lr, (T)hpd.regU, (T)hpd.regI, (T)hpd.regB, (T)hpd.regC, (T)hpd.gm};
 
     if (g < count) {
-        const int32_t tb = unit_off[ubegin + g], te = unit_off[ubegin + g + 1];
-        const ChainPre<T> pre = chain_prefetch_ids<T, M::has_ctx, HUB_ITEM>(a, tb, te, l16, dmax);
-        chain_unit<T, MODEL, NV, RAGGED, HUB_ITEM>(a, hp, pre, chain_smem + (size_t)gib * chain_group_lds(HC ? a.n_conds : 0, dmax, sizeof(T)),
+        const ChainHdr hd = chain_header(unit_hdr, ubegin + g);
+        chain_unit<T, MODEL, NV, RAGGED, HUB_ITEM>(a, hp, chain_prefetch_ids<T, M::has_ctx, HUB_ITEM>(a, hd, l16, dmax), chain_smem + (size_t)gib * chain_group_lds(HC ? a.n_conds : 0, dmax, sizeof(T)),
                                                    l16, K, dmax, gloss);
     }
 
@@ -417,7 +435,7 @@
 }
 
 template <int MODEL, int LPT, bool HUB_ITEM>
-__global__ __launch_bounds__(256) void sgd_chain_small(SgdArgs<float> a, const int32_t *__restrict__ unit_off, int64_t ubegin, int count,
+__global__ __launch_bounds__(256) void sgd_chain_small(SgdArgs<float> a, const ChainUnitHdr *__restrict__ unit_hdr, int64_t ubegin, int count,
                                                        int64_t slot0) {
     using M = Traits<MODEL>;
     static_assert(MODEL != CAMF_C, "CAMF_C has no level schedule (shared condBias)");
@@ -435,8 +453,9 @@
     const ChainHp<float> hp{(float)hpd.lr, (float)hpd.regU, (float)hpd.regI, (float)hpd.regB, (float)hpd.regC, (float)hpd.gm};
 
     if (g < count) {
-        const int32_t tb = unit_off[ubegin + g], te = unit_off[ubegin + g + 1];
-        const int len = te - tb;
+        const ChainHdr hd = chain_header(unit_hdr, ubegin + g);
+        const int32_t tb = hd.tb;
+        const int len = hd.len;
         unsigned char *gbase = chain_smem + (size_t)gib * chain_group_lds(HC ? a.n_conds : 0, dmax, sizeof(float));
         float *s_hc = reinterpret_cast<float *>(gbase);
         float *s_rr = s_hc + (HC ? a.n_conds : 0);
@@ -444,8 +463,7 @@
         int *s_cd = s_sp + 16;
         const int n_cd = len * dmax;
 
-        const int hub = HUB_ITEM ? a.sj[tb] : a.su[tb];
-        const int sp0 = HUB_ITEM ? a.su[tb] : a.sj[tb];
+        const int hub = hd.hub, sp0 = hd.sp0;
         const int cd0 = lt < dmax ? a.sconds[(int64_t)tb * dmax + lt] : -1;
         int my_sp[16 / LPT];
         float my_rr[16 / LPT];
@@ -626,7 +644,7 @@
 }
 
 template <typename T>
-hipError_t launch_chain_level(const SgdArgs<T> &a, const LaunchCfg &cfg, bool hub_is_item, const int32_t *unit_off, int64_t ubegin,
+hipError_t launch_chain_level(const SgdArgs<T> &a, const LaunchCfg &cfg, bool hub_is_item, const ChainUnitHdr *unit_hdr, int64_t ubegin,
                               int count, int64_t slot0, hipStream_t s) {
     if (count <= 0) return hipSuccess;
     const bool f64 = sizeof(T) == 8;
@@ -637,13 +655,13 @@
     });
     if (!fn) return hipErrorInvalidValue;
     SgdArgs<T> args = a;
-    void *params[] = {&args, &unit_off, &ubegin, &count, &slot0};
+    void *params[] = {&args, &unit_hdr, &ubegin, &count, &slot0};
     const size_t lds = (size_t)groups * (chain_lds_bytes(cfg.model, a.n_conds, a.dmax, f64, hub_is_item) / 16);
     return hipLaunchKernel(fn, dim3((unsigned)chain_level_blocks(a.k, a.dmax, f64, count)), dim3(256), params, lds, s);
 }
-template hipError_t launch_chain_level<float>(const SgdArgs<float> &, const LaunchCfg &, bool, const int32_t *, int64_t, int, int64_t,
+template hipError_t launch_chain_level<float>(const SgdArgs<float> &, const LaunchCfg &, bool, const ChainUnitHdr *, int64_t, int, int64_t,
                                               hipStream_t);
-template hipError_t launch_chain_level<double>(const SgdArgs<double> &, const LaunchCfg &, bool, const int32_t *, int64_t, int, int64_t,
+template hipError_t launch_chain_level<double>(const SgdArgs<double> &, const LaunchCfg &, bool, const ChainUnitHdr *, int64_t, int, int64_t,
                                                hipStream_t);
 
 }
diff --git a/carskit_amd/csrc/cmi_api.cpp b/carskit_amd/csrc/cmi_api.cpp
--- a/carskit_amd/csrc/cmi_api.cpp
+++ b/carskit_amd/csrc/cmi_api.cpp
@@ -100,7 +100,7 @@
         h->graph_exec = nullptr;
     }
     abi_free(h->d_su, h->d_sj, h->d_sconds, h->d_ctx_ptr, h->d_ctx_conds, h->d_sr, h->d_loss_part, h->d_flow_err, h->d_tail_off, h->d_blk_off,
-             h->d_unit_off, h->d_ui_ptr, h->d_ui_items, h->d_own_recs, h->d_own_off, h->d_tagged);
+             h->d_unit_hdr, h->d_ui_ptr, h->d_ui_items, h->d_own_recs, h->d_own_off, h->d_tagged);
     h->sched = Sched::NONE;
     h->level_kernel = LevelKernel::GENERIC;
     h->owner_stalled = false;
@@ -807,7 +807,7 @@
                                                 h->f64, h->d_su, h->d_sj, h->d_sconds, h->d_sr);
     }
     free_keep(keep);
-    if (e == hipSuccess && h->sched == Sched::CHAIN) e = abi_upload(&h->d_unit_off, csch.unit_off, h->stream);
+    if (e == hipSuccess && h->sched == Sched::CHAIN) e = abi_upload(&h->d_unit_hdr, csch.unit_hdr, h->stream);
     return e;
 }
 
@@ -846,6 +846,7 @@
         h->d_arena = spec.take(arena_bytes);
         if (!h->d_arena) e = hipMalloc(&h->d_arena, arena_bytes);
     }
+    if (e == hipSuccess) e = (hipError_t)chain_headers_set_next(h->stream, h->n_units, h->d_unit_hdr, h->d_next);
     if (e == hipSuccess) e = hipStreamSynchronize(h->stream);
     if (e == hipSuccess) {
         h->arena_on = true;
@@ -992,7 +993,7 @@
     if (h->sched == Sched::OWNER)
         h->tuple_bytes = (n + (int64_t)h->n_owners * 2 * owner_depth()) * (int64_t)owner_rec_bytes(owner_mask_words(h->model, h->n_conds));
     else
-        h->tuple_bytes = n * (8 + (int64_t)esize(h) + 4 * (int64_t)dmax) + (h->sched == Sched::CHAIN ? 4 * (h->n_units + 1) : 0) +
+        h->tuple_bytes = n * (8 + (int64_t)esize(h) + 4 * (int64_t)dmax) + (h->sched == Sched::CHAIN ? (int64_t)sizeof(ChainUnitHdr) * (h->n_units + 1) : 0) +
                          (h->arena_on ? 4 * n : 0);
     h->have_ratings = true;
     return CMI_OK;
@@ -1055,8 +1056,8 @@
     if (h->sched == Sched::CHAIN) {
         const bool hi = h->chain_hub_item;
         const bool hub_b = hi ? bj : bu, spk_b = hi ? bu : bj, hub_c = hi ? ic : uc, spk_c = hi ? uc : ic;
-        const int64_t unit_sect = row + (hub_b ? 2 * SECT : 0) + (hub_c ? ctx_row_sect : 0) + 4;
-        const int64_t unit_own = row + (hub_b ? 2 * e : 0) + (hub_c ? ctx_row_own : 0) + 4;
+        const int64_t unit_sect = row + (hub_b ? 2 * SECT : 0) + (hub_c ? ctx_row_sect : 0) + (int64_t)sizeof(ChainUnitHdr);
+        const int64_t unit_own = row + (hub_b ? 2 * e : 0) + (hub_c ? ctx_row_own : 0) + (int64_t)sizeof(ChainUnitHdr);
         const int64_t arena_idx = h->arena_on ? 4 : 0;
         const int64_t tup_sect = stream + arena_idx + row + (spk_b ? 2 * SECT : 0) + (spk_c ? cells_sect : 0);
         const int64_t tup_own = stream + arena_idx + row + (spk_b ? 2 * e : 0) + (spk_c ? cells_own : 0);
@@ -1225,7 +1226,7 @@
         const int64_t b = h->level_off[(size_t)l], slot = h->slot_off[(size_t)l];
         const int cnt = (int)(h->level_off[(size_t)l + 1] - b);
         const int32_t run = h->tail_len[(size_t)l];
-        if (h->sched == Sched::CHAIN) e = launch_chain_level<T>(a, cfg, h->chain_hub_item, h->d_unit_off, b, cnt, slot, h->stream);
+        if (h->sched == Sched::CHAIN) e = launch_chain_level<T>(a, cfg, h->chain_hub_item, h->d_unit_hdr, b, cnt, slot, h->stream);
         else if (run > 0) {
             e = launch_narrow_run<T>(a, cfg, h->level_kernel, h->d_tail_off + l, run, slot, h->stream);
             l += run - 1;
@@ -1821,6 +1822,45 @@
     });
 }
 
+extern "C" int cmi_chain_schedule_headers(int device, int64_t n, const int32_t *u, const int32_t *j, int32_t n_users, int32_t n_items, int hub,
+                                          int max_chain, int32_t *hdr, int64_t hdr_cap, int64_t *n_units) {
+    return abi_barrier(cmi_thread_err(), "cmi_chain_schedule_headers", [&] {
+        if (n < 0 || (n > 0 && (!u || !j)) || n_users <= 0 || n_items <= 0 || !n_units || max_chain < 1) return CMI_E_INVALID;
+        if (device >= cmi_device_count()) return CMI_E_NO_DEVICE;
+        for (int64_t t = 0; t < n; ++t)
+            if (u[t] < 0 || u[t] >= n_users || j[t] < 0 || j[t] >= n_items) return CMI_E_INVALID;
+        ChainSchedule cs;
+        if (device < 0) {
+            if (!build_chain_schedule(n, u, j, n_users, n_items, hub, max_chain, cs)) return CMI_E_UNSUPPORTED;
+        } else {
+            hipStream_t st = nullptr;
+            if (hipSetDevice(device) != hipSuccess || hipStreamCreateWithFlags(&st, hipStreamNonBlocking) != hipSuccess) return CMI_E_HIP;
+            const bool ok = build_chain_schedule_device(device, st, n, u, j, n_users, n_items, hub, max_chain, cs);
+            (void)hipStreamDestroy(st);
+            if (!ok) return CMI_E_UNSUPPORTED;
+        }
+        *n_units = cs.n_units();
+        if (!hdr) return CMI_OK;
+        if (hdr_cap < cs.n_units() + 1) return CMI_E_INVALID;
+        memcpy(hdr, cs.unit_hdr.data(), cs.unit_hdr.size() * sizeof(ChainUnitHdr));
+        return CMI_OK;
+    });
+}
+
+extern "C" int cmi_chain_unit_headers(cmi_handle h, int32_t *hdr, int64_t hdr_cap, int64_t *n_units) {
+    if (!h || !n_units) return CMI_E_INVALID;
+    return abi_barrier(h->err, "cmi_chain_unit_headers", [&] {
+        if (!h->have_ratings || h->sched != Sched::CHAIN) CMI_FAIL(h, CMI_E_INVALID, "chain_unit_headers: the instance has no hub-chain schedule");
+        *n_units = h->n_units;
+        if (!hdr) return (int)CMI_OK;
+        if (hdr_cap < h->n_units + 1) return (int)CMI_E_INVALID;
+        CMI_HIP(h, hipSetDevice(h->device));
+        CMI_HIP(h, hipStreamSynchronize(h->stream));
+        CMI_HIP(h, hipMemcpy(hdr, h->d_unit_hdr, (size_t)(h->n_units + 1) * sizeof(ChainUnitHdr), hipMemcpyDeviceToHost));
+        return (int)CMI_OK;
+    });
+}
+
 extern "C" int cmi_owner_schedule(int64_t n, const int32_t *u, const int32_t *j, int32_t n_users, int32_t n_items, int hub, int n_owners,
                                   int depth, int32_t *perm, int64_t *own_off, uint32_t *want, uint32_t *flags, int *hub_used) {
     return abi_barrier(cmi_thread_err(), "cmi_owner_schedule", [&] {
diff --git a/carskit_amd/csrc/cmi_instance.hpp b/carskit_amd/csrc/cmi_instance.hpp
--- a/carskit_amd/csrc/cmi_instance.hpp
+++ b/carskit_amd/csrc/cmi_instance.hpp
@@ -28,7 +28,7 @@
     Sched sched = Sched::NONE;
     cmi::LevelKernel level_kernel = cmi::LevelKernel::GENERIC;
     bool chain_hub_item = true;
-    int32_t *d_unit_off = nullptr;
+    cmi::ChainUnitHdr *d_unit_hdr = nullptr;
     int64_t n_units = 0;
     bool arena_on = false, arena_valid = false, table_valid = true;
     bool arena_probe_table = false;
diff --git a/carskit_amd/csrc/level_schedule.cpp b/carskit_amd/csrc/level_schedule.cpp
--- a/carskit_amd/csrc/level_schedule.cpp
+++ b/carskit_amd/csrc/level_schedule.cpp
@@ -258,6 +258,7 @@
     if (max_chain < 1) max_chain = 1;
     if (max_chain > 255) max_chain = 255;
     out.hub_is_item = hub == 0 ? 0 : 1;
+    out.unit_hdr.assign(1, ChainUnitHdr{0, 0, 0, 0});
     if (n <= 0) return true;
     if (n >= (int64_t)1 << 31) return false;
     struct Side {
@@ -335,6 +336,14 @@
         for (int64_t t = b; t < e; ++t)
             out.perm[(size_t)out.unit_off[(size_t)rank[(size_t)unit_of[(size_t)t]]] + pos[(size_t)t]] = (int32_t)t;
     });
+    out.unit_hdr.assign((size_t)nu + 1, ChainUnitHdr{0, 0, 0, 0});
+    parallel_ranges(nu, host_threads(nu), [&](int, int64_t b, int64_t e) {
+        for (int64_t q = b; q < e; ++q) {
+            const int32_t tb = out.unit_off[(size_t)q], t = out.perm[(size_t)tb];
+            out.unit_hdr[(size_t)q] = ChainUnitHdr{tb, hub ? j[t] : u[t], hub ? u[t] : j[t], 0};
+        }
+    });
+    out.unit_hdr[(size_t)nu].tb = (int32_t)n;
     return true;
 }
 
diff --git a/carskit_amd/csrc/level_schedule.hpp b/carskit_amd/csrc/level_schedule.hpp
--- a/carskit_amd/csrc/level_schedule.hpp
+++ b/carskit_amd/csrc/level_schedule.hpp
@@ -18,10 +18,15 @@
                           int within_level_order, LevelSchedule &out);
 
 
+struct alignas(16) ChainUnitHdr {
+    int32_t tb, hub, sp0, nx0;
+};
+static_assert(sizeof(ChainUnitHdr) == 16, "the chain kernels load a header as one 16-byte vector");
 struct ChainSchedule {
     std::vector<int32_t> perm;
     std::vector<int32_t> unit_off;
     std::vector<int64_t> level_off;
+    std::vector<ChainUnitHdr> unit_hdr;
     int hub_is_item = 1;
     int64_t max_level_units = 0;
     int64_t n_units() const { return (int64_t)unit_off.size() - 1; }
diff --git a/carskit_amd/csrc/mf_sgd_kernels.hpp b/carskit_amd/csrc/mf_sgd_kernels.hpp
--- a/carskit_amd/csrc/mf_sgd_kernels.hpp
+++ b/carskit_amd/csrc/mf_sgd_kernels.hpp
@@ -2,6 +2,8 @@
 
 #include <hip/hip_runtime.h>
 #include <stdint.h>
+
+#include "level_schedule.hpp"
 
 namespace cmi {
 
@@ -75,7 +77,7 @@
 int chain_groups_per_block(int k, int dmax, bool f64);
 int chain_level_blocks(int k, int dmax, bool f64, int count);
 template <typename T>
-hipError_t launch_chain_level(const SgdArgs<T> &a, const LaunchCfg &cfg, bool hub_is_item, const int32_t *unit_off, int64_t ubegin,
+hipError_t launch_chain_level(const SgdArgs<T> &a, const LaunchCfg &cfg, bool hub_is_item, const ChainUnitHdr *unit_hdr, int64_t ubegin,
                               int count, int64_t slot0, hipStream_t s);
 
 template <typename T>
diff --git a/carskit_amd/csrc/sched_device.hip b/carskit_amd/csrc/sched_device.hip
--- a/carskit_amd/csrc/sched_device.hip
+++ b/carskit_amd/csrc/sched_device.hip
@@ -265,6 +265,21 @@
     for (int64_t t = (int64_t)blockIdx.x * blockDim.x + threadIdx.x; t < n; t += (int64_t)gridDim.x * blockDim.x)
         perm[unit_off[rank_of[dense[unit_of[t]]]] + pos[t]] = (int32_t)t;
 }
+__global__ void k_unit_hdr(const int32_t *unit_off, const int32_t *perm, const int32_t *hub_of, const int32_t *spoke_of, int64_t nu, ChainUnitHdr *hdr) {
+    for (int64_t q = (int64_t)blockIdx.x * blockDim.x + threadIdx.x; q <= nu; q += (int64_t)gridDim.x * blockDim.x) {
+        const int32_t tb = unit_off[q];
+        ChainUnitHdr r{tb, 0, 0, 0};
+        if (q < nu) {
+            const int32_t t = perm[tb];
+            r.hub = hub_of[t];
+            r.sp0 = spoke_of[t];
+        }
+        hdr[q] = r;
+    }
+}
+__global__ void k_unit_hdr_next(const int32_t *next, int64_t nu, ChainUnitHdr *hdr) {
+    for (int64_t q = (int64_t)blockIdx.x * blockDim.x + threadIdx.x; q < nu; q += (int64_t)gridDim.x * blockDim.x) hdr[q].nx0 = next[hdr[q].tb];
+}
 __global__ void k_level_off(const uint32_t *skey, int64_t nu, int32_t nl, int32_t max_chain, int64_t *level_off) {
     const int l = blockIdx.x * blockDim.x + threadIdx.x;
     if (l > nl) return;
@@ -433,6 +448,7 @@
     if (max_chain < 1) max_chain = 1;
     if (max_chain > 255) max_chain = 255;
     out.hub_is_item = hub == 0 ? 0 : 1;
+    out.unit_hdr.assign(1, ChainUnitHdr{0, 0, 0, 0});
     if (n <= 0) return true;
     if (n >= ((int64_t)1 << 31) - 1024) return false;
     if (hipSetDevice(device) != hipSuccess) return false;
@@ -522,6 +538,7 @@
     int32_t *uid = pool.get<int32_t>((size_t)nu), *suid = pool.get<int32_t>((size_t)nu), *rank_of = pool.get<int32_t>((size_t)nu);
     int32_t *len_sorted = pool.get<int32_t>((size_t)nu + 1), *unit_off = pool.get<int32_t>((size_t)nu + 1), *perm = pool.get<int32_t>((size_t)n);
     uint8_t *ulen = pool.get<uint8_t>((size_t)nu);
+    ChainUnitHdr *hdr = pool.get<ChainUnitHdr>((size_t)nu + 1);
     int64_t *level_off = pool.get<int64_t>((size_t)nl + 1);
     if (pool.err != hipSuccess) return fail("allocation", pool.err);
     hipLaunchKernelGGL(k_flags, dim3(grid_for(n)), dim3(256), 0, s, wo.unit_level, n, flag);
@@ -551,9 +568,11 @@
         if (hipError_t e = rocprim::exclusive_scan(tmp, tb, len_sorted, unit_off, 0, (size_t)nu + 1, rocprim::plus<int32_t>(), s)) return fail("scan", e);
     }
     hipLaunchKernelGGL(k_perm, dim3(grid_for(n)), dim3(256), 0, s, wo.unit_of, wo.pos, dense, rank_of, unit_off, n, perm);
+    hipLaunchKernelGGL(k_unit_hdr, dim3(grid_for(nu + 1)), dim3(256), 0, s, unit_off, perm, hub ? dj : du, hub ? du : dj, nu, hdr);
     hipLaunchKernelGGL(k_level_off, dim3((unsigned)((nl + 1 + 255) / 256)), dim3(256), 0, s, skey, nu, nl, max_chain, level_off);
     if (hipError_t e = hipGetLastError()) return fail("kernels", e);
     out.unit_off.assign((size_t)nu + 1, 0);
+    out.unit_hdr.assign((size_t)nu + 1, ChainUnitHdr{0, 0, 0, 0});
     out.level_off.assign((size_t)nl + 1, 0);
     if (keep) {
         for (int32_t *q : {du, dj, perm}) pool.ptrs.erase(std::find(pool.ptrs.begin(), pool.ptrs.end(), (void *)q));
@@ -565,6 +584,7 @@
         if (hipMemcpyAsync(out.perm.data(), perm, (size_t)n * 4, hipMemcpyDeviceToHost, s) != hipSuccess) return fail("copy back", hipGetLastError());
     }
     if (hipMemcpyAsync(out.unit_off.data(), unit_off, ((size_t)nu + 1) * 4, hipMemcpyDeviceToHost, s) != hipSuccess) return fail("copy back", hipGetLastError());
+    if (hipMemcpyAsync(out.unit_hdr.data(), hdr, ((size_t)nu + 1) * sizeof(ChainUnitHdr), hipMemcpyDeviceToHost, s) != hipSuccess) return fail("copy back", hipGetLastError());
     if (hipMemcpyAsync(out.level_off.data(), level_off, ((size_t)nl + 1) * 8, hipMemcpyDeviceToHost, s) != hipSuccess) return fail("copy back", hipGetLastError());
     if (hipError_t e = hipStreamSynchronize(s)) return fail("synchronize", e);
     lap("unit sort + offsets + copy back");
@@ -625,4 +645,10 @@
     return (int)hipStreamSynchronize(s);
 }
 
-}
+int chain_headers_set_next(void *stream, int64_t n_units, ChainUnitHdr *d_unit_hdr, const int32_t *d_next) {
+    if (n_units <= 0) return (int)hipSuccess;
+    hipLaunchKernelGGL(k_unit_hdr_next, dim3(grid_for(n_units)), dim3(256), 0, (hipStream_t)stream, d_next, n_units, d_unit_hdr);
+    return (int)hipGetLastError();
+}
+
+}
diff --git a/carskit_amd/csrc/sched_device.hpp b/carskit_amd/csrc/sched_device.hpp
--- a/carskit_amd/csrc/sched_device.hpp
+++ b/carskit_amd/csrc/sched_device.hpp
@@ -22,4 +22,6 @@
 
 int arena_positions_device(void *stream, int64_t n, const int32_t *d_spoke_stream, int64_t n_spokes, int32_t *d_next, int32_t *d_first);
 
+int chain_headers_set_next(void *stream, int64_t n_units, ChainUnitHdr *d_unit_hdr, const int32_t *d_next);
+
 }
diff --git a/include/carskit_mi355x.h b/include/carskit_mi355x.h
--- a/include/carskit_mi355x.h
+++ b/include/carskit_mi355x.h
@@ -236,6 +236,10 @@
                               int32_t *perm, int32_t *unit_off, int64_t unit_cap, int64_t *level_off, int64_t level_cap,
                               int64_t *n_units, int64_t *n_levels, int *hub_used);
 
+int cmi_chain_schedule_headers(int device, int64_t n, const int32_t *u, const int32_t *j, int32_t n_users, int32_t n_items, int hub,
+                               int max_chain, int32_t *hdr, int64_t hdr_cap, int64_t *n_units);
+int cmi_chain_unit_headers(cmi_handle h, int32_t *hdr, int64_t hdr_cap, int64_t *n_units);
+
 int cmi_narrow_runs(int64_t n_levels, const int64_t *level_off, int64_t max_tuples, int64_t min_levels, int32_t *run_len,
                     int64_t *n_launches);
 int cmi_conflict_free_blocks(int64_t n, const int32_t *u, const int32_t *j, int32_t n_users, int32_t n_items, int32_t max_block,
```

After: 3.876 billion. -1.5%, worse.
